# avikde/robobee3d

Hardware: AMD Instinct MI355X
Metric: closed-loop MPC steps/sec (QP+dyn) (higher is better)
Workload: dtype f32

## Files before the change

### robobee3d_amd/asmstep.py

```python
import functools
import os
import struct

from . import asmgen, asmtext, symbolic
from .asmgen import (A_D, A_L, A_LO, A_M, A_Q, NLDS, NVZ, S_ALPHA, S_CNT, S_ITERS, S_OMA, S_RHO, S_RINV, S_SIGMA,
                     V_W, V_WZ, V_X, V_Y, V_Z, Emit, f32bits, pk, _sb, _vp)

HERE = os.path.dirname(os.path.abspath(__file__))

PTRS = ["state", "ctrl", "ref", "ws", "out", "stats", "status", "info", "Ib", "gain", "aT0",
        "taskf", "weights", "wl", "wlu", "wlw",
        "done"]
NPTR_RES = 11
INTS = ["stride", "K", "maxIter", "nsub", "plant", "seq"]
TAIL_INTS = ["refstep"]
FLOATS = ["dt", "dtg", "Tmax", "wpr", "wpf", "ws_", "wvr", "wvf", "wds", "wthrust", "wmom",
          "iwpr", "iwpf", "iws", "iwvr", "iwvf", "iwds", "iwthrust", "iwmom",
          "Ib0", "Ib1", "Ib2", "Ibi0", "Ibi1", "Ibi2", "h", "hh", "h6", "taulim", "gpl", "idt", "mbg"]
WNAMES = ["wpr", "wpf", "ws_", "wvr", "wvf", "wds", "wthrust", "wmom"]
WROW = {"ws_": 0, "wds": 1, "wpr": 2, "wpf": 3, "wvr": 4, "wvf": 5, "wthrust": 6, "wmom": 7}
A_W, A_IW = 230, 238
S_PARAM = 4
S_PBLK = 2
S_PTR = {n: 40 + 2 * k for k, n in enumerate(PTRS[:NPTR_RES])}
S_PTR["taskf"], S_PTR["weights"] = 0, 96
S_PTR["wl"], S_PTR["wlu"], S_PTR["wlw"] = 30, 32, 34
S_INT = {"stride": 10, "K": 13, "maxIter": S_ITERS, "nsub": 5, "plant": 39}
S_F = {n: 64 + k for k, n in enumerate(FLOATS)}
assert max(S_F.values()) <= 95
S_STEP, S_SUB, S_RUIZ = 12, 15, 15
S_EXACT = 14
S_MBAD, S_MP0 = 62, 14
S_M0, S_M1, S_M2, S_M3 = 30, 32, 34, 36
S_C = {"minscal": 16, "maxscal": 17, "c45": 18, "eps10": 19, "eps": 38, "rho": 6, "rinv": 7, "rmin": 8,
       "rmininv": 9, "infty_ms": 100, "rhotol": 101}
S_TMP = 4
OFF = {}
_o = 0
for _n in PTRS:
    OFF[_n] = _o
    _o += 8
for _n in INTS + FLOATS + TAIL_INTS:
    OFF[_n] = _o
    _o += 4
PARAM_BYTES = _o
HIST_INTS = ["statestep", "outstep", "statusstep", "infostep"]
HIST_OFF = (PARAM_BYTES + 7) // 8 * 8
for _k, _n in enumerate(HIST_INTS):
    OFF[_n] = HIST_OFF + 4 * _k
HIST_BYTES = 4 * len(HIST_INTS)
S_HIST = 32
IMP_OFF = HIST_OFF + HIST_BYTES
assert IMP_OFF % 8 == 0
OFF["imp"], OFF["impstep"] = IMP_OFF, IMP_OFF + 8
IMP_BYTES = 16
S_IMP = 32

VFIRST, VEND = 2, 256
NRING = 6
XV_N, XV_B = 2, 254
NT_PTRS = ("state", "ctrl", "ref", "out", "stats")
A_SPARE, N_SPARE_D = 246, 9


class Pool:

    def __init__(self, e):
        self.e = e
        self.free_ = set(range(VFIRST, VEND))
        self.peak = 0
        self.fixed = set()

    def _take(self, regs):
        for r in regs:
            assert r in self.free_, "v%d is not free" % r
            self.free_.discard(r)
        self.peak = max(self.peak, VEND - VFIRST - len(self.free_))

    def reserve(self, lo, n):
        self._take(range(lo, lo + n))
        return lo

    def get(self):
        cand = sorted(self.free_)
        assert cand, "out of VGPRs"
        for r in cand:
            if (r ^ 1) not in self.free_:
                self._take([r])
                return r
        self._take([cand[0]])
        return cand[0]

    def get2(self):
        for r in sorted(self.free_):
            if r % 2 == 0 and r + 1 in self.free_:
                self._take([r, r + 1])
                return r
        raise AssertionError("out of aligned VGPR pairs")

    def get4(self):
        for r in sorted(self.free_):
            if r % 4 == 0 and all(r + k in self.free_ for k in range(4)):
                self._take([r, r + 1, r + 2, r + 3])
                return r
        raise AssertionError("out of aligned VGPR quads")

    def getn(self, n):
        for r in sorted(self.free_):
            if r % 2 == 0 and all(r + k in self.free_ for k in range(n)):
                self._take(range(r, r + n))
                return r
        raise AssertionError("out of consecutive VGPRs")

    def getn_high(self, n):
        r = VEND - n - (VEND - n) % 2
        assert all(r + k in self.free_ for k in range(n)), "top of the register file is not free"
        self._take(range(r, r + n))
        return r

    def free(self, *regs, kill=True):
        for r in regs:
            assert r not in self.free_ and VFIRST <= r < VEND, "double free v%d" % r
            self.free_.add(r)
            if kill:
                self.e("kill", "v%d" % r)

    def free_range(self, lo, n, kill=True):
        self.free(*range(lo, lo + n), kill=kill)


def v(n):
    return "v%d" % n


def SF_(n):
    return "s%d" % S_F[n]


def sg(n):
    return "s%d" % n


def sp(n):
    return "s[%d:%d]" % (n, n + 1)

# ... 17 lines not shown
    return ("v[%d:%d]" % (base, base + 1), lo_reg % 2, hi_reg % 2)


def PS(sreg):
    if sreg % 2 == 0:
        return ("s[%d:%d]" % (sreg, sreg + 1), 0, 0)
    return ("s[%d:%d]" % (sreg - 1, sreg), 1, 1)


class Struct:
    def __init__(self, N=3, perm=None):
        s = symbolic.analyse(N, perm)
        self.s = s
        self.plan = asmgen.solve_plan(s)
        self.lpos = self.plan[2]
        self.xs, self.zs, self.xinv, self.zinv = asmgen.slot_maps(s)
        nx, nc = s.nx, s.nc
        self.neq = 2 * s.N * symbolic.NY
        self.col_of = [0] * len(s.A_i)
        self.rows = [[] for _ in range(nc)]
        for j in range(nx):
            for p in range(s.A_p[j], s.A_p[j + 1]):
                self.col_of[p] = j
                self.rows[s.A_i[p]].append(p)
        self.unit = {}
        for p, tag in enumerate(s.A_tag):
            if tag[0] == 'c' and abs(tag[1]) == 1.0 and s.A_i[p] not in self.unit:
                self.unit[s.A_i[p]] = (p, self.col_of[p])
        assert len(self.unit) == nc
        used, pairs = set(), []
        for p in range(len(s.A_i)):
            if p in used:
                continue
            i0, j0 = s.A_i[p], self.col_of[p]
            for q_ in range(p + 1, len(s.A_i)):
                if q_ in used:
                    continue
                i1, j1 = s.A_i[q_], self.col_of[q_]
                if (self.zs[i0] ^ 1) == self.zs[i1] and (j0 == j1 or (self.xs[j0] ^ 1) == self.xs[j1]):
                    lo, hi = (p, q_) if self.zs[i0] % 2 == 0 else (q_, p)
                    pairs.append((lo, hi))
                    used.update((p, q_))
                    break
        self.apairs = pairs
        self.asingles = [p for p in range(len(s.A_i)) if p not in used]
        self.apos = [0] * len(s.A_i)
        k = 0
        for (lo, hi) in pairs:
            self.apos[lo], self.apos[hi] = k, k + 1
            k += 2
        for p in self.asingles:
            self.apos[p] = k
            k += 1
        self.na = k
        self.pair_of = {}
        for (lo, hi) in pairs:
            self.pair_of[lo] = self.pair_of[hi] = (lo, hi)
        NYv = symbolic.NY
        self.qnz = list(range(s.N * NYv)) + [s.N * NYv + k_ * NYv + i for k_ in range(s.N) for i in range(3)]
        self.qslot = {}
        for j in range(s.N * NYv):
            self.qslot[j] = self.xs[j]
        base = s.N * NYv
        for k_ in range(s.N):
            for i in range(3):
                self.qslot[s.N * NYv + k_ * NYv + i] = base + 3 * k_ + i
        self.nq = base + 3 * s.N
        self.qzero = frozenset(j for j in range(nx) if j not in self.qslot)
        lnz = set(range(6)) | set(range(3 * 6, 3 * 6 + 6)) | set(range(4 * 6, 4 * 6 + 3)) | {5 * 6 + 2}
        self.lzero = frozenset(i for i in range(self.neq) if i not in lnz) if s.N == 3 else frozenset()

    def weight_of(self, j):
        N, NYv = self.s.N, symbolic.NY
        if j < N * NYv:
            k, i = divmod(j, NYv)
            return ("wpf" if k == N - 1 else "wpr") if i < 3 else "ws_"
        if j < 2 * N * NYv:
            k, i = divmod(j - N * NYv, NYv)
            return ("wvf" if k == N - 1 else "wvr") if i < 3 else "wds"
        return "wthrust" if (j - 2 * N * NYv) % 3 == 0 else "wmom"


class StepGen:
    def __init__(self, N=3, perm=None, quad=False, exact_ruiz=False):
        self.st = Struct(N, perm)
        self.s = self.st.s
        self.e = Emit()
        self.pool = Pool(self.e)
        self.lab = 20
        self.lab_spec = 500
        self.quad = quad
        self.speculate = not quad and not exact_ruiz
        self.ruiz_span = self.restart_at = None
        self.nt = () if quad else ("nt",)
        self.homes = asmgen.Homes(NRING, 0 if quad else XV_N, XV_B)

    def label(self):
        self.lab += 1
        return str(self.lab)

    def label_spec(self):
        self.lab_spec += 1
        return str(self.lab_spec)

    def rcp_nr(self, dst, src, t):
        e = self.e
        e("v_rcp_f32", v(dst), v(src))
        e("s_nop", 0)
        e("v_fma_f32", v(t), "-" + v(src), v(dst), 1.0)
        e("v_fma_f32", v(dst), v(t), v(dst), v(dst))

    def rows_ptr(self, voff, first_row):
        e = self.e
        if first_row == 0:
            e("v_mov_b32", v(voff), "v0")
        else:
            e("s_mul_i32", sg(S_TMP), sg(S_INT["stride"]), first_row)
            e("v_add_u32", v(voff), sg(S_TMP), "v0")

    def load_taskf(self):
        e = self.e
        e("s_lshl_b32", sg(S_TMP), sg(S_STEP), 5)
        e("s_load_dwordx2", sp(S_M0), sp(S_PTR["taskf"]), sg(S_TMP), "offset:0")
        e("s_load_dwordx4", "s[%d:%d]" % (S_M0 + 2, S_M0 + 5), sp(S_PTR["taskf"]), sg(S_TMP), "offset:8")
        e("s_load_dwordx2", sp(S_M0 + 6), sp(S_PTR["taskf"]), sg(S_TMP), "offset:24")
        e("s_waitcnt", "vmcnt(0) lgkmcnt(0)")

    def adv(self, voff):
        self.e("v_add_u32", v(voff), sg(S_INT["stride"]), v(voff))

    def advance_ptr(self, ptr, sstep):
        e, lo = self.e, S_PTR[ptr]
        e("s_add_i32", sg(lo), sg(lo), sg(sstep))
        e("s_cmp_lt_u32", sg(lo), sg(sstep))
        e("s_cselect_b32", sg(sstep), 1, 0)
        e("s_add_i32", sg(lo + 1), sg(lo + 1), sg(sstep))

    def impulse(self, Y0, YS):
        e = self.e
        lab_off = self.label()
        lo, hi, st, oh = S_IMP, S_IMP + 1, S_IMP + 2, S_IMP + 3
        e("s_mov_b32", sg(S_TMP), IMP_OFF)
        e("s_load_dwordx4", "s[%d:%d]" % (S_IMP, S_IMP + 3), sp(S_PBLK), sg(S_TMP))
        e("s_waitcnt", "lgkmcnt(0)")
        e("s_cmp_eq_u64", sp(lo), 0)
        e("s_cbranch_scc1", lab_off + "f")
        e("s_mul_hi_u32", sg(oh), sg(S_STEP), sg(st))
        e("s_mul_i32", sg(st), sg(S_STEP), sg(st))
        e("s_add_i32", sg(hi), sg(hi), sg(oh))
        for i in range(6):
            addend = st if i == 0 else S_INT["stride"]
            lab_nc = self.label()
            e("s_add_i32", sg(lo), sg(lo), sg(addend))
            e("s_cmp_gt_u32", sg(addend), sg(lo))
            e("s_cbranch_scc0", lab_nc + "f")
            e("s_add_i32", sg(hi), sg(hi), 1)
            e("label", lab_nc)
            e("global_load_dword", v(YS + i), "v0", sp(lo))
        e("s_waitcnt", "vmcnt(0)")
        for i in range(6):
            e("v_add_f32", v(Y0 + 12 + i), v(Y0 + 12 + i), v(YS + i))
        e("label", lab_off)

    def load_rows(self, ptr, first_row, regs, voff=None):
        own = voff is None
        if own:
            voff = self.pool.get()
        self.rows_ptr(voff, first_row)
        for k, r in enumerate(regs):
            self.e("global_load_dword", r if isinstance(r, str) else v(r), v(voff), sp(S_PTR[ptr]),
                   *(self.nt if ptr in NT_PTRS or ptr == "ws" else ()))
            if k + 1 < len(regs):
                self.adv(voff)
        if own:
            self.pool.free(voff, kill=False)

    def store_rows(self, ptr, first_row, regs, voff=None):
        own = voff is None
        if own:
            voff = self.pool.get()
        self.rows_ptr(voff, first_row)
        for k, r in enumerate(regs):
            self.e("global_store_dword", v(voff), v(r), sp(S_PTR[ptr]),
                   *(self.nt if ptr in NT_PTRS else ()))
            if k + 1 < len(regs):
                self.adv(voff)
        if own:
            self.pool.free(voff, kill=False)

    def prologue(self):
        e = self.e
        P = sp(S_PARAM)
        e("s_mov_b64", sp(S_PBLK), P)
        P = sp(S_PBLK)
        e("s_load_dwordx16", "s[40:55]", P, OFF["state"])
        e("s_load_dwordx4", "s[56:59]", P, OFF["state"] + 64)
        e("s_load_dwordx2", "s[60:61]", P, OFF["state"] + 80)
        e("s_load_dwordx2", sp(S_PTR["taskf"]), P, OFF["taskf"])
        e("s_load_dwordx2", sp(S_PTR["weights"]), P, OFF["weights"])
        e("s_load_dwordx16", "s[64:79]", P, OFF[FLOATS[0]])
        e("s_load_dwordx16", "s[80:95]", P, OFF[FLOATS[0]] + 64)
        for n in S_INT:
            e("s_load_dword", sg(S_INT[n]), P, OFF[n])
        assert len(FLOATS) == 32
        import numpy as np
        f32 = np.float32
        for reg, val in ((S_ALPHA, 1.6), (S_OMA, float(f32(1.0) - f32(1.6))), (S_SIGMA, 1e-6), (S_RINV, 0.01), (S_RHO, 100.0)):
            e("s_mov_b32", sg(reg), f32bits(val))
            e("s_mov_b32", sg(reg + 1), f32bits(val))
        for name, val in (("minscal", 1e-4), ("maxscal", 1e4), ("c45", float(f32(1.0) / f32(self.s.nx))),
                          ("eps", 1e-4), ("eps10", float(f32(10) * f32(1e-4))), ("rho", 0.1), ("rinv", float(f32(1.0) / f32(0.1))),
                          ("rmin", 1e-6), ("rmininv", float(f32(1.0) / f32(1e-6))),
                          ("infty_ms", float(f32(1e30) * f32(1e-4))), ("rhotol", 1e-4)):
            e("s_mov_b32", sg(S_C[name]), f32bits(val))
        e("s_waitcnt", "lgkmcnt(0)")
        e("s_mov_b32", sg(S_STEP), 0)

    def phase_a(self):
        e, pool, st, s = self.e, self.pool, self.st, self.s
        N, NYv = s.N, symbolic.NY
        nx, nc, neq = s.nx, s.nc, st.neq
        SF = lambda n: sg(S_F[n])
        ST = [pool.get() for _ in range(18)]
        RF = [pool.get() for _ in range(9)]
        T0, EP = pool.get(), [pool.get() for _ in range(N)]
        voff = pool.get()
        self.load_rows("state", 0, ST, voff)
        self.load_rows("ref", 0, RF, voff)
        self.load_rows("ctrl", nx + 2 * nc, [T0] + EP, voff)
        WV = {n: pool.get() for n in WNAMES}
        IWV = {n: pool.get() for n in WNAMES}
        self.WV = WV
        lab_w, lab_w2 = self.label(), self.label()
        e("s_cmp_eq_u64", sp(S_PTR["weights"]), 0)
        e("s_cbranch_scc1", lab_w + "f")
        self.rows_ptr(voff, 0)
        by_row = sorted(WNAMES, key=lambda n: WROW[n])
        for k, n in enumerate(by_row):
            e("global_load_dword", v(WV[n]), v(voff), sp(S_PTR["weights"]))
            if k + 1 < len(by_row):
                self.adv(voff)
        e("s_waitcnt", "vmcnt(0)")
        t = pool.get()
        for n in WNAMES:
            self.rcp_nr(IWV[n], WV[n], t)
        pool.free(t)
        e("s_branch", lab_w2 + "f")
        e("label", lab_w)
        for n in WNAMES:
            e("v_mov_b32", v(WV[n]), SF(n))
            e("v_mov_b32", v(IWV[n]), SF("i" + n.rstrip("_")))
        e("label", lab_w2)
        for k, n in enumerate(WNAMES):
            e("v_accvgpr_write_b32", "a%d" % (A_W + k), v(WV[n]))
            e("v_accvgpr_write_b32", "a%d" % (A_IW + k), v(IWV[n]))
        pool.free(*IWV.values(), *WV.values())
        lab_tk = self.label()
        e("s_cmp_eq_u64", sp(S_PTR["taskf"]), 0)
        e("s_cbranch_scc1", lab_tk + "f")
        self.load_taskf()
        for i in range(3):
            e("v_add_f32", v(RF[i]), sg(S_M0 + i), v(RF[i]))
            e("v_mov_b32", v(RF[3 + i]), sg(S_M0 + 3 + i))
        e("v_mov_b32", v(RF[6]), sg(S_M0 + 6))
        e("v_mov_b32", v(RF[7]), 0)
        e("v_mov_b32", v(RF[8]), sg(S_M0 + 7))
        e("label", lab_tk)
        ibi0, ibi1 = pool.get(), pool.get()
        lab_ib, lab_ib2 = self.label(), self.label()
        e("s_cmp_eq_u64", sp(S_PTR["Ib"]), 0)
        e("s_cbranch_scc1", lab_ib + "f")
        t = pool.get()
        self.load_rows("Ib", 0, [ibi0, ibi1], voff)
        e("s_waitcnt", "vmcnt(0)")
        tt = pool.get()
        for r in (ibi0, ibi1):
            e("v_mov_b32", v(tt), v(r))
            self.rcp_nr(r, tt, t)
        pool.free(t, tt)
        e("s_branch", lab_ib2 + "f")
        e("label", lab_ib)
        e("v_mov_b32", v(ibi0), SF("Ibi0"))
        e("v_mov_b32", v(ibi1), SF("Ibi1"))
        e("label", lab_ib2)
        e("s_waitcnt", "vmcnt(0)")
        lab_t = self.label()
        e("s_cmp_eq_u64", sp(S_PTR["aT0"]), 0)
        e("s_cbranch_scc1", lab_t + "f")
        e("s_cmp_lg_u32", sg(S_STEP), 0)
        e("s_cbranch_scc1", lab_t + "f")
        t = pool.get()
        e("global_load_dword", v(t), "v0", sp(S_PTR["aT0"]))
        e("s_waitcnt", "vmcnt(0)")
        e("v_cmp_le_f32", "vcc", 0, v(t))
        e("v_cndmask_b32", v(T0), v(T0), v(t), "vcc")
        pool.free(t)
        e("label", lab_t)
        self.store_rows("ctrl", nx + 2 * nc, [T0], voff)
# ... 574 lines not shown
                    e("v_mov_b32", v(XV_B + pos - NLDS - NVZ), v(nL[j]))
                else:
                    e("v_accvgpr_write_b32", "a%d" % (A_L + pos - NLDS), v(nL[j]))
                pool.free(nL.pop(j))
            retire_dinv(c)

        for op in s.factor_ops:
            k = op["k"]
            src = s.K_src[op["diag"]]
            dk = pool.get()
            if src[0] == 'P':
                e("v_add_f32", v(dk), sg(S_SIGMA), v(RP(src[1])))
                pool.free(RP(src[1]))
            else:
                assert src[0] == 'R'
                i = src[1]
                if i < neq:
                    e("v_mul_f32", v(dk), -1.0, self._vconst_rinv())
                else:
                    e("v_accvgpr_read_b32", v(dk), "a%d" % (A_M + 9 + i - neq))
                    e("s_nop", 0)
                    e("v_mul_f32", v(dk), -1.0, v(dk))
            y = {}
            for (b, p) in op["init"]:
                assert s.K_src[p][0] == 'A'
                y[b] = (RA(s.K_src[p][1]), False)
            for (c, upd, new) in op["elim"]:
                yc, owned = y.pop(c)
                for (lj, row) in upd:
                    if row in y:
                        reg, own = y[row]
                        if own:
                            e("v_fmac_f32", v(reg), v(nL[lj]), v(yc))
                        else:
                            nr = pool.get()
                            e("v_fma_f32", v(nr), v(nL[lj]), v(yc), v(reg))
                            pool.free(reg)
                            y[row] = (nr, True)
                    else:
                        nr = pool.get()
                        e("v_mul_f32", v(nr), v(nL[lj]), v(yc))
                        y[row] = (nr, True)
                nl = pool.get()
                e("v_mul_f32", v(nl), "-" + v(yc), v(Dinv[c]))
                e("v_fmac_f32", v(dk), v(yc), v(nl))
                nL[new] = nl
                pool.free(yc)
            assert not y
            di = pool.get()
            self.rcp_nr(di, dk, t)
            pool.free(dk)
            Dinv[k] = di
            for c in done_at.get(k, []):
                retire_col(c)
            if k not in last_row:
                retire_dinv(k)
        assert not nL and not Dinv
        pool.free(t)
        if self._rinv_reg is not None:
            pool.free(self._rinv_reg)
            self._rinv_reg = None
        if st.na % 2:
            pool.free(self.VA + st.na)
        pool.free(self.VP + nx)

    _rinv_reg = None

    def _vconst_rinv(self):
        if self._rinv_reg is None:
            self._rinv_reg = self.pool.get()
            self.e("v_mov_b32", v(self._rinv_reg), sg(S_RINV))
        return v(self._rinv_reg)

    def admm(self):
        e, pool, st, s = self.e, self.pool, self.st, self.s
        nx, nc = s.nx, s.nc
        left = set(range(VFIRST, VEND)) - pool.free_ - set(range(246, 256))
        assert not left, "phase A leaked registers: %s" % sorted(left)
        pool.reserve(V_W, V_X - V_W)
        pool.reserve(V_X, V_Y - V_X)
        pool.reserve(V_Y, V_Z - V_Y)
        pool.reserve(V_Z, 40)
        voff = 245
        self.load_rows("ctrl", 0, [V_X + st.xs[r] for r in range(nx)] + [V_Y + st.zs[r] for r in range(nc)] +
                       [V_Z + st.zs[r] for r in range(nc)], voff)
        for pad in (V_X + nx, V_Y + nc, V_Z + nc, V_W + nx, V_WZ + nc):
            e("v_mov_b32", v(pad), 0)
        e("s_waitcnt", "vmcnt(0) lgkmcnt(0)")
        plan = st.plan
        zk = dict(qzero=st.qzero, lzero=st.lzero, homes=self.homes)
        asmgen.body(e, s, first=True, capture=True, plan=plan, delta_in_w=True, **zk)
        if self.quad:
            from . import asmquad
            lab6 = self.label()
            e("s_cmp_lt_i32", sg(S_ITERS), 2)
            e("s_cbranch_scc1", lab6 + "f")
            asmquad.section(e, asmquad.QuadPlan(st), self.label)
            e("label", lab6)
        else:
            self._admm_rest(plan, zk)
        for i in range(st.neq):
            pool.free(V_Z + st.zs[i], kill=True)
        pool.free_range(246, 10)


    def _admm_rest(self, plan, zk):
        e, s, st = self.e, self.s, self.st
        import numpy as np
        for p_ in range(NVZ):
            e("v_accvgpr_read_b32", v(V_Z + p_), "a%d" % (A_L + p_))
        lab7, lab6 = self.label(), self.label()
        e("s_sub_i32", sg(S_CNT), sg(S_ITERS), 1)
        e("s_cmp_lt_i32", sg(S_CNT), 1)
        e("s_cbranch_scc1", lab6 + "f")
        e("label", lab7)
        asmgen.body(e, s, first=False, capture=False, plan=plan, lv=True, dy3_in_w=True, **zk)
        e("s_sub_i32", sg(S_CNT), sg(S_CNT), 1)
        e("s_cmp_gt_i32", sg(S_CNT), 0)
        e("s_cbranch_scc1", lab7 + "b")
        k = float(np.float32(1.6) / (np.float32(1.6) - np.float32(1.0)))
        e("s_mov_b32", sg(S_TMP), f32bits(k))
        nx, neq = s.nx, st.neq
        for p_ in range(0, nx - 1, 2):
            pk(e, "v_pk_add_f32", V_W + p_, [P2(V_X + p_), P2(V_W + p_)], [0, 1])
        for p_ in range(0, nx - 1, 2):
            pk(e, "v_pk_mul_f32", V_W + p_, [PS(S_TMP), P2(V_W + p_)])
        if nx % 2:
            jl = st.xinv[nx - 1]
            e("v_sub_f32", v(V_W + st.xs[jl]), v(V_X + st.xs[jl]), v(V_W + st.xs[jl]))
            e("v_mul_f32", v(V_W + st.xs[jl]), sg(S_TMP), v(V_W + st.xs[jl]))
        for p_ in range(0, neq, 2):
            pk(e, "v_pk_add_f32", V_WZ + p_, [P2(V_Y + p_), P2(V_WZ + p_)], [0, 1])
        for p_ in range(0, neq, 2):
            pk(e, "v_pk_mul_f32", V_WZ + p_, [PS(S_TMP), P2(V_WZ + p_)])
        e("label", lab6)

    def phase_c(self):
        e, pool, st, s = self.e, self.pool, self.st, self.s
        N, NYv = s.N, symbolic.NY
        nx, nc, neq = s.nx, s.nc, st.neq
        SF = lambda n: sg(S_F[n])
        g_ = pool.get
        XR = lambda j: V_X + st.xs[j]
        YR = lambda i: V_Y + st.zs[i]
        ZR = lambda i: V_Z + st.zs[i]
        DXR = lambda j: V_W + st.xs[j]
        DYR = lambda i: V_WZ + st.zs[i]
        voff = g_()
        def slot_blocks(n, chunk=16):
            n2 = n + n % 2
            blocks = [(lo, pool.getn(min(chunk, n2 - lo))) for lo in range(0, n2, chunk)]
            def reg(slot):
                for lo, base in reversed(blocks):
                    if slot >= lo:
                        return base + slot - lo
            return reg, [(base, min(chunk, n2 - lo)) for lo, base in blocks]
        DS, dblocks = slot_blocks(nx)
        DR = lambda j: DS(st.xs[j])
        cr, T0 = g_(), g_()
        npark = 0 if self.quad else N_SPARE_D
        self.load_rows("ws", npark, [DR(j) for j in range(npark, nx)], voff)
        if npark:
            for j in range(npark):
                e("v_accvgpr_read_b32", v(DR(j)), "a%d" % (A_SPARE + j))
            e("v_accvgpr_read_b32", v(cr), "a%d" % (A_SPARE + N_SPARE_D))
        else:
            self.load_rows("ws", asmgen.WS_C - asmgen.WS_DS, [cr], voff)
        self.load_rows("ctrl", nx + 2 * nc, [T0], voff)
        e("v_mov_b32", v(DS(nx)), 0)
        zt = [g_() for _ in range(4)]
        self.rows_ptr(voff, 0)
        for r in range(nx):
            e("global_store_dword", v(voff), v(XR(r)), sp(S_PTR["ctrl"]), *self.nt)
            self.adv(voff)
        for r in range(nc):
            e("global_store_dword", v(voff), v(YR(r)), sp(S_PTR["ctrl"]), *self.nt)
            self.adv(voff)
        for r in range(nc):
            if r < neq:
                t_ = zt[r % 4]
                e("v_accvgpr_read_b32", v(t_), "a%d" % (A_LO + r))
                e("global_store_dword", v(voff), v(t_), sp(S_PTR["ctrl"]), *self.nt)
            else:
                e("global_store_dword", v(voff), v(ZR(r)), sp(S_PTR["ctrl"]), *self.nt)
            self.adv(voff)
        pool.free(*zt)
        e("s_waitcnt", "vmcnt(0)")
        for k in range(0, nx + 1, 2):
            pk(e, "v_pk_mul_f32", V_W + k, [P2(DS(k)), P2(V_W + k)])
            pk(e, "v_pk_mul_f32", V_X + k, [P2(DS(k)), P2(V_X + k)])
        for base, n_ in dblocks:
            pool.free_range(base, n_)
        ES, eblocks = slot_blocks(nc)
        ER = lambda i: ES(st.zs[i])
        ST = [g_() for _ in range(18)]
        RF = [g_() for _ in range(9)]
        self.load_rows("ws", asmgen.WS_ES - asmgen.WS_DS, [ER(i) for i in range(nc)], voff)
        self.load_rows("state", 0, ST, voff)
        self.load_rows("ref", 0, RF, voff)
        e("v_mov_b32", v(ES(nc)), 1.0)
        lab_tk = self.label()
        e("s_cmp_eq_u64", sp(S_PTR["taskf"]), 0)
        e("s_cbranch_scc1", lab_tk + "f")
        self.load_taskf()
        for i in range(3):
            e("v_add_f32", v(RF[i]), sg(S_M0 + i), v(RF[i]))
            e("v_mov_b32", v(RF[3 + i]), sg(S_M0 + 3 + i))
        e("v_mov_b32", v(RF[6]), sg(S_M0 + 6))
        e("v_mov_b32", v(RF[7]), 0)
        e("v_mov_b32", v(RF[8]), sg(S_M0 + 7))
        e("label", lab_tk)
        cinv, t = g_(), g_()
        self.rcp_nr(cinv, cr, t)
        pool.free(cr)
        ibi0, ibi1 = g_(), g_()
        lab_ib, lab_ib2 = self.label(), self.label()
        e("s_cmp_eq_u64", sp(S_PTR["Ib"]), 0)
        e("s_cbranch_scc1", lab_ib + "f")
        self.load_rows("Ib", 0, [ibi0, ibi1], voff)
        e("s_waitcnt", "vmcnt(0)")
        tt = g_()
        for r in (ibi0, ibi1):
            e("v_mov_b32", v(tt), v(r))
            self.rcp_nr(r, tt, t)
        pool.free(tt)
        e("s_branch", lab_ib2 + "f")
        e("label", lab_ib)
        e("v_mov_b32", v(ibi0), SF("Ibi0"))
        e("v_mov_b32", v(ibi1), SF("Ibi1"))
        e("label", lab_ib2)
        e("s_waitcnt", "vmcnt(0)")
        for k in range(0, nc + 1, 2):
            pk(e, "v_pk_mul_f32", V_WZ + k, [P2(ES(k)), P2(V_WZ + k)])
            pk(e, "v_pk_mul_f32", V_Y + k, [P2(ES(k)), P2(V_Y + k)])
        for k in range(0, nc + 1, 2):
            pk(e, "v_pk_mul_f32", V_Y + k, [P2(V_Y + k), PB(cinv)])
        pool.free(cinv)
        zu3 = [g_() for _ in range(N)]
        for k in range(N):
            e("v_rcp_f32", v(zu3[k]), v(ER(neq + k)))
        e("s_nop", 0)
        for k in range(N):
            e("v_mul_f32", v(zu3[k]), v(ZR(neq + k)), v(zu3[k]))
        for base, n_ in eblocks:
            pool.free_range(base, n_)
        for k in range(N):
            pool.free(ZR(neq + k))
        pool.free(V_Z + nc)
        p0, R0, dq0 = ST[0:3], ST[3:12], ST[12:18]
        dtT0 = g_()
        e("v_mul_f32", v(dtT0), SF("dt"), v(T0))
        s0dt = [g_() for _ in range(3)]
        Bdt = [g_() for _ in range(6)]
        for i in range(3):
            e("v_mul_f32", v(s0dt[i]), SF("dt"), v(R0[6 + i]))
            e("v_mul_f32", v(Bdt[i]), "-" + v(R0[i + 3]), v(ibi0))
            e("v_mul_f32", v(Bdt[3 + i]), v(R0[i]), v(ibi1))
        for i in range(6):
            e("v_mul_f32", v(Bdt[i]), SF("dt"), v(Bdt[i]))
        pool.free(ibi0, ibi1)
        ds0 = [g_() for _ in range(3)]
        for r in range(3):
            e("v_mul_f32", v(t), "-" + v(R0[r]), v(dq0[4]))
            e("v_mul_f32", v(ds0[r]), v(R0[r + 3]), v(dq0[3]))
            e("v_add_f32", v(ds0[r]), v(t), v(ds0[r]))
            e("v_mul_f32", v(ds0[r]), -1.0, v(ds0[r]))
        y0 = p0 + R0[6:9]
        dy0 = dq0[0:3] + ds0
        LR = {}
# ... 175 lines not shown
        e("v_fma_f32", v(a1), sg(S_C["eps"]), v(reld), sg(S_C["eps"]))
        lt(MD0, v(dua), v(a1))
        e("v_fma_f32", v(a1), sg(S_C["eps10"]), v(relp), sg(S_C["eps10"]))
        lt(MP1, v(pri), v(a1))
        e("v_fma_f32", v(a1), sg(S_C["eps10"]), v(reld), sg(S_C["eps10"]))
        lt(MD1, v(dua), v(a1))
        e("v_mov_b32", v(stv), -2)

        def cert(epsname, okmask, code, kind):
            nrm_, n_, s_, third = (ndy, lhs, nrm, None) if kind == "p" else (ndx, qdx, nP, nAdx)
            e("v_mul_f32", v(a1), sg(S_C[epsname]), v(nrm_))
            lt(MT, sg(S_C[epsname]), v(nrm_))
            e("s_andn2_b64", MT, MT, okmask)
            lt("vcc", v(n_), "-" + v(a1))
            e("s_and_b64", MT, MT, "vcc")
            lt("vcc", v(s_), v(a1))
            e("s_and_b64", MT, MT, "vcc")
            if third is not None:
                lt("vcc", v(a1), v(third))
                e("s_andn2_b64", MT, MT, "vcc")
            e("v_cndmask_b32_e64", v(stv), v(stv), code, MT)
        cert("eps10", MD1, 4, "d")
        cert("eps10", MP1, 3, "p")
        e("s_and_b64", MT, MP1, MD1)
        e("v_cndmask_b32_e64", v(stv), v(stv), 2, MT)
        cert("eps", MD0, -4, "d")
        cert("eps", MP0, -3, "p")
        e("s_and_b64", MT, MP0, MD0)
        e("v_cndmask_b32_e64", v(stv), v(stv), 1, MT)
        lt(MT, v(infv), v(pri))
        lt("vcc", v(infv), v(dua))
        e("s_or_b64", MT, MT, "vcc")
        e("v_cmp_u_f32", "vcc", v(nan), v(nan))
        e("s_or_b64", MT, MT, "vcc")
        e("v_cndmask_b32_e64", v(stv), v(stv), -7, MT)
        e("v_cmp_eq_i32_e64", MBAD, -7, v(stv))
        for code in (-3, 3, -4, 4):
            e("v_cmp_eq_i32_e64", MT, code, v(stv))
            e("s_or_b64", MBAD, MBAD, MT)
        pool.free(ndy, lhs, nrm, ndx, qdx, nP, nAdx, relp, reld, nAx, nz, nq, nAty, nPx, nan, infv, a3, a4)
        nanv = g_()
        e("v_mov_b32", v(nanv), f32bits(2143289344.0))
        sol = [XR(2 * N * NYv + i) for i in range(3)] + [XR(N * NYv + i) for i in range(6)]
        e("s_mov_b64", "vcc", MBAD)
        for r in sol:
            e("v_cndmask_b32", v(r), v(r), v(nanv), "vcc")
        pool.free(nanv)
        u0, u1, u2 = sol[0:3]
        dy1 = sol[3:9]
        OUT = [g_() for _ in range(9)]
        e("v_add_f32", v(OUT[0]), v(T0), v(u0))
        e("v_mov_b32", v(OUT[1]), v(u1))
        e("v_mov_b32", v(OUT[2]), v(u2))
        e("v_mul_f32", v(a1), v(R0[0]), v(dy1[3]))
        e("v_mul_f32", v(t), v(R0[1]), v(dy1[4]))
        e("v_add_f32", v(a1), v(a1), v(t))
        e("v_mul_f32", v(t), v(R0[2]), v(dy1[5]))
        e("v_add_f32", v(a1), v(a1), v(t))
        e("v_mul_f32", v(a2), v(R0[3]), v(dy1[3]))
        e("v_mul_f32", v(t), v(R0[4]), v(dy1[4]))
        e("v_add_f32", v(a2), v(a2), v(t))
        e("v_mul_f32", v(t), v(R0[5]), v(dy1[5]))
        e("v_add_f32", v(a2), v(a2), v(t))
        for i in range(3):
            e("v_sub_f32", v(OUT[3 + i]), v(dy1[i]), v(dq0[i]))
        e("v_sub_f32", v(OUT[6]), "-" + v(a2), v(dq0[3]))
        e("v_sub_f32", v(OUT[7]), v(a1), v(dq0[4]))
        e("v_sub_f32", v(OUT[8]), 0, v(dq0[5]))
        for i in range(6):
            e("v_mul_f32", v(OUT[3 + i]), SF("idt"), v(OUT[3 + i]))
        self.store_rows("out", 0, OUT, voff)
        lab_s, lab_i, lab_c = self.label(), self.label(), self.label()
        e("s_cmp_eq_u64", sp(S_PTR["status"]), 0)
        e("s_cbranch_scc1", lab_s + "f")
        e("global_store_dword", "v0", v(stv), sp(S_PTR["status"]))
        e("label", lab_s)
        e("s_cmp_eq_u64", sp(S_PTR["info"]), 0)
        e("s_cbranch_scc1", lab_i + "f")
        self.store_rows("info", 0, [pri, dua], voff)
        e("label", lab_i)
        e("s_and_saveexec_b64", sp(S_M1), MBAD)
        e("s_cbranch_execz", lab_c + "f")
        e("v_mov_b32", v(a1), 0)
        self.rows_ptr(voff, 0)
        for r in range(nx + 2 * nc):
            e("global_store_dword", v(voff), v(a1), sp(S_PTR["ctrl"]))
            self.adv(voff)
        e("label", lab_c)
        e("s_mov_b64", "exec", sp(S_M1))
        pool.free(pri, dua, stv, a1, a2, t, T0, *RF)
        pool.free_range(V_W, V_X - V_W, kill=False)
        pool.free_range(V_X, V_Y - V_X, kill=False)
        pool.free_range(V_Y, V_Z - V_Y, kill=False)
        T0n = g_()
        e("v_mov_b32", v(T0n), v(OUT[0]))
        self.wl_step(OUT, R0, T0n, voff)
        self.store_rows("ctrl", nx + 2 * nc, [T0n], voff)
        pool.free(T0n)
        self.plant(ST, OUT, voff)
        pool.free(*OUT, *ST, voff)
        assert len(pool.free_) == VEND - VFIRST, "phase C leaked registers: %s" % sorted(set(range(VFIRST, VEND)) - pool.free_)

    def wl_step(self, OUT, R0, T0n, voff):
        e, pool = self.e, self.pool
        g_ = pool.get
        lab_end = self.label()
        P = sp(S_PBLK)
        e("s_load_dwordx2", sp(S_PTR["wl"]), P, OFF["wl"])
        e("s_load_dwordx2", sp(S_PTR["wlu"]), P, OFF["wlu"])
        e("s_load_dwordx2", sp(S_PTR["wlw"]), P, OFF["wlw"])
        e("s_waitcnt", "lgkmcnt(0)")
        e("s_cmp_eq_u64", sp(S_PTR["wl"]), 0)
        e("s_cbranch_scc1", lab_end + "f")
        O_UMIN, O_UMAX, O_DUMAX, O_QW, O_A0, O_A1, O_A2, O_MD = 0, 4, 8, 12, 18, 24, 48, 144
        a1, a2, t = g_(), g_(), g_()
        zero = g_()
        e("v_mov_b32", v(zero), 0)

        def prm(dst, word):
            e("global_load_dword", v(dst), v(zero), sp(S_PTR["wl"]), "offset:%d" % (4 * word))
        u0 = [g_() for _ in range(4)]
        self.load_rows("wlu", 0, u0, voff)
        Md = [g_() for _ in range(6)]
        for i in range(6):
            prm(Md[i], O_MD + i)
        e("s_waitcnt", "vmcnt(0)")
        h0 = [g_() for _ in range(3)]
        pd = [g_() for _ in range(6)]
        for c in range(3):
            e("v_mul_f32", v(h0[c]), SF_("mbg"), v(R0[2 + 3 * c]))
        for i in range(6):
            e("v_mul_f32", v(pd[i]), v(Md[i]), v(OUT[3 + i]))
        w0 = [g_() for _ in range(6)]
        a0v = [g_() for _ in range(6)]
        A1 = [[g_() for _ in range(4)] for _ in range(6)]
        PA = [g_() for _ in range(21)]
        vout = [g_() for _ in range(4)]
        dot, quad = g_(), g_()
        for i in range(6):
            prm(PA[0], O_A0 + i)
            for l in range(4):
                prm(PA[1 + l], O_A1 + 4 * i + l)
            for k in range(16):
                prm(PA[5 + k], O_A2 + 16 * i + k)
            e("s_waitcnt", "vmcnt(0)")
            e("v_mul_f32", v(dot), v(u0[0]), v(PA[1]))
            for l in range(1, 4):
                e("v_mul_f32", v(t), v(u0[l]), v(PA[1 + l]))
                e("v_add_f32", v(dot), v(dot), v(t))
            for r in range(4):
                e("v_mul_f32", v(vout[r]), v(PA[5 + r]), v(u0[0]))
                for l in range(1, 4):
                    e("v_mul_f32", v(t), v(PA[5 + r + 4 * l]), v(u0[l]))
                    e("v_add_f32", v(vout[r]), v(vout[r]), v(t))
            e("v_mul_f32", v(quad), v(u0[0]), v(vout[0]))
            for l in range(1, 4):
                e("v_mul_f32", v(t), v(u0[l]), v(vout[l]))
                e("v_add_f32", v(quad), v(quad), v(t))
            e("v_add_f32", v(a1), v(PA[0]), v(dot))
            e("v_mul_f32", v(a2), 0.5, v(quad))
            e("v_add_f32", v(w0[i]), v(a1), v(a2))
            if i < 3:
                e("v_sub_f32", v(a0v[i]), v(w0[i]), v(h0[i]))
            else:
                e("v_mov_b32", v(a0v[i]), v(w0[i]))
            e("v_sub_f32", v(a0v[i]), v(a0v[i]), v(pd[i]))
# ... 322 lines not shown
        for k in range(0, 8, 2):
            pk(e, "v_pk_fma_f32", QS + k, [PS(S_F["hh"]), P2(QA + k), P2(Q0 + k)])
        vf(QS, QK)
        for k in range(0, 8, 2):
            pk(e, "v_pk_fma_f32", QA + k, [PB(two), P2(QK + k), P2(QA + k)])
            pk(e, "v_pk_fma_f32", QS + k, [PS(S_F["hh"]), P2(QK + k), P2(Q0 + k)])
        vf(QS, QK)
        for k in range(0, 8, 2):
            pk(e, "v_pk_fma_f32", QA + k, [PB(two), P2(QK + k), P2(QA + k)])
            pk(e, "v_pk_fma_f32", QS + k, [PS(S_F["h"]), P2(QK + k), P2(Q0 + k)])
        vf(QS, QK)
        for k in range(0, 8, 2):
            pk(e, "v_pk_add_f32", QA + k, [P2(QA + k), P2(QK + k)])
        for k in range(0, 8, 2):
            pk(e, "v_pk_fma_f32", Q0 + k, [PS(S_F["h6"]), P2(QA + k), P2(Q0 + k)])
        e("s_nop", 1)
        for r in range(3):
            e("v_mov_b32_dpp", v(PA + r), v(Q0), asmquad.qperm([r] * 4))
        e("s_nop", 1)
        for r in range(3):
            e("v_fmac_f32", v(serr), v(PA + r), v(PA + r))
        e("v_add_f32", v(seff), v(seff), v(einc))
        e("s_sub_i32", sg(S_SUB), sg(S_SUB), 1)
        e("s_cmp_gt_i32", sg(S_SUB), 0)
        e("s_cbranch_scc1", top + "b")
        e("s_nop", 1)
        for r in range(3):
            e("v_mov_b32_dpp", v(Y0 + r), v(Q0), asmquad.qperm([r] * 4))
            e("v_mov_b32_dpp", v(Y0 + 12 + r), v(Q0 + 1), asmquad.qperm([r] * 4))
            for c in range(3):
                e("v_mov_b32_dpp", v(Y0 + 3 + r + 3 * c), v(Q0 + 2 + c), asmquad.qperm([r] * 4))
        for i in range(3):
            e("v_mov_b32", v(Y0 + 15 + i), v(Q0 + 5 + i))
        e("s_nop", 1)
        e("quad_end", tuple(keep))

    def program(self):
        e = self.e
        self.prologue()
        top = self.label()
        e("label", top)
        if self.speculate:
            e("s_mov_b32", sg(S_EXACT), 0)
            self.lab_restart = self.label_spec()
            e("label", self.lab_restart)
        self.phase_a()
        self.admm()
        self.phase_c()
        e("s_load_dword", sg(S_TMP), sp(S_PBLK), OFF["refstep"])
        e("s_load_dwordx4", "s[%d:%d]" % (S_HIST, S_HIST + 3), sp(S_PBLK), HIST_OFF)
        e("s_waitcnt", "lgkmcnt(0)")
        e("s_add_u32", sg(S_PTR["ref"]), sg(S_PTR["ref"]), sg(S_TMP))
        e("s_addc_u32", sg(S_PTR["ref"] + 1), sg(S_PTR["ref"] + 1), 0)
        for n in ("out", "status", "info"):
            self.advance_ptr(n, S_HIST + HIST_INTS.index(n + "step"))
        e("s_add_i32", sg(S_STEP), sg(S_STEP), 1)
        e("s_cmp_lt_i32", sg(S_STEP), sg(S_INT["K"]))
        e("s_cbranch_scc1", top + "b")
        e("s_waitcnt", "vmcnt(0) lgkmcnt(0)")
        lab = self.label()
        e("s_load_dwordx2", sp(S_M0), sp(S_PBLK), OFF["done"])
        e("s_load_dword", sg(S_M1), sp(S_PBLK), OFF["seq"])
        e("s_waitcnt", "lgkmcnt(0)")
        e("s_cmp_eq_u64", sp(S_M0), 0)
        e("s_cbranch_scc1", lab + "f")
        e("buffer_wbl2", "sc0 sc1")
        e("s_waitcnt", "vmcnt(0)")
        a, b = self.pool.get(), self.pool.get()
        e("v_mov_b32", v(a), 0)
        e("v_mov_b32", v(b), sg(S_M1))
        e("global_store_dword", v(a), v(b), sp(S_M0), "sc0 sc1")
        e("s_waitcnt", "vmcnt(0)")
        self.pool.free(a, b)
        e("label", lab)
        return e.ins


fmt = functools.partial(asmtext.fmt, hex_ints=asmtext.HEX_ABOVE_64)


PSEUDO = ("kill", "quad_begin", "quad_end")


def write(path=None, N=3, perm=None, quad=False):
    path = path or os.path.join(HERE, "csrc", "umpc_step_asm_quad.h" if quad else "umpc_step_asm.h")
    g = StepGen(N, perm, quad=quad)
    ins = [t for t in g.program() if t[0] not in PSEUDO]
    if quad:
        head = ["// GENERATED by robobee3d_amd/asmstep.py (quad=True) + asmquad.py -- do not edit.", asmgen.switch_banner(),
               "// The all-assembly fp32 step kernel body, ONE ROBOT PER LANE QUAD (16 robots per wavefront): %d instructions."
               % len(ins),
               "// Every lane of a quad gets the same v0 (= 4 * robot) and its own LDS slice; include umpc_step_asm.h first (StepParams).",
               "#pragma once"]
    else:
        head = ["// GENERATED by robobee3d_amd/asmstep.py -- do not edit.", asmgen.switch_banner(),
               "// The all-assembly fp32 step kernel body: %d instructions (K closed-loop steps of one wavefront)." % len(ins),
               "#pragma once", "#include <stddef.h>", "#include <stdint.h>", "namespace umpcasm {",
               "// parameter block read by the kernel with s_load (byte offsets are part of the generated code)",
               "struct StepParams {"]
        for n in PTRS:
            head.append("  const void *%s;" % n)
        for n in INTS:
            head.append("  int32_t %s;" % n)
        for n in FLOATS:
            head.append("  float %s;" % n)
        for n in TAIL_INTS:
            head.append("  int32_t %s;" % n)
        head += ["};", "static_assert(sizeof(StepParams) == %d, \"StepParams layout\");" % ((PARAM_BYTES + 7) // 8 * 8),
                "// step history (umpcBatchSetHistory): bytes the state / out / status / info pointers advance per closed-loop step,",
                "// read by the stream at byte %d of the kernarg segment: the kernels take ONE StepArgs as their first argument" % HIST_OFF,
                "struct StepHist {"] + ["  int32_t %s;" % n for n in HIST_INTS] + ["};",
                "// velocity impulses (umpcBatchSetImpulses): slice `cursor` of the table [steps][6][B] (null: none) and the bytes per slice,",
                "// read by the stream at byte %d of the kernarg segment" % IMP_OFF,
                "struct StepImp {", "  const void *imp;", "  int32_t impstep;", "  int32_t pad_;", "};",
                "struct StepArgs {", "  StepParams p;", "  StepHist h;", "  StepImp i;", "};",
                "static_assert(offsetof(StepArgs, h) == %d && sizeof(StepHist) == %d, \"StepHist layout\");" % (HIST_OFF, HIST_BYTES),
                "static_assert(offsetof(StepArgs, i) == %d && sizeof(StepImp) == %d && offsetof(StepImp, impstep) == 8, \"StepImp layout\");" % (IMP_OFF, IMP_BYTES),
                "constexpr int STEP_LDS_BYTES_PER_LANE = %d;" % (NLDS * 4), "}  // namespace umpcasm",
                "// inputs: v0 = 4 * robot, v1 = lane LDS address, s[4:5] = &StepParams (kernarg)"]
    asmtext.write_if_changed(path, asmtext.asm_block(
        head, "UMPC_STEP_ASM%s(voff, ldsaddr, params)" % ("_QUAD" if quad else ""), ins,
        '"{v0}"(voff), "{v1}"(ldsaddr), "{s[4:5]}"(params)',
        asmtext.clobbers(range(2, 256), range(256), range(4, 102)), fmt))
    return path, len(ins)


_KEEP_V = {0, 1} | set(range(V_W, V_Z)) | set(range(V_Z + 2 * 3 * symbolic.NY, V_Z + 40))
QUAD = {None: None}


def _quad():
    from . import isasim
    if QUAD[None] is None:
        QUAD.update({None: isasim.Quad(v=_KEEP_V, dead_v=set(range(256)) - _KEEP_V, a=range(A_LO, 256), dead_a=range(A_LO)),
                     "ruiz": isasim.Quad(a=range(256)), "plant": isasim.Quad(a=range(256))})
    return QUAD


FLAT = ("taskf", "wl")
STRIDE = 4096
PBASE = 0x00007E0080000000


def simulate(ins, arrays, ints, floats, max_exec=3000000, ptr_xform=None, lanes=1, hits=False):
    import numpy as np
    from . import isasim
    base_of = {n: 0x00007F0080000000 + (k << 36) for k, n in enumerate(PTRS + ["impulse"])}
    ptr_xform = ptr_xform or (lambda a: a)
    blob = bytearray(IMP_OFF + IMP_BYTES)
    for n in PTRS:
        struct.pack_into("<Q", blob, OFF[n], ptr_xform(base_of[n]) if arrays.get(n) is not None else 0)
    stride = STRIDE if lanes == 1 else 4 * lanes
    allints = dict(ints, stride=stride)
    allints.setdefault("seq", 0)
    allints.setdefault("refstep", 0)
    for n in HIST_INTS:
        allints.setdefault(n, 0)
    for n in INTS + TAIL_INTS + HIST_INTS:
        struct.pack_into("<i", blob, OFF[n], int(allints[n]))
    for n in FLOATS:
        struct.pack_into("<f", blob, OFF[n], float(floats[n]))
    allints.setdefault("impstep", 6 * stride if arrays.get("impulse") is not None else 0)
    struct.pack_into("<Q", blob, OFF["imp"], ptr_xform(base_of["impulse"]) if arrays.get("impulse") is not None else 0)
    struct.pack_into("<i", blob, OFF["impstep"], int(allints["impstep"]))
    regions = [(PBASE, 4, np.frombuffer(bytes(blob), np.uint32))] + \
        [(base_of[n], 4 if n in FLAT or lanes > 1 else STRIDE, arrays[n].reshape(-1))
         for n in PTRS + ["impulse"] if arrays.get(n) is not None]
    assert all(arrays[n].flags.c_contiguous for n in PTRS + ["impulse"] if arrays.get(n) is not None)
    m = isasim.Machine(ins, lanes, regions=regions, sgpr={S_PARAM: PBASE & 0xFFFFFFFF, S_PARAM + 1: PBASE >> 32},
                       vgpr={0: 4 * np.arange(lanes)}, lds=np.zeros((lanes, NLDS), np.uint32), max_exec=max_exec,
                       quad=_quad() if lanes == 1 else None)
    if hits:
        m.hits = np.zeros(len(ins), np.int64)
    isasim.run(m)
    simulate.last_hits = m.hits
    simulate.last_quad_sections = {("admm" if k is None else k): n for k, n in m.sections.items()}
    simulate.last_quad_instructions = sum(m.sections.values())
    return m.nexec


if __name__ == "__main__":
    p, n = write()
    print("wrote", p, n, "instructions")


def host_floats(dt=5.0, g=9.81e-3, TtoWmax=2.0, ws=1e1, wds=1e3, wpr=1.0, wpf=5.0, wvr=1e3, wvf=2e3, wthrust=1e-1, wmom=1e-2,
                Ib=(3333.0, 3333.0, 1000.0), dtsim=0.2, taulim=100.0, mb=100.0):
    import numpy as np
    f = np.float32
    one = f(1.0)
    w = dict(wpr=f(wpr), wpf=f(wpf), ws_=f(ws), wvr=f(wvr), wvf=f(wvf), wds=f(wds), wthrust=f(wthrust), wmom=f(wmom))
    d = dict(dt=f(dt), dtg=f(f(dt) * f(g)), Tmax=f(f(TtoWmax) * f(g)), **w)
    for k, val in w.items():
        d["i" + k.rstrip("_")] = f(one / val)
    for i in range(3):
        d["Ib%d" % i] = f(Ib[i])
        d["Ibi%d" % i] = f(one / f(Ib[i]))
    d.update(h=f(dtsim), hh=f(f(0.5) * f(dtsim)), h6=f(f(dtsim) / f(6.0)), taulim=f(taulim), gpl=f(9.81e-3), idt=f(one / f(dt)),
             mbg=f(f(mb) * f(g)))
    assert set(d) == set(FLOATS), set(FLOATS) ^ set(d)
    return {k: float(val) for k, val in d.items()}
```

### robobee3d_amd/csrc/umpc_mi355x.hip

```cpp
#include <hip/hip_runtime.h>

#include <chrono>
#include <cstdint>
#include <cstdio>
#include <cstdlib>
#include <cstring>
#include <map>
#include <mutex>
#include <string>

#include "umpc_handle.h"
#include "umpc_step.h"
#ifndef UMPC_STEP_ASM_HEADER
#define UMPC_STEP_ASM_HEADER "umpc_step_asm.h"
#endif
#include UMPC_STEP_ASM_HEADER
#include "umpc_step_asm_quad.h"
#include "umpc_n3_general.h"

namespace {

using umpc::DevParams;
using namespace umpcgen;

// ... 99 lines not shown
}

template <typename T>
__device__ __forceinline__ void assemble_rows(const DevParams<T> &prm, int B_, int b, const T *state, const T *ctrl,
                                              const T *refA, const T *IbA, const T *actualT0, T *l, T *u, T *q, T *Px, T *Ax) {
  const size_t B = (size_t)B_;
  T p[3], R[9], dq[6], ref[9], Ibi[3];
#pragma unroll
  for (int i = 0; i < 3; ++i) p[i] = state[(size_t)i * B + b];
#pragma unroll
  for (int i = 0; i < 9; ++i) R[i] = state[(size_t)(3 + i) * B + b];
#pragma unroll
  for (int i = 0; i < 6; ++i) dq[i] = state[(size_t)(12 + i) * B + b];
#pragma unroll
  for (int i = 0; i < 9; ++i) ref[i] = refA[(size_t)i * B + b];
#pragma unroll
  for (int i = 0; i < 3; ++i) Ibi[i] = T(1) / (IbA ? IbA[(size_t)i * B + b] : prm.Ib[i]);
  T T0 = ctrl ? ctrl[(size_t)(NX + 2 * NC) * B + b] : T(0);
  if (actualT0 && (!ctrl || actualT0[b] >= T(0))) T0 = actualT0[b];
  umpc::RawQP<T> qp;
  const umpc::Weights<T> wt = {prm.ws, prm.wds, prm.wpr, prm.wpf, prm.wvr, prm.wvf, prm.wthrust, prm.wmom};
  umpc::assemble(prm, wt, Ibi, T0, p, R, dq, ref, qp);
#pragma unroll
  for (int i = 0; i < NC; ++i) {
    l[(size_t)i * B + b] = qp.l[i];
    u[(size_t)i * B + b] = i < NEQ ? qp.l[i] : qp.u3[i - NEQ];
  }
#pragma unroll
  for (int j = 0; j < NX; ++j) { q[(size_t)j * B + b] = qp.q[j]; Px[(size_t)j * B + b] = qp.Px[j]; }
  int o = 0;
#pragma unroll
  for (int k = 0; k < 3 * (N - 2); ++k) Ax[(size_t)(o++) * B + b] = qp.dtT0;
#pragma unroll
  for (int k = 0; k < 6 * N; ++k) Ax[(size_t)(o++) * B + b] = prm.dt;
#pragma unroll
  for (int k = 0; k < N; ++k)
#pragma unroll
    for (int i = 0; i < 3; ++i) Ax[(size_t)(o++) * B + b] = qp.s0dt[i];
#pragma unroll
  for (int k = 0; k < N; ++k)
#pragma unroll
    for (int i = 0; i < 6; ++i) Ax[(size_t)(o++) * B + b] = qp.Btaudt[i];
}

__global__ void umpc_taskf_kernel(DevParams<float> prm, int K, float t0, float *tab) {
  const int k = blockIdx.x * blockDim.x + threadIdx.x;
  if (k >= K) return;
  float r[9] = {0.f, 0.f, 0.f, 0.f, 0.f, 0.f, 0.f, 0.f, 0.f};
  const float tnow = t0 + float(k) * (float(prm.nsub) * prm.dtsim);
  umpc::task_reference(prm.task, prm.task_p, tnow, r);
  float *o = tab + 8 * (size_t)k;
  o[0] = r[0]; o[1] = r[1]; o[2] = r[2]; o[3] = r[3]; o[4] = r[4]; o[5] = r[5]; o[6] = r[6]; o[7] = r[8];
}

template <typename T>
__global__ void umpc_init_ctrl_kernel(int B_, T *ctrl) {
  const size_t B = (size_t)B_;
  for (size_t i = (size_t)blockIdx.x * blockDim.x + threadIdx.x; i < (size_t)UMPC_CTRL_ROWS * B;
       i += (size_t)gridDim.x * blockDim.x)
    ctrl[i] = (i / B) >= (size_t)(NX + 2 * NC + 1) ? T(1) : T(0);
}

}

struct RolloutArrays {
  void *state = nullptr, *ctrl = nullptr;
  const void *ref = nullptr, *actualT0 = nullptr, *Ib = nullptr, *gain = nullptr;
  void *out = nullptr, *stats = nullptr;
  int32_t *status = nullptr;
  void *info = nullptr;
};

struct HistStep { size_t state = 0, out = 0, status = 0, info = 0; };

static int launched(umpc_batch_t *h, const char *kernel) {
  h->last_kernel = kernel;
  return launch_status("umpcBatchRollout");
}

static umpcasm::StepParams make_step_params(umpc_batch_t *h, int K, int nsub, const RolloutArrays &io) {
  umpcasm::StepParams p;
  p.state = io.state; p.ctrl = io.ctrl; p.ref = io.ref; p.out = io.out; p.stats = io.stats; p.status = io.status;
  p.ws = (char *)h->ws + (size_t)umpcasm::WS_DS * (size_t)h->B * 4;
  p.info = io.info; p.Ib = io.Ib; p.gain = io.gain; p.aT0 = io.actualT0;
  p.taskf = nullptr; p.weights = h->weights; p.wl = h->wl; p.wlu = h->wlu; p.wlw = h->wlw;
  p.done = nullptr; p.seq = 0; p.refstep = 0;
  p.stride = h->B * 4; p.K = K; p.maxIter = h->prm.maxIter; p.nsub = nsub; p.plant = h->prm.plant_mode;
  const umpc_batch_params_t &q = h->prm;
  const float one = 1.0f;
  p.dt = (float)q.dt; p.dtg = (float)q.dt * (float)q.g; p.Tmax = (float)q.TtoWmax * (float)q.g;
  p.wpr = (float)q.wpr; p.wpf = (float)q.wpf; p.ws_ = (float)q.ws; p.wvr = (float)q.wvr; p.wvf = (float)q.wvf;
  p.wds = (float)q.wds; p.wthrust = (float)q.wthrust; p.wmom = (float)q.wmom;
  p.iwpr = one / p.wpr; p.iwpf = one / p.wpf; p.iws = one / p.ws_; p.iwvr = one / p.wvr; p.iwvf = one / p.wvf;
  p.iwds = one / p.wds; p.iwthrust = one / p.wthrust; p.iwmom = one / p.wmom;
  p.Ib0 = (float)q.Ib[0]; p.Ib1 = (float)q.Ib[1]; p.Ib2 = (float)q.Ib[2];
  p.Ibi0 = one / p.Ib0; p.Ibi1 = one / p.Ib1; p.Ibi2 = one / p.Ib2;
  p.h = (float)q.dtsim; p.hh = 0.5f * p.h; p.h6 = p.h / 6.0f; p.taulim = (float)q.taulim; p.gpl = 9.81e-3f;
  p.idt = one / p.dt;
  p.mbg = h->wl ? h->wl_md2 * (float)q.g : 0.0f;
  return p;
}

template <typename T>
static int launch_quad64_stepwise(const umpc::StepIO<T> &a, int K, const T *actualT0, const HistStep &hs, hipStream_t stream) {
  for (int k = 0; k < K; ++k) {
    umpc::StepIO<T> ak = a;
    if (hs.state) {
      ak.state = a.state + ((size_t)k + 1) * hs.state;
      const hipError_t ec = hipMemcpyAsync(ak.state, a.state + (size_t)k * hs.state, hs.state * sizeof(T),
                                           hipMemcpyDeviceToDevice, stream);
      if (ec != hipSuccess) return fail(ec, "umpcBatchRollout: history");
    }
    ak.ref = a.ref + (size_t)k * a.ref_step; ak.out = a.out + (size_t)k * hs.out;
    if (a.status) ak.status = a.status + (size_t)k * hs.status;
    if (a.info) ak.info = a.info + (size_t)k * hs.info;
    ak.t0 = a.t0 + T(k) * (T(a.prm.nsub) * a.prm.dtsim);
    ak.ref_step = ak.state_step = ak.out_step = ak.status_step = ak.info_step = ak.imp_step = 0;
    ak.imp = nullptr;
    hipLaunchKernelGGL((umpc_rollout_kernel<T, true, true, true>), dim3((a.B + kBlock / 4 - 1) / (kBlock / 4)), dim3(kBlock), 0,
                       stream, ak, 1, k == 0 ? actualT0 : nullptr, 0);
    if (a.imp)
      hipLaunchKernelGGL(umpc_impulse_kernel<T>, dim3((a.B + 255) / 256), dim3(256), 0, stream, ak.state,
                         a.imp + (size_t)k * a.imp_step, a.B);
    const hipError_t el = hipGetLastError();
    if (el != hipSuccess) return fail(el, "umpcBatchRollout: history / impulses");
  }
  return 0;
}

template <typename T>
static int launch_steps(umpc_batch_t *h, int K, int nsub, RolloutArrays io, const HistStep &hs, void *stream) {
  size_t ref_step = 0;
  if (h->reftab) {
    ref_step = (size_t)9 * (size_t)h->B;
    io.ref = (const T *)h->reftab + (size_t)h->ref_c.cursor * ref_step;
  }
  umpc::StepIO<T> a;
  a.prm = make_dev_task<T>(h);
  a.prm.nsub = nsub;
  a.B = h->B;
  a.state = (T *)io.state; a.ctrl = (T *)io.ctrl; a.ref = (const T *)io.ref; a.ref_step = (unsigned)ref_step;
  a.state_step = (unsigned)hs.state; a.out_step = (unsigned)hs.out; a.status_step = (unsigned)hs.status; a.info_step = (unsigned)hs.info;
  const size_t imp_step = (size_t)6 * (size_t)h->B;
  const bool imp_on = h->imp_on(K, nsub);
  a.imp = imp_on ? (const T *)h->imptab + (size_t)h->imp_c.cursor * imp_step : nullptr;
  a.imp_step = imp_on ? (unsigned)imp_step : 0u;
  a.weights = (const T *)h->weights; a.t0 = (T)h->t_ms;
  a.Ib = (const T *)io.Ib; a.gain = (const T *)io.gain; a.ws = (T *)h->ws; a.out = (T *)io.out; a.stats = (T *)io.stats;
  a.status = io.status; a.info = (T *)io.info;
  a.wl = h->wl; a.wlu = (T *)h->wlu; a.wlw = (T *)h->wlw;
  const hipStream_t s = (hipStream_t)stream;
  const int grid = (h->B + kBlock - 1) / kBlock, qgrid = (h->B + kBlock / 4 - 1) / (kBlock / 4);
  if constexpr (sizeof(T) == 4) {
    static const bool no_asm = getenv("UMPC_NO_ASM_STEP") != nullptr;
    const bool fits = (size_t)UMPC_CTRL_ROWS * (size_t)h->B * 4 < ((size_t)1 << 31);
    if (!no_asm && h->step_kernel != 1 && fits && K >= 1 && h->prm.maxIter >= 1) {
      umpcasm::StepArgs pa;
      umpcasm::StepParams &p = pa.p;
      p = make_step_params(h, K, nsub, io);
      p.refstep = (int32_t)(ref_step * 4);
      pa.h.statestep = (int32_t)(hs.state * 4); pa.h.outstep = (int32_t)(hs.out * 4);
      pa.h.statusstep = (int32_t)(hs.status * 4); pa.h.infostep = (int32_t)(hs.info * 4);
      pa.i.imp = a.imp; pa.i.impstep = (int32_t)(a.imp_step * 4); pa.i.pad_ = 0;
      if (h->task != 0) {
        if (K > h->taskf_cap) {
          if (h->taskf) (void)hipFree(h->taskf);
          h->taskf = nullptr; h->taskf_cap = 0;
          const int cap = K < 1024 ? 1024 : K;
          const hipError_t em = hipMalloc((void **)&h->taskf, (size_t)cap * 8 * sizeof(float));
          if (em != hipSuccess) return fail(em, "umpcBatchRollout: task table");
          h->taskf_cap = cap;
        }
        hipLaunchKernelGGL(umpc_taskf_kernel, dim3((K + 255) / 256), dim3(256), 0, s, a.prm, K, a.t0, h->taskf);
        p.taskf = h->taskf;
      }
      if (h->step_kernel == 3 || (h->step_kernel == 0 && h->global_B <= quad_max_b())) {
        hipLaunchKernelGGL(umpc_rollout_asm_quad_kernel, dim3(qgrid), dim3(kBlock), 0, s, pa, h->B);
        return launched(h, "umpc_rollout_asm_quad_kernel");
      }
      static const int skew_us10 = [] { const char *e_ = getenv("UMPC_ASM_SKEW_US"); return e_ ? (int)(atof(e_) * 10) : 0; }();
      static const int skew_groups = [] { const char *e_ = getenv("UMPC_ASM_SKEW_GROUPS"); return e_ ? atoi(e_) : 4; }();
      const int skew_ticks = (h->B >= 32768 && K >= 2) ? skew_us10 * 10 : 0;
      hipLaunchKernelGGL(umpc_rollout_asm_kernel, dim3(grid), dim3(kBlock), 0, s, pa, h->B, skew_ticks,
                         skew_groups < 1 ? 1 : skew_groups);
      return launched(h, "umpc_rollout_asm_kernel");
    }
  }
  const T *const aT0 = (const T *)io.actualT0;
  if constexpr (sizeof(T) == 8) {
    static const bool no_ldsf = getenv("UMPC_NO_F64_LDS") != nullptr;
    static const bool no_asm64 = getenv("UMPC_NO_ASM64") != nullptr;
    static const int ldsf_max_grid = [] { const char *e_ = getenv("UMPC_F64_LDS_MAX_GRID"); return e_ ? atoi(e_) : 0x7fffffff; }();
    if (!no_ldsf && grid <= ldsf_max_grid) {
      const bool asm64 = !no_asm64 && h->step_kernel != 1 && (size_t)umpc::WS_ROWS * (size_t)h->B * 8 < ((size_t)1 << 31);
      static const int quad64_max_b = [] { const char *e_ = getenv("UMPC_QUAD64"); return e_ ? atoi(e_) : 4096; }();
      const bool want_quad = h->step_kernel == 3 || (h->step_kernel == 0 && h->global_B <= quad64_max_b);
      if (asm64 && h->prm.maxIter >= 2 && want_quad) {
        const bool moved = hs.state || hs.out || hs.status || hs.info || a.imp;
        if (!moved) hipLaunchKernelGGL((umpc_rollout_kernel<T, true, true, true>), dim3(qgrid), dim3(kBlock), 0, s, a, K, aT0, 0);
        else if (const int rc = launch_quad64_stepwise<T>(a, K, aT0, hs, s)) return rc;
        return launched(h, "umpc_rollout_kernel<double, LDSF, ASM64, QUAD>");
      }
      if (asm64 && h->prm.maxIter >= 1) {
        hipLaunchKernelGGL((umpc_rollout_kernel<T, true, true>), dim3(grid), dim3(kBlock), 0, s, a, K, aT0, 0);
        return launched(h, "umpc_rollout_kernel<double, LDSF, ASM64>");
      }
      hipLaunchKernelGGL((umpc_rollout_kernel<T, true, false>), dim3(grid), dim3(kBlock), 0, s, a, K, aT0, 0);
      return launched(h, "umpc_rollout_kernel<double, LDSF>");
    }
  }
  const char *env = getenv("UMPC_SKEW_US");
  const int skew_us = env ? atoi(env) : (K >= 64 && sizeof(T) == 4 && h->B >= 32768 ? 80 : 0);
  hipLaunchKernelGGL((umpc_rollout_kernel<T, false, false>), dim3(grid), dim3(kBlock), 0, s, a, K, aT0, skew_us * 100);
  return launched(h, sizeof(T) == 4 ? "umpc_rollout_kernel<float>" : "umpc_rollout_kernel<double>");
}

template <typename T>
static int launch_rollout(umpc_batch_t *h, int K, int nsub, const RolloutArrays &io, void *stream) {
  const bool hist = h->hist_on(K, nsub), imp = h->imp_on(K, nsub);
  if (h->reftab && !h->ref_c.fits("umpcBatchRollout", "reference trajectory", "K ", K)) return -1;
  if (hist && !h->hist_c.fits("umpcBatchRollout", "step history", "K ", K)) return -1;
  if (imp && !h->imp_c.fits("umpcBatchRollout", "impulse table", "K ", K)) return -1;
  if (!io.state || !io.ctrl || (!io.ref && !h->reftab) || !io.out) { g_err = "umpcBatchRollout: null array"; return -1; }
  RolloutArrays t = io;
  HistStep hs;
  const size_t B = (size_t)h->B, c = (size_t)h->hist_c.cursor, last = (size_t)K - 1;
  if (hist && h->hist_state) { hs.state = 18 * B; t.state = (T *)h->hist_state + c * hs.state; }
  if (hist && h->hist_out) { hs.out = 9 * B; t.out = (T *)h->hist_out + c * hs.out; }
  if (hist && h->hist_status) { hs.status = B; t.status = h->hist_status + c * hs.status; }
  if (hist && h->hist_info) { hs.info = 2 * B; t.info = (T *)h->hist_info + c * hs.info; }
  const hipStream_t s = (hipStream_t)stream;
  hipError_t e = hipSuccess;
  if (hs.state && t.state != io.state) e = hipMemcpyAsync(t.state, io.state, hs.state * sizeof(T), hipMemcpyDeviceToDevice, s);
  if (e != hipSuccess) return fail(e, "umpcBatchRollout: history");
  if (const int rc = launch_steps<T>(h, K, nsub, t, hs, stream)) return rc;
  T *const st_end = (T *)t.state + (size_t)K * hs.state;
  if (hs.state && st_end != (T *)io.state) e = hipMemcpyAsync(io.state, st_end, hs.state * sizeof(T), hipMemcpyDeviceToDevice, s);
  if (e == hipSuccess && hs.out)
// ... 501 lines not shown
```

### robobee3d_amd/csrc/umpc_step_asm.h

```cpp
#pragma once
#include <stddef.h>
#include <stdint.h>
namespace umpcasm {
struct StepParams {
  const void *state;
  const void *ctrl;
  const void *ref;
  const void *ws;
  const void *out;
  const void *stats;
  const void *status;
  const void *info;
  const void *Ib;
  const void *gain;
  const void *aT0;
  const void *taskf;
  const void *weights;
  const void *wl;
  const void *wlu;
  const void *wlw;
  const void *done;
  int32_t stride;
  int32_t K;
  int32_t maxIter;
  int32_t nsub;
  int32_t plant;
  int32_t seq;
  float dt;
  float dtg;
  float Tmax;
  float wpr;
  float wpf;
  float ws_;
  float wvr;
  float wvf;
  float wds;
  float wthrust;
  float wmom;
  float iwpr;
  float iwpf;
  float iws;
  float iwvr;
  float iwvf;
  float iwds;
  float iwthrust;
  float iwmom;
  float Ib0;
  float Ib1;
  float Ib2;
  float Ibi0;
  float Ibi1;
  float Ibi2;
  float h;
  float hh;
  float h6;
  float taulim;
  float gpl;
  float idt;
  float mbg;
  int32_t refstep;
};
static_assert(sizeof(StepParams) == 296, "StepParams layout");
struct StepHist {
  int32_t statestep;
  int32_t outstep;
  int32_t statusstep;
  int32_t infostep;
};
struct StepImp {
  const void *imp;
  int32_t impstep;
  int32_t pad_;
};
struct StepArgs {
  StepParams p;
  StepHist h;
  StepImp i;
};
static_assert(offsetof(StepArgs, h) == 296 && sizeof(StepHist) == 16, "StepHist layout");
static_assert(offsetof(StepArgs, i) == 312 && sizeof(StepImp) == 16 && offsetof(StepImp, impstep) == 8, "StepImp layout");
constexpr int STEP_LDS_BYTES_PER_LANE = 640;
}
#define UMPC_STEP_ASM(voff, ldsaddr, params) asm volatile( \
  "s_mov_b64 s[2:3], s[4:5]\n" \
  "s_load_dwordx16 s[40:55], s[2:3], 0x0\n" \
  "s_load_dwordx4 s[56:59], s[2:3], 0x40\n" \
  "s_load_dwordx2 s[60:61], s[2:3], 0x50\n" \
  "s_load_dwordx2 s[0:1], s[2:3], 0x58\n" \
  "s_load_dwordx2 s[96:97], s[2:3], 0x60\n" \
  "s_load_dwordx16 s[64:79], s[2:3], 0xa0\n" \
  "s_load_dwordx16 s[80:95], s[2:3], 0xe0\n" \
  "s_load_dword s10, s[2:3], 0x88\n" \
  "s_load_dword s13, s[2:3], 0x8c\n" \
  "s_load_dword s11, s[2:3], 0x90\n" \
  "s_load_dword s5, s[2:3], 0x94\n" \
  "s_load_dword s39, s[2:3], 0x98\n" \
  "s_mov_b32 s20, 0x3fcccccd\n" \
  "s_mov_b32 s21, 0x3fcccccd\n" \
  "s_mov_b32 s22, 0xbf19999a\n" \
  "s_mov_b32 s23, 0xbf19999a\n" \
  "s_mov_b32 s24, 0x358637bd\n" \
  "s_mov_b32 s25, 0x358637bd\n" \
  "s_mov_b32 s26, 0x3c23d70a\n" \
  "s_mov_b32 s27, 0x3c23d70a\n" \
  "s_mov_b32 s28, 0x42c80000\n" \
  "s_mov_b32 s29, 0x42c80000\n" \
  "s_mov_b32 s16, 0x38d1b717\n" \
  "s_mov_b32 s17, 0x461c4000\n" \
  "s_mov_b32 s18, 0x3cb60b61\n" \
  "s_mov_b32 s38, 0x38d1b717\n" \
  "s_mov_b32 s19, 0x3a83126e\n" \
  "s_mov_b32 s6, 0x3dcccccd\n" \
  "s_mov_b32 s7, 0x41200000\n" \
  "s_mov_b32 s8, 0x358637bd\n" \
  "s_mov_b32 s9, 0x49742400\n" \
  "s_mov_b32 s100, 0x6aa56fa6\n" \
  "s_mov_b32 s101, 0x38d1b717\n" \
  "s_waitcnt lgkmcnt(0)\n" \
  "s_mov_b32 s12, 0\n" \
  "21:\n" \
  "s_mov_b32 s14, 0\n" \
  "501:\n" \
  "v_mov_b32 v33, v0\n" \
  "global_load_dword v2, v33, s[40:41] nt\n" \
  "v_add_u32 v33, s10, v33\n" \
  "global_load_dword v3, v33, s[40:41] nt\n" \
  "v_add_u32 v33, s10, v33\n" \
  "global_load_dword v4, v33, s[40:41] nt\n" \
  "v_add_u32 v33, s10, v33\n" \
  "global_load_dword v5, v33, s[40:41] nt\n" \
  "v_add_u32 v33, s10, v33\n" \
  "global_load_dword v6, v33, s[40:41] nt\n" \
  "v_add_u32 v33, s10, v33\n" \
  "global_load_dword v7, v33, s[40:41] nt\n" \
  "v_add_u32 v33, s10, v33\n" \
  "global_load_dword v8, v33, s[40:41] nt\n" \
  "v_add_u32 v33, s10, v33\n" \
  "global_load_dword v9, v33, s[40:41] nt\n" \
  "v_add_u32 v33, s10, v33\n" \
  "global_load_dword v10, v33, s[40:41] nt\n" \
  "v_add_u32 v33, s10, v33\n" \
  "global_load_dword v11, v33, s[40:41] nt\n" \
  "v_add_u32 v33, s10, v33\n" \
  "global_load_dword v12, v33, s[40:41] nt\n" \
  "v_add_u32 v33, s10, v33\n" \
  "global_load_dword v13, v33, s[40:41] nt\n" \
  "v_add_u32 v33, s10, v33\n" \
  "global_load_dword v14, v33, s[40:41] nt\n" \
  "v_add_u32 v33, s10, v33\n" \
  "global_load_dword v15, v33, s[40:41] nt\n" \
  "v_add_u32 v33, s10, v33\n" \
  "global_load_dword v16, v33, s[40:41] nt\n" \
  "v_add_u32 v33, s10, v33\n" \
  "global_load_dword v17, v33, s[40:41] nt\n" \
  "v_add_u32 v33, s10, v33\n" \
  "global_load_dword v18, v33, s[40:41] nt\n" \
  "v_add_u32 v33, s10, v33\n" \
  "global_load_dword v19, v33, s[40:41] nt\n" \
  "v_mov_b32 v33, v0\n" \
  "global_load_dword v20, v33, s[44:45] nt\n" \
  "v_add_u32 v33, s10, v33\n" \
  "global_load_dword v21, v33, s[44:45] nt\n" \
  "v_add_u32 v33, s10, v33\n" \
  "global_load_dword v22, v33, s[44:45] nt\n" \
  "v_add_u32 v33, s10, v33\n" \
  "global_load_dword v23, v33, s[44:45] nt\n" \
  "v_add_u32 v33, s10, v33\n" \
  "global_load_dword v24, v33, s[44:45] nt\n" \
  "v_add_u32 v33, s10, v33\n" \
  "global_load_dword v25, v33, s[44:45] nt\n" \
  "v_add_u32 v33, s10, v33\n" \
  "global_load_dword v26, v33, s[44:45] nt\n" \
  "v_add_u32 v33, s10, v33\n" \
  "global_load_dword v27, v33, s[44:45] nt\n" \
  "v_add_u32 v33, s10, v33\n" \
  "global_load_dword v28, v33, s[44:45] nt\n" \
  "s_mul_i32 s4, s10, 0x7b\n" \
  "v_add_u32 v33, s4, v0\n" \
  "global_load_dword v29, v33, s[42:43] nt\n" \
  "v_add_u32 v33, s10, v33\n" \
  "global_load_dword v30, v33, s[42:43] nt\n" \
  "v_add_u32 v33, s10, v33\n" \
  "global_load_dword v31, v33, s[42:43] nt\n" \
  "v_add_u32 v33, s10, v33\n" \
  "global_load_dword v32, v33, s[42:43] nt\n" \
  "s_cmp_eq_u64 s[96:97], 0\n" \
  "s_cbranch_scc1 22f\n" \
  "v_mov_b32 v33, v0\n" \
  "global_load_dword v36, v33, s[96:97]\n" \
  "v_add_u32 v33, s10, v33\n" \
  "global_load_dword v39, v33, s[96:97]\n" \
  "v_add_u32 v33, s10, v33\n" \
  "global_load_dword v34, v33, s[96:97]\n" \
  "v_add_u32 v33, s10, v33\n" \
  "global_load_dword v35, v33, s[96:97]\n" \
  "v_add_u32 v33, s10, v33\n" \
  "global_load_dword v37, v33, s[96:97]\n" \
  "v_add_u32 v33, s10, v33\n" \
  "global_load_dword v38, v33, s[96:97]\n" \
  "v_add_u32 v33, s10, v33\n" \
  "global_load_dword v40, v33, s[96:97]\n" \
// ... 3645 lines not shown
  "v_fmac_f32 v14, v144, v159\n" \
  "v_mul_f32 v12, -v159, v4\n" \
  "v_fmac_f32 v3, v159, v12\n" \
  "v_fmac_f32 v121, v139, v93\n" \
  "v_fmac_f32 v14, v120, v93\n" \
  "v_mul_f32 v159, -v93, v164\n" \
  "v_fmac_f32 v3, v93, v159\n" \
  "v_fmac_f32 v14, v7, v121\n" \
  "v_mul_f32 v93, -v121, v6\n" \
  "v_fmac_f32 v3, v121, v93\n" \
  "v_mul_f32 v121, -v14, v27\n" \
  "v_fmac_f32 v3, v14, v121\n" \
  "v_rcp_f32 v14, v3\n" \
  "s_nop 0\n" \
  "v_fma_f32 v2, -v3, v14, 1.0\n" \
  "v_fma_f32 v14, v2, v14, v14\n" \
  "ds_write_b32 v1, v188 offset:6156\n" \
  "ds_write_b32 v1, v136 offset:7172\n" \
  "v_accvgpr_write_b32 a76, v17\n" \
  "ds_write_b32 v1, v135 offset:24580\n" \
  "ds_write_b32 v1, v165 offset:24588\n" \
  "v_accvgpr_write_b32 a88, v137\n" \
  "ds_write_b32 v1, v147 offset:11276\n" \
  "ds_write_b32 v1, v124 offset:12292\n" \
  "ds_write_b32 v1, v176 offset:12300\n" \
  "v_accvgpr_write_b32 a103, v97\n" \
  "ds_write_b32 v1, v73 offset:32780\n" \
  "ds_write_b32 v1, v134 offset:30724\n" \
  "ds_write_b32 v1, v189 offset:30732\n" \
  "v_accvgpr_write_b32 a108, v154\n" \
  "ds_write_b32 v1, v96 offset:20480\n" \
  "ds_write_b32 v1, v145 offset:20484\n" \
  "ds_write_b32 v1, v85 offset:27660\n" \
  "v_accvgpr_write_b32 a123, v11\n" \
  "ds_write_b32 v1, v95 offset:20488\n" \
  "ds_write_b32 v1, v140 offset:20492\n" \
  "ds_write_b32 v1, v22 offset:21504\n" \
  "v_accvgpr_write_b32 a124, v15\n" \
  "ds_write_b32 v1, v155 offset:37896\n" \
  "ds_write_b32 v1, v141 offset:39944\n" \
  "v_accvgpr_write_b32 a0, v206\n" \
  "ds_write_b32 v1, v106 offset:37900\n" \
  "v_accvgpr_write_b32 a126, v114\n" \
  "v_accvgpr_write_b32 a7, v13\n" \
  "ds_write_b32 v1, v127 offset:39948\n" \
  "v_accvgpr_write_b32 a8, v208\n" \
  "v_accvgpr_write_b32 a1, v122\n" \
  "v_accvgpr_write_b32 a9, v123\n" \
  "v_accvgpr_write_b32 a128, v158\n" \
  "v_accvgpr_write_b32 a27, v23\n" \
  "v_accvgpr_write_b32 a28, v5\n" \
  "v_accvgpr_write_b32 a29, v128\n" \
  "v_accvgpr_write_b32 a30, v146\n" \
  "v_accvgpr_write_b32 a31, v207\n" \
  "v_accvgpr_write_b32 a129, v84\n" \
  "v_accvgpr_write_b32 a32, v125\n" \
  "v_accvgpr_write_b32 a33, v10\n" \
  "v_mov_b32 v254, v26\n" \
  "v_accvgpr_write_b32 a39, v92\n" \
  "v_accvgpr_write_b32 a34, v129\n" \
  "v_accvgpr_write_b32 a35, v177\n" \
  "v_accvgpr_write_b32 a130, v126\n" \
  "v_accvgpr_write_b32 a40, v16\n" \
  "v_accvgpr_write_b32 a38, v107\n" \
  "v_mov_b32 v255, v90\n" \
  "v_accvgpr_write_b32 a41, v138\n" \
  "v_accvgpr_write_b32 a42, v91\n" \
  "v_accvgpr_write_b32 a131, v94\n" \
  "v_accvgpr_write_b32 a43, v72\n" \
  "v_accvgpr_write_b32 a44, v102\n" \
  "v_accvgpr_write_b32 a45, v144\n" \
  "v_accvgpr_write_b32 a46, v12\n" \
  "v_accvgpr_write_b32 a132, v4\n" \
  "v_accvgpr_write_b32 a47, v139\n" \
  "v_accvgpr_write_b32 a48, v120\n" \
  "v_accvgpr_write_b32 a49, v159\n" \
  "v_accvgpr_write_b32 a133, v164\n" \
  "v_accvgpr_write_b32 a50, v7\n" \
  "v_accvgpr_write_b32 a51, v93\n" \
  "v_accvgpr_write_b32 a134, v6\n" \
  "v_accvgpr_write_b32 a52, v121\n" \
  "v_accvgpr_write_b32 a135, v27\n" \
  "v_accvgpr_write_b32 a136, v14\n" \
  "v_mov_b32 v245, v0\n" \
  "global_load_dword v88, v245, s[42:43] nt\n" \
  "v_add_u32 v245, s10, v245\n" \
  "global_load_dword v89, v245, s[42:43] nt\n" \
  "v_add_u32 v245, s10, v245\n" \
  "global_load_dword v90, v245, s[42:43] nt\n" \
  "v_add_u32 v245, s10, v245\n" \
  "global_load_dword v92, v245, s[42:43] nt\n" \
  "v_add_u32 v245, s10, v245\n" \
  "global_load_dword v93, v245, s[42:43] nt\n" \
  "v_add_u32 v245, s10, v245\n" \
  "global_load_dword v91, v245, s[42:43] nt\n" \
  "v_add_u32 v245, s10, v245\n" \
  "global_load_dword v94, v245, s[42:43] nt\n" \
  "v_add_u32 v245, s10, v245\n" \
  "global_load_dword v95, v245, s[42:43] nt\n" \
  "v_add_u32 v245, s10, v245\n" \
  "global_load_dword v96, v245, s[42:43] nt\n" \
  "v_add_u32 v245, s10, v245\n" \
  "global_load_dword v98, v245, s[42:43] nt\n" \
  "v_add_u32 v245, s10, v245\n" \
  "global_load_dword v99, v245, s[42:43] nt\n" \
  "v_add_u32 v245, s10, v245\n" \
  "global_load_dword v97, v245, s[42:43] nt\n" \
  "v_add_u32 v245, s10, v245\n" \
  "global_load_dword v100, v245, s[42:43] nt\n" \
  "v_add_u32 v245, s10, v245\n" \
  "global_load_dword v101, v245, s[42:43] nt\n" \
  "v_add_u32 v245, s10, v245\n" \
  "global_load_dword v102, v245, s[42:43] nt\n" \
  "v_add_u32 v245, s10, v245\n" \
  "global_load_dword v104, v245, s[42:43] nt\n" \
  "v_add_u32 v245, s10, v245\n" \
  "global_load_dword v105, v245, s[42:43] nt\n" \
  "v_add_u32 v245, s10, v245\n" \
  "global_load_dword v103, v245, s[42:43] nt\n" \
  "v_add_u32 v245, s10, v245\n" \
  "global_load_dword v106, v245, s[42:43] nt\n" \
  "v_add_u32 v245, s10, v245\n" \
  "global_load_dword v107, v245, s[42:43] nt\n" \
  "v_add_u32 v245, s10, v245\n" \
  "global_load_dword v108, v245, s[42:43] nt\n" \
  "v_add_u32 v245, s10, v245\n" \
  "global_load_dword v110, v245, s[42:43] nt\n" \
  "v_add_u32 v245, s10, v245\n" \
  "global_load_dword v111, v245, s[42:43] nt\n" \
  "v_add_u32 v245, s10, v245\n" \
  "global_load_dword v109, v245, s[42:43] nt\n" \
  "v_add_u32 v245, s10, v245\n" \
  "global_load_dword v112, v245, s[42:43] nt\n" \
  "v_add_u32 v245, s10, v245\n" \
  "global_load_dword v113, v245, s[42:43] nt\n" \
  "v_add_u32 v245, s10, v245\n" \
  "global_load_dword v114, v245, s[42:43] nt\n" \
  "v_add_u32 v245, s10, v245\n" \
  "global_load_dword v116, v245, s[42:43] nt\n" \
  "v_add_u32 v245, s10, v245\n" \
  "global_load_dword v117, v245, s[42:43] nt\n" \
  "v_add_u32 v245, s10, v245\n" \
  "global_load_dword v115, v245, s[42:43] nt\n" \
  "v_add_u32 v245, s10, v245\n" \
  "global_load_dword v118, v245, s[42:43] nt\n" \
  "v_add_u32 v245, s10, v245\n" \
  "global_load_dword v119, v245, s[42:43] nt\n" \
  "v_add_u32 v245, s10, v245\n" \
  "global_load_dword v120, v245, s[42:43] nt\n" \
  "v_add_u32 v245, s10, v245\n" \
  "global_load_dword v122, v245, s[42:43] nt\n" \
  "v_add_u32 v245, s10, v245\n" \
  "global_load_dword v123, v245, s[42:43] nt\n" \
  "v_add_u32 v245, s10, v245\n" \
  "global_load_dword v121, v245, s[42:43] nt\n" \
  "v_add_u32 v245, s10, v245\n" \
  "global_load_dword v124, v245, s[42:43] nt\n" \
  "v_add_u32 v245, s10, v245\n" \
  "global_load_dword v125, v245, s[42:43] nt\n" \
  "v_add_u32 v245, s10, v245\n" \
  "global_load_dword v126, v245, s[42:43] nt\n" \
  "v_add_u32 v245, s10, v245\n" \
  "global_load_dword v127, v245, s[42:43] nt\n" \
  "v_add_u32 v245, s10, v245\n" \
  "global_load_dword v128, v245, s[42:43] nt\n" \
  "v_add_u32 v245, s10, v245\n" \
// ... 80 lines not shown
  "global_load_dword v170, v245, s[42:43] nt\n" \
  "v_add_u32 v245, s10, v245\n" \
  "global_load_dword v171, v245, s[42:43] nt\n" \
  "v_add_u32 v245, s10, v245\n" \
  "global_load_dword v172, v245, s[42:43] nt\n" \
  "v_add_u32 v245, s10, v245\n" \
  "global_load_dword v174, v245, s[42:43] nt\n" \
  "v_add_u32 v245, s10, v245\n" \
  "global_load_dword v175, v245, s[42:43] nt\n" \
  "v_add_u32 v245, s10, v245\n" \
  "global_load_dword v176, v245, s[42:43] nt\n" \
  "v_add_u32 v245, s10, v245\n" \
  "global_load_dword v178, v245, s[42:43] nt\n" \
  "v_add_u32 v245, s10, v245\n" \
  "global_load_dword v179, v245, s[42:43] nt\n" \
  "v_add_u32 v245, s10, v245\n" \
  "global_load_dword v177, v245, s[42:43] nt\n" \
  "v_add_u32 v245, s10, v245\n" \
  "global_load_dword v180, v245, s[42:43] nt\n" \
  "v_add_u32 v245, s10, v245\n" \
  "global_load_dword v181, v245, s[42:43] nt\n" \
  "v_add_u32 v245, s10, v245\n" \
  "global_load_dword v182, v245, s[42:43] nt\n" \
  "v_add_u32 v245, s10, v245\n" \
  "global_load_dword v184, v245, s[42:43] nt\n" \
  "v_add_u32 v245, s10, v245\n" \
  "global_load_dword v185, v245, s[42:43] nt\n" \
  "v_add_u32 v245, s10, v245\n" \
  "global_load_dword v183, v245, s[42:43] nt\n" \
  "v_add_u32 v245, s10, v245\n" \
  "global_load_dword v186, v245, s[42:43] nt\n" \
  "v_add_u32 v245, s10, v245\n" \
  "global_load_dword v187, v245, s[42:43] nt\n" \
  "v_add_u32 v245, s10, v245\n" \
  "global_load_dword v188, v245, s[42:43] nt\n" \
  "v_add_u32 v245, s10, v245\n" \
  "global_load_dword v190, v245, s[42:43] nt\n" \
  "v_add_u32 v245, s10, v245\n" \
  "global_load_dword v191, v245, s[42:43] nt\n" \
  "v_add_u32 v245, s10, v245\n" \
  "global_load_dword v189, v245, s[42:43] nt\n" \
  "v_add_u32 v245, s10, v245\n" \
  "global_load_dword v192, v245, s[42:43] nt\n" \
  "v_add_u32 v245, s10, v245\n" \
  "global_load_dword v193, v245, s[42:43] nt\n" \
  "v_add_u32 v245, s10, v245\n" \
  "global_load_dword v194, v245, s[42:43] nt\n" \
  "v_add_u32 v245, s10, v245\n" \
  "global_load_dword v196, v245, s[42:43] nt\n" \
  "v_add_u32 v245, s10, v245\n" \
  "global_load_dword v197, v245, s[42:43] nt\n" \
  "v_add_u32 v245, s10, v245\n" \
  "global_load_dword v195, v245, s[42:43] nt\n" \
  "v_add_u32 v245, s10, v245\n" \
  "global_load_dword v198, v245, s[42:43] nt\n" \
  "v_add_u32 v245, s10, v245\n" \
  "global_load_dword v199, v245, s[42:43] nt\n" \
  "v_add_u32 v245, s10, v245\n" \
  "global_load_dword v200, v245, s[42:43] nt\n" \
  "v_add_u32 v245, s10, v245\n" \
  "global_load_dword v202, v245, s[42:43] nt\n" \
  "v_add_u32 v245, s10, v245\n" \
  "global_load_dword v203, v245, s[42:43] nt\n" \
  "v_add_u32 v245, s10, v245\n" \
  "global_load_dword v201, v245, s[42:43] nt\n" \
  "v_add_u32 v245, s10, v245\n" \
  "global_load_dword v204, v245, s[42:43] nt\n" \
  "v_add_u32 v245, s10, v245\n" \
  "global_load_dword v205, v245, s[42:43] nt\n" \
  "v_add_u32 v245, s10, v245\n" \
  "global_load_dword v206, v245, s[42:43] nt\n" \
  "v_add_u32 v245, s10, v245\n" \
  "global_load_dword v208, v245, s[42:43] nt\n" \
  "v_add_u32 v245, s10, v245\n" \
  "global_load_dword v209, v245, s[42:43] nt\n" \
  "v_add_u32 v245, s10, v245\n" \
  "global_load_dword v207, v245, s[42:43] nt\n" \
  "v_add_u32 v245, s10, v245\n" \
  "global_load_dword v210, v245, s[42:43] nt\n" \
  "v_add_u32 v245, s10, v245\n" \
  "global_load_dword v211, v245, s[42:43] nt\n" \
  "v_add_u32 v245, s10, v245\n" \
  "global_load_dword v212, v245, s[42:43] nt\n" \
  "v_mov_b32 v133, 0\n" \
  "v_mov_b32 v173, 0\n" \
  "v_mov_b32 v213, 0\n" \
  "v_mov_b32 v47, 0\n" \
  "v_mov_b32 v87, 0\n" \
  "s_waitcnt vmcnt(0) lgkmcnt(0)\n" \
  "v_accvgpr_read_b32 v230, a137\n" \
  "v_accvgpr_read_b32 v231, a138\n" \
  "v_accvgpr_read_b32 v232, a139\n" \
  "v_accvgpr_read_b32 v233, a142\n" \
  "v_accvgpr_read_b32 v234, a140\n" \
  "v_accvgpr_read_b32 v235, a141\n" \
  "v_pk_fma_f32 v[2:3], s[24:25], v[88:89], v[230:231] op_sel:[0,0,0] op_sel_hi:[0,1,1] neg_lo:[0,0,1] neg_hi:[0,0,1]\n" \
  "v_accvgpr_read_b32 v236, a143\n" \
  "v_accvgpr_read_b32 v237, a144\n" \
  "v_pk_fma_f32 v[4:5], s[24:25], v[90:91], v[232:233] op_sel:[0,0,0] op_sel_hi:[0,1,1] neg_lo:[0,0,1] neg_hi:[0,0,1]\n" \
  "v_accvgpr_read_b32 v230, a145\n" \
  "v_accvgpr_read_b32 v231, a148\n" \
  "v_pk_fma_f32 v[6:7], s[24:25], v[92:93], v[234:235] op_sel:[0,0,0] op_sel_hi:[0,1,1] neg_lo:[0,0,1] neg_hi:[0,0,1]\n" \
  "v_accvgpr_read_b32 v232, a146\n" \
  "v_accvgpr_read_b32 v233, a147\n" \
  "v_pk_fma_f32 v[8:9], s[24:25], v[94:95], v[236:237] op_sel:[0,0,0] op_sel_hi:[0,1,1] neg_lo:[0,0,1] neg_hi:[0,0,1]\n" \
  "v_accvgpr_read_b32 v234, a149\n" \
  "v_accvgpr_read_b32 v235, a150\n" \
  "v_pk_fma_f32 v[10:11], s[24:25], v[96:97], v[230:231] op_sel:[0,0,0] op_sel_hi:[0,1,1] neg_lo:[0,0,1] neg_hi:[0,0,1]\n" \
  "v_accvgpr_read_b32 v236, a151\n" \
  "v_accvgpr_read_b32 v237, a154\n" \
  "v_pk_fma_f32 v[12:13], s[24:25], v[98:99], v[232:233] op_sel:[0,0,0] op_sel_hi:[0,1,1] neg_lo:[0,0,1] neg_hi:[0,0,1]\n" \
  "v_accvgpr_read_b32 v230, a152\n" \
  "v_accvgpr_read_b32 v231, a153\n" \
  "v_pk_fma_f32 v[14:15], s[24:25], v[100:101], v[234:235] op_sel:[0,0,0] op_sel_hi:[0,1,1] neg_lo:[0,0,1] neg_hi:[0,0,1]\n" \
  "v_accvgpr_read_b32 v232, a155\n" \
  "v_accvgpr_read_b32 v233, a156\n" \
  "v_pk_fma_f32 v[16:17], s[24:25], v[102:103], v[236:237] op_sel:[0,0,0] op_sel_hi:[0,1,1] neg_lo:[0,0,1] neg_hi:[0,0,1]\n" \
  "v_accvgpr_read_b32 v234, a157\n" \
  "v_pk_fma_f32 v[18:19], s[24:25], v[104:105], v[230:231] op_sel:[0,0,0] op_sel_hi:[0,1,1] neg_lo:[0,0,1] neg_hi:[0,0,1]\n" \
  "v_pk_fma_f32 v[20:21], s[24:25], v[106:107], v[232:233] op_sel:[0,0,0] op_sel_hi:[0,1,1] neg_lo:[0,0,1] neg_hi:[0,0,1]\n" \
  "v_accvgpr_read_b32 v236, a161\n" \
  "v_accvgpr_read_b32 v237, a162\n" \
  "v_pk_mul_f32 v[22:23], s[24:25], v[108:109] op_sel:[0,0] op_sel_hi:[0,1] neg_lo:[0,0] neg_hi:[0,0]\n" \
  "v_sub_f32 v22, v22, v234\n" \
  "v_accvgpr_read_b32 v230, a163\n" \
  "v_pk_mul_f32 v[24:25], s[24:25], v[110:111] op_sel:[0,0] op_sel_hi:[0,1] neg_lo:[0,0] neg_hi:[0,0]\n" \
  "v_pk_fma_f32 v[26:27], s[24:25], v[112:113], v[236:237] op_sel:[0,0,0] op_sel_hi:[0,1,1] neg_lo:[0,0,1] neg_hi:[0,0,1]\n" \
  "v_accvgpr_read_b32 v232, a167\n" \
  "v_accvgpr_read_b32 v233, a168\n" \
  "v_pk_mul_f32 v[28:29], s[24:25], v[114:115] op_sel:[0,0] op_sel_hi:[0,1] neg_lo:[0,0] neg_hi:[0,0]\n" \
  "v_sub_f32 v28, v28, v230\n" \
  "v_accvgpr_read_b32 v234, a169\n" \
  "v_pk_mul_f32 v[30:31], s[24:25], v[116:117] op_sel:[0,0] op_sel_hi:[0,1] neg_lo:[0,0] neg_hi:[0,0]\n" \
  "v_pk_fma_f32 v[32:33], s[24:25], v[118:119], v[232:233] op_sel:[0,0,0] op_sel_hi:[0,1,1] neg_lo:[0,0,1] neg_hi:[0,0,1]\n" \
  "v_pk_mul_f32 v[34:35], s[24:25], v[120:121] op_sel:[0,0] op_sel_hi:[0,1] neg_lo:[0,0] neg_hi:[0,0]\n" \
  "v_sub_f32 v34, v34, v234\n" \
  "v_pk_mul_f32 v[36:37], s[24:25], v[122:123] op_sel:[0,0] op_sel_hi:[0,1] neg_lo:[0,0] neg_hi:[0,0]\n" \
  "v_pk_mul_f32 v[38:39], s[24:25], v[124:125] op_sel:[0,0] op_sel_hi:[0,1] neg_lo:[0,0] neg_hi:[0,0]\n" \
  "v_pk_mul_f32 v[40:41], s[24:25], v[126:127] op_sel:[0,0] op_sel_hi:[0,1] neg_lo:[0,0] neg_hi:[0,0]\n" \
  "v_pk_mul_f32 v[42:43], s[24:25], v[128:129] op_sel:[0,0] op_sel_hi:[0,1] neg_lo:[0,0] neg_hi:[0,0]\n" \
  "v_pk_mul_f32 v[44:45], s[24:25], v[130:131] op_sel:[0,0] op_sel_hi:[0,1] neg_lo:[0,0] neg_hi:[0,0]\n" \
  "v_mul_f32 v46, s24, v132\n" \
  "v_pk_fma_f32 v[48:49], s[26:27], v[134:135], v[174:175] op_sel:[0,0,0] op_sel_hi:[0,1,1] neg_lo:[1,0,0] neg_hi:[1,0,0]\n" \
  "ds_read_b128 v[214:217], v1 offset:0\n" \
  "v_pk_fma_f32 v[50:51], s[26:27], v[136:137], v[176:177] op_sel:[0,0,0] op_sel_hi:[0,1,1] neg_lo:[1,0,0] neg_hi:[1,0,0]\n" \
  "v_pk_fma_f32 v[52:53], s[26:27], v[138:139], v[178:179] op_sel:[0,0,0] op_sel_hi:[0,1,1] neg_lo:[1,0,0] neg_hi:[1,0,0]\n" \
  "ds_read_b128 v[218:221], v1 offset:1024\n" \
  "v_pk_fma_f32 v[54:55], s[26:27], v[140:141], v[180:181] op_sel:[0,0,0] op_sel_hi:[0,1,1] neg_lo:[1,0,0] neg_hi:[1,0,0]\n" \
  "v_pk_fma_f32 v[56:57], s[26:27], v[142:143], v[182:183] op_sel:[0,0,0] op_sel_hi:[0,1,1] neg_lo:[1,0,0] neg_hi:[1,0,0]\n" \
  "ds_read_b128 v[222:225], v1 offset:2048\n" \
  "v_pk_fma_f32 v[58:59], s[26:27], v[144:145], v[184:185] op_sel:[0,0,0] op_sel_hi:[0,1,1] neg_lo:[1,0,0] neg_hi:[1,0,0]\n" \
  "v_pk_fma_f32 v[60:61], s[26:27], v[146:147], v[186:187] op_sel:[0,0,0] op_sel_hi:[0,1,1] neg_lo:[1,0,0] neg_hi:[1,0,0]\n" \
  "ds_read_b128 v[226:229], v1 offset:3072\n" \
  "v_pk_fma_f32 v[62:63], s[26:27], v[148:149], v[188:189] op_sel:[0,0,0] op_sel_hi:[0,1,1] neg_lo:[1,0,0] neg_hi:[1,0,0]\n" \
  "v_pk_fma_f32 v[64:65], s[26:27], v[150:151], v[190:191] op_sel:[0,0,0] op_sel_hi:[0,1,1] neg_lo:[1,0,0] neg_hi:[1,0,0]\n" \
  "ds_read_b128 v[246:249], v1 offset:4096\n" \
  "v_pk_fma_f32 v[66:67], s[26:27], v[152:153], v[192:193] op_sel:[0,0,0] op_sel_hi:[0,1,1] neg_lo:[1,0,0] neg_hi:[1,0,0]\n" \
  "v_pk_fma_f32 v[68:69], s[26:27], v[154:155], v[194:195] op_sel:[0,0,0] op_sel_hi:[0,1,1] neg_lo:[1,0,0] neg_hi:[1,0,0]\n" \
  "ds_read_b128 v[250:253], v1 offset:5120\n" \
  "v_pk_fma_f32 v[70:71], s[26:27], v[156:157], v[196:197] op_sel:[0,0,0] op_sel_hi:[0,1,1] neg_lo:[1,0,0] neg_hi:[1,0,0]\n" \
  "v_pk_fma_f32 v[72:73], s[26:27], v[158:159], v[198:199] op_sel:[0,0,0] op_sel_hi:[0,1,1] neg_lo:[1,0,0] neg_hi:[1,0,0]\n" \
  "v_pk_fma_f32 v[74:75], s[26:27], v[160:161], v[200:201] op_sel:[0,0,0] op_sel_hi:[0,1,1] neg_lo:[1,0,0] neg_hi:[1,0,0]\n" \
  "v_pk_fma_f32 v[76:77], s[26:27], v[162:163], v[202:203] op_sel:[0,0,0] op_sel_hi:[0,1,1] neg_lo:[1,0,0] neg_hi:[1,0,0]\n" \
  "v_pk_fma_f32 v[78:79], s[26:27], v[164:165], v[204:205] op_sel:[0,0,0] op_sel_hi:[0,1,1] neg_lo:[1,0,0] neg_hi:[1,0,0]\n" \
  "v_accvgpr_read_b32 v236, a227\n" \
  "v_pk_fma_f32 v[80:81], s[26:27], v[166:167], v[206:207] op_sel:[0,0,0] op_sel_hi:[0,1,1] neg_lo:[1,0,0] neg_hi:[1,0,0]\n" \
// ... 1914 lines not shown
  "v_pk_add_f32 v[2:3], v[88:89], v[2:3] op_sel:[0,0] op_sel_hi:[1,1] neg_lo:[0,1] neg_hi:[0,1]\n" \
  "v_pk_add_f32 v[4:5], v[90:91], v[4:5] op_sel:[0,0] op_sel_hi:[1,1] neg_lo:[0,1] neg_hi:[0,1]\n" \
  "v_pk_add_f32 v[6:7], v[92:93], v[6:7] op_sel:[0,0] op_sel_hi:[1,1] neg_lo:[0,1] neg_hi:[0,1]\n" \
  "v_pk_add_f32 v[8:9], v[94:95], v[8:9] op_sel:[0,0] op_sel_hi:[1,1] neg_lo:[0,1] neg_hi:[0,1]\n" \
  "v_pk_add_f32 v[10:11], v[96:97], v[10:11] op_sel:[0,0] op_sel_hi:[1,1] neg_lo:[0,1] neg_hi:[0,1]\n" \
  "v_pk_add_f32 v[12:13], v[98:99], v[12:13] op_sel:[0,0] op_sel_hi:[1,1] neg_lo:[0,1] neg_hi:[0,1]\n" \
  "v_pk_add_f32 v[14:15], v[100:101], v[14:15] op_sel:[0,0] op_sel_hi:[1,1] neg_lo:[0,1] neg_hi:[0,1]\n" \
  "v_pk_add_f32 v[16:17], v[102:103], v[16:17] op_sel:[0,0] op_sel_hi:[1,1] neg_lo:[0,1] neg_hi:[0,1]\n" \
  "v_pk_add_f32 v[18:19], v[104:105], v[18:19] op_sel:[0,0] op_sel_hi:[1,1] neg_lo:[0,1] neg_hi:[0,1]\n" \
  "v_pk_add_f32 v[20:21], v[106:107], v[20:21] op_sel:[0,0] op_sel_hi:[1,1] neg_lo:[0,1] neg_hi:[0,1]\n" \
  "v_pk_add_f32 v[22:23], v[108:109], v[22:23] op_sel:[0,0] op_sel_hi:[1,1] neg_lo:[0,1] neg_hi:[0,1]\n" \
  "v_pk_add_f32 v[24:25], v[110:111], v[24:25] op_sel:[0,0] op_sel_hi:[1,1] neg_lo:[0,1] neg_hi:[0,1]\n" \
  "v_pk_add_f32 v[26:27], v[112:113], v[26:27] op_sel:[0,0] op_sel_hi:[1,1] neg_lo:[0,1] neg_hi:[0,1]\n" \
  "v_pk_add_f32 v[28:29], v[114:115], v[28:29] op_sel:[0,0] op_sel_hi:[1,1] neg_lo:[0,1] neg_hi:[0,1]\n" \
  "v_pk_add_f32 v[30:31], v[116:117], v[30:31] op_sel:[0,0] op_sel_hi:[1,1] neg_lo:[0,1] neg_hi:[0,1]\n" \
  "v_pk_add_f32 v[32:33], v[118:119], v[32:33] op_sel:[0,0] op_sel_hi:[1,1] neg_lo:[0,1] neg_hi:[0,1]\n" \
  "v_pk_add_f32 v[34:35], v[120:121], v[34:35] op_sel:[0,0] op_sel_hi:[1,1] neg_lo:[0,1] neg_hi:[0,1]\n" \
  "v_pk_add_f32 v[36:37], v[122:123], v[36:37] op_sel:[0,0] op_sel_hi:[1,1] neg_lo:[0,1] neg_hi:[0,1]\n" \
  "v_pk_add_f32 v[38:39], v[124:125], v[38:39] op_sel:[0,0] op_sel_hi:[1,1] neg_lo:[0,1] neg_hi:[0,1]\n" \
  "v_pk_add_f32 v[40:41], v[126:127], v[40:41] op_sel:[0,0] op_sel_hi:[1,1] neg_lo:[0,1] neg_hi:[0,1]\n" \
  "v_pk_add_f32 v[42:43], v[128:129], v[42:43] op_sel:[0,0] op_sel_hi:[1,1] neg_lo:[0,1] neg_hi:[0,1]\n" \
  "v_pk_add_f32 v[44:45], v[130:131], v[44:45] op_sel:[0,0] op_sel_hi:[1,1] neg_lo:[0,1] neg_hi:[0,1]\n" \
  "v_pk_mul_f32 v[2:3], s[4:5], v[2:3] op_sel:[0,0] op_sel_hi:[0,1] neg_lo:[0,0] neg_hi:[0,0]\n" \
  "v_pk_mul_f32 v[4:5], s[4:5], v[4:5] op_sel:[0,0] op_sel_hi:[0,1] neg_lo:[0,0] neg_hi:[0,0]\n" \
  "v_pk_mul_f32 v[6:7], s[4:5], v[6:7] op_sel:[0,0] op_sel_hi:[0,1] neg_lo:[0,0] neg_hi:[0,0]\n" \
  "v_pk_mul_f32 v[8:9], s[4:5], v[8:9] op_sel:[0,0] op_sel_hi:[0,1] neg_lo:[0,0] neg_hi:[0,0]\n" \
  "v_pk_mul_f32 v[10:11], s[4:5], v[10:11] op_sel:[0,0] op_sel_hi:[0,1] neg_lo:[0,0] neg_hi:[0,0]\n" \
  "v_pk_mul_f32 v[12:13], s[4:5], v[12:13] op_sel:[0,0] op_sel_hi:[0,1] neg_lo:[0,0] neg_hi:[0,0]\n" \
  "v_pk_mul_f32 v[14:15], s[4:5], v[14:15] op_sel:[0,0] op_sel_hi:[0,1] neg_lo:[0,0] neg_hi:[0,0]\n" \
  "v_pk_mul_f32 v[16:17], s[4:5], v[16:17] op_sel:[0,0] op_sel_hi:[0,1] neg_lo:[0,0] neg_hi:[0,0]\n" \
  "v_pk_mul_f32 v[18:19], s[4:5], v[18:19] op_sel:[0,0] op_sel_hi:[0,1] neg_lo:[0,0] neg_hi:[0,0]\n" \
  "v_pk_mul_f32 v[20:21], s[4:5], v[20:21] op_sel:[0,0] op_sel_hi:[0,1] neg_lo:[0,0] neg_hi:[0,0]\n" \
  "v_pk_mul_f32 v[22:23], s[4:5], v[22:23] op_sel:[0,0] op_sel_hi:[0,1] neg_lo:[0,0] neg_hi:[0,0]\n" \
  "v_pk_mul_f32 v[24:25], s[4:5], v[24:25] op_sel:[0,0] op_sel_hi:[0,1] neg_lo:[0,0] neg_hi:[0,0]\n" \
  "v_pk_mul_f32 v[26:27], s[4:5], v[26:27] op_sel:[0,0] op_sel_hi:[0,1] neg_lo:[0,0] neg_hi:[0,0]\n" \
  "v_pk_mul_f32 v[28:29], s[4:5], v[28:29] op_sel:[0,0] op_sel_hi:[0,1] neg_lo:[0,0] neg_hi:[0,0]\n" \
  "v_pk_mul_f32 v[30:31], s[4:5], v[30:31] op_sel:[0,0] op_sel_hi:[0,1] neg_lo:[0,0] neg_hi:[0,0]\n" \
  "v_pk_mul_f32 v[32:33], s[4:5], v[32:33] op_sel:[0,0] op_sel_hi:[0,1] neg_lo:[0,0] neg_hi:[0,0]\n" \
  "v_pk_mul_f32 v[34:35], s[4:5], v[34:35] op_sel:[0,0] op_sel_hi:[0,1] neg_lo:[0,0] neg_hi:[0,0]\n" \
  "v_pk_mul_f32 v[36:37], s[4:5], v[36:37] op_sel:[0,0] op_sel_hi:[0,1] neg_lo:[0,0] neg_hi:[0,0]\n" \
  "v_pk_mul_f32 v[38:39], s[4:5], v[38:39] op_sel:[0,0] op_sel_hi:[0,1] neg_lo:[0,0] neg_hi:[0,0]\n" \
  "v_pk_mul_f32 v[40:41], s[4:5], v[40:41] op_sel:[0,0] op_sel_hi:[0,1] neg_lo:[0,0] neg_hi:[0,0]\n" \
  "v_pk_mul_f32 v[42:43], s[4:5], v[42:43] op_sel:[0,0] op_sel_hi:[0,1] neg_lo:[0,0] neg_hi:[0,0]\n" \
  "v_pk_mul_f32 v[44:45], s[4:5], v[44:45] op_sel:[0,0] op_sel_hi:[0,1] neg_lo:[0,0] neg_hi:[0,0]\n" \
  "v_sub_f32 v46, v132, v46\n" \
  "v_mul_f32 v46, s4, v46\n" \
  "v_pk_add_f32 v[48:49], v[134:135], v[48:49] op_sel:[0,0] op_sel_hi:[1,1] neg_lo:[0,1] neg_hi:[0,1]\n" \
  "v_pk_add_f32 v[50:51], v[136:137], v[50:51] op_sel:[0,0] op_sel_hi:[1,1] neg_lo:[0,1] neg_hi:[0,1]\n" \
  "v_pk_add_f32 v[52:53], v[138:139], v[52:53] op_sel:[0,0] op_sel_hi:[1,1] neg_lo:[0,1] neg_hi:[0,1]\n" \
  "v_pk_add_f32 v[54:55], v[140:141], v[54:55] op_sel:[0,0] op_sel_hi:[1,1] neg_lo:[0,1] neg_hi:[0,1]\n" \
  "v_pk_add_f32 v[56:57], v[142:143], v[56:57] op_sel:[0,0] op_sel_hi:[1,1] neg_lo:[0,1] neg_hi:[0,1]\n" \
  "v_pk_add_f32 v[58:59], v[144:145], v[58:59] op_sel:[0,0] op_sel_hi:[1,1] neg_lo:[0,1] neg_hi:[0,1]\n" \
  "v_pk_add_f32 v[60:61], v[146:147], v[60:61] op_sel:[0,0] op_sel_hi:[1,1] neg_lo:[0,1] neg_hi:[0,1]\n" \
  "v_pk_add_f32 v[62:63], v[148:149], v[62:63] op_sel:[0,0] op_sel_hi:[1,1] neg_lo:[0,1] neg_hi:[0,1]\n" \
  "v_pk_add_f32 v[64:65], v[150:151], v[64:65] op_sel:[0,0] op_sel_hi:[1,1] neg_lo:[0,1] neg_hi:[0,1]\n" \
  "v_pk_add_f32 v[66:67], v[152:153], v[66:67] op_sel:[0,0] op_sel_hi:[1,1] neg_lo:[0,1] neg_hi:[0,1]\n" \
  "v_pk_add_f32 v[68:69], v[154:155], v[68:69] op_sel:[0,0] op_sel_hi:[1,1] neg_lo:[0,1] neg_hi:[0,1]\n" \
  "v_pk_add_f32 v[70:71], v[156:157], v[70:71] op_sel:[0,0] op_sel_hi:[1,1] neg_lo:[0,1] neg_hi:[0,1]\n" \
  "v_pk_add_f32 v[72:73], v[158:159], v[72:73] op_sel:[0,0] op_sel_hi:[1,1] neg_lo:[0,1] neg_hi:[0,1]\n" \
  "v_pk_add_f32 v[74:75], v[160:161], v[74:75] op_sel:[0,0] op_sel_hi:[1,1] neg_lo:[0,1] neg_hi:[0,1]\n" \
  "v_pk_add_f32 v[76:77], v[162:163], v[76:77] op_sel:[0,0] op_sel_hi:[1,1] neg_lo:[0,1] neg_hi:[0,1]\n" \
  "v_pk_add_f32 v[78:79], v[164:165], v[78:79] op_sel:[0,0] op_sel_hi:[1,1] neg_lo:[0,1] neg_hi:[0,1]\n" \
  "v_pk_add_f32 v[80:81], v[166:167], v[80:81] op_sel:[0,0] op_sel_hi:[1,1] neg_lo:[0,1] neg_hi:[0,1]\n" \
  "v_pk_add_f32 v[82:83], v[168:169], v[82:83] op_sel:[0,0] op_sel_hi:[1,1] neg_lo:[0,1] neg_hi:[0,1]\n" \
  "v_pk_mul_f32 v[48:49], s[4:5], v[48:49] op_sel:[0,0] op_sel_hi:[0,1] neg_lo:[0,0] neg_hi:[0,0]\n" \
  "v_pk_mul_f32 v[50:51], s[4:5], v[50:51] op_sel:[0,0] op_sel_hi:[0,1] neg_lo:[0,0] neg_hi:[0,0]\n" \
  "v_pk_mul_f32 v[52:53], s[4:5], v[52:53] op_sel:[0,0] op_sel_hi:[0,1] neg_lo:[0,0] neg_hi:[0,0]\n" \
  "v_pk_mul_f32 v[54:55], s[4:5], v[54:55] op_sel:[0,0] op_sel_hi:[0,1] neg_lo:[0,0] neg_hi:[0,0]\n" \
  "v_pk_mul_f32 v[56:57], s[4:5], v[56:57] op_sel:[0,0] op_sel_hi:[0,1] neg_lo:[0,0] neg_hi:[0,0]\n" \
  "v_pk_mul_f32 v[58:59], s[4:5], v[58:59] op_sel:[0,0] op_sel_hi:[0,1] neg_lo:[0,0] neg_hi:[0,0]\n" \
  "v_pk_mul_f32 v[60:61], s[4:5], v[60:61] op_sel:[0,0] op_sel_hi:[0,1] neg_lo:[0,0] neg_hi:[0,0]\n" \
  "v_pk_mul_f32 v[62:63], s[4:5], v[62:63] op_sel:[0,0] op_sel_hi:[0,1] neg_lo:[0,0] neg_hi:[0,0]\n" \
  "v_pk_mul_f32 v[64:65], s[4:5], v[64:65] op_sel:[0,0] op_sel_hi:[0,1] neg_lo:[0,0] neg_hi:[0,0]\n" \
  "v_pk_mul_f32 v[66:67], s[4:5], v[66:67] op_sel:[0,0] op_sel_hi:[0,1] neg_lo:[0,0] neg_hi:[0,0]\n" \
  "v_pk_mul_f32 v[68:69], s[4:5], v[68:69] op_sel:[0,0] op_sel_hi:[0,1] neg_lo:[0,0] neg_hi:[0,0]\n" \
  "v_pk_mul_f32 v[70:71], s[4:5], v[70:71] op_sel:[0,0] op_sel_hi:[0,1] neg_lo:[0,0] neg_hi:[0,0]\n" \
  "v_pk_mul_f32 v[72:73], s[4:5], v[72:73] op_sel:[0,0] op_sel_hi:[0,1] neg_lo:[0,0] neg_hi:[0,0]\n" \
  "v_pk_mul_f32 v[74:75], s[4:5], v[74:75] op_sel:[0,0] op_sel_hi:[0,1] neg_lo:[0,0] neg_hi:[0,0]\n" \
  "v_pk_mul_f32 v[76:77], s[4:5], v[76:77] op_sel:[0,0] op_sel_hi:[0,1] neg_lo:[0,0] neg_hi:[0,0]\n" \
  "v_pk_mul_f32 v[78:79], s[4:5], v[78:79] op_sel:[0,0] op_sel_hi:[0,1] neg_lo:[0,0] neg_hi:[0,0]\n" \
  "v_pk_mul_f32 v[80:81], s[4:5], v[80:81] op_sel:[0,0] op_sel_hi:[0,1] neg_lo:[0,0] neg_hi:[0,0]\n" \
  "v_pk_mul_f32 v[82:83], s[4:5], v[82:83] op_sel:[0,0] op_sel_hi:[0,1] neg_lo:[0,0] neg_hi:[0,0]\n" \
  "30:\n" \
  "s_mul_i32 s4, s10, 9\n" \
  "v_add_u32 v174, s4, v0\n" \
  "global_load_dword v186, v174, s[46:47] nt\n" \
  "v_add_u32 v174, s10, v174\n" \
  "global_load_dword v187, v174, s[46:47] nt\n" \
  "v_add_u32 v174, s10, v174\n" \
  "global_load_dword v185, v174, s[46:47] nt\n" \
  "v_add_u32 v174, s10, v174\n" \
  "global_load_dword v188, v174, s[46:47] nt\n" \
  "v_add_u32 v174, s10, v174\n" \
  "global_load_dword v189, v174, s[46:47] nt\n" \
  "v_add_u32 v174, s10, v174\n" \
  "global_load_dword v190, v174, s[46:47] nt\n" \
  "v_add_u32 v174, s10, v174\n" \
  "global_load_dword v192, v174, s[46:47] nt\n" \
  "v_add_u32 v174, s10, v174\n" \
  "global_load_dword v193, v174, s[46:47] nt\n" \
  "v_add_u32 v174, s10, v174\n" \
  "global_load_dword v191, v174, s[46:47] nt\n" \
  "v_add_u32 v174, s10, v174\n" \
  "global_load_dword v194, v174, s[46:47] nt\n" \
  "v_add_u32 v174, s10, v174\n" \
  "global_load_dword v195, v174, s[46:47] nt\n" \
  "v_add_u32 v174, s10, v174\n" \
  "global_load_dword v196, v174, s[46:47] nt\n" \
  "v_add_u32 v174, s10, v174\n" \
  "global_load_dword v198, v174, s[46:47] nt\n" \
  "v_add_u32 v174, s10, v174\n" \
  "global_load_dword v199, v174, s[46:47] nt\n" \
  "v_add_u32 v174, s10, v174\n" \
  "global_load_dword v197, v174, s[46:47] nt\n" \
  "v_add_u32 v174, s10, v174\n" \
  "global_load_dword v200, v174, s[46:47] nt\n" \
  "v_add_u32 v174, s10, v174\n" \
  "global_load_dword v201, v174, s[46:47] nt\n" \
  "v_add_u32 v174, s10, v174\n" \
  "global_load_dword v202, v174, s[46:47] nt\n" \
  "v_add_u32 v174, s10, v174\n" \
  "global_load_dword v204, v174, s[46:47] nt\n" \
  "v_add_u32 v174, s10, v174\n" \
  "global_load_dword v205, v174, s[46:47] nt\n" \
  "v_add_u32 v174, s10, v174\n" \
  "global_load_dword v203, v174, s[46:47] nt\n" \
  "v_add_u32 v174, s10, v174\n" \
  "global_load_dword v206, v174, s[46:47] nt\n" \
  "v_add_u32 v174, s10, v174\n" \
  "global_load_dword v207, v174, s[46:47] nt\n" \
  "v_add_u32 v174, s10, v174\n" \
  "global_load_dword v214, v174, s[46:47] nt\n" \
  "v_add_u32 v174, s10, v174\n" \
  "global_load_dword v216, v174, s[46:47] nt\n" \
  "v_add_u32 v174, s10, v174\n" \
  "global_load_dword v217, v174, s[46:47] nt\n" \
  "v_add_u32 v174, s10, v174\n" \
  "global_load_dword v215, v174, s[46:47] nt\n" \
  "v_add_u32 v174, s10, v174\n" \
  "global_load_dword v218, v174, s[46:47] nt\n" \
  "v_add_u32 v174, s10, v174\n" \
  "global_load_dword v219, v174, s[46:47] nt\n" \
  "v_add_u32 v174, s10, v174\n" \
  "global_load_dword v220, v174, s[46:47] nt\n" \
  "v_add_u32 v174, s10, v174\n" \
  "global_load_dword v221, v174, s[46:47] nt\n" \
  "v_add_u32 v174, s10, v174\n" \
  "global_load_dword v222, v174, s[46:47] nt\n" \
  "v_add_u32 v174, s10, v174\n" \
  "global_load_dword v223, v174, s[46:47] nt\n" \
  "v_add_u32 v174, s10, v174\n" \
  "global_load_dword v224, v174, s[46:47] nt\n" \
  "v_add_u32 v174, s10, v174\n" \
  "global_load_dword v225, v174, s[46:47] nt\n" \
  "v_add_u32 v174, s10, v174\n" \
  "global_load_dword v226, v174, s[46:47] nt\n" \
  "v_accvgpr_read_b32 v176, a246\n" \
  "v_accvgpr_read_b32 v177, a247\n" \
  "v_accvgpr_read_b32 v178, a248\n" \
  "v_accvgpr_read_b32 v180, a249\n" \
  "v_accvgpr_read_b32 v181, a250\n" \
  "v_accvgpr_read_b32 v179, a251\n" \
  "v_accvgpr_read_b32 v182, a252\n" \
  "v_accvgpr_read_b32 v183, a253\n" \
  "v_accvgpr_read_b32 v184, a254\n" \
  "v_accvgpr_read_b32 v175, a255\n" \
  "s_mul_i32 s4, s10, 0x7b\n" \
  "v_add_u32 v174, s4, v0\n" \
  "global_load_dword v208, v174, s[42:43] nt\n" \
  "v_mov_b32 v227, 0\n" \
  "v_mov_b32 v174, v0\n" \
  "global_store_dword v174, v88, s[42:43] nt\n" \
  "v_add_u32 v174, s10, v174\n" \
  "global_store_dword v174, v89, s[42:43] nt\n" \
  "v_add_u32 v174, s10, v174\n" \
  "global_store_dword v174, v90, s[42:43] nt\n" \
  "v_add_u32 v174, s10, v174\n" \
  "global_store_dword v174, v92, s[42:43] nt\n" \
  "v_add_u32 v174, s10, v174\n" \
  "global_store_dword v174, v93, s[42:43] nt\n" \
  "v_add_u32 v174, s10, v174\n" \
  "global_store_dword v174, v91, s[42:43] nt\n" \
  "v_add_u32 v174, s10, v174\n" \
  "global_store_dword v174, v94, s[42:43] nt\n" \
  "v_add_u32 v174, s10, v174\n" \
  "global_store_dword v174, v95, s[42:43] nt\n" \
  "v_add_u32 v174, s10, v174\n" \
  "global_store_dword v174, v96, s[42:43] nt\n" \
  "v_add_u32 v174, s10, v174\n" \
  "global_store_dword v174, v98, s[42:43] nt\n" \
  "v_add_u32 v174, s10, v174\n" \
  "global_store_dword v174, v99, s[42:43] nt\n" \
  "v_add_u32 v174, s10, v174\n" \
  "global_store_dword v174, v97, s[42:43] nt\n" \
  "v_add_u32 v174, s10, v174\n" \
  "global_store_dword v174, v100, s[42:43] nt\n" \
  "v_add_u32 v174, s10, v174\n" \
  "global_store_dword v174, v101, s[42:43] nt\n" \
  "v_add_u32 v174, s10, v174\n" \
  "global_store_dword v174, v102, s[42:43] nt\n" \
  "v_add_u32 v174, s10, v174\n" \
  "global_store_dword v174, v104, s[42:43] nt\n" \
  "v_add_u32 v174, s10, v174\n" \
  "global_store_dword v174, v105, s[42:43] nt\n" \
  "v_add_u32 v174, s10, v174\n" \
  "global_store_dword v174, v103, s[42:43] nt\n" \
  "v_add_u32 v174, s10, v174\n" \
  "global_store_dword v174, v106, s[42:43] nt\n" \
  "v_add_u32 v174, s10, v174\n" \
  "global_store_dword v174, v107, s[42:43] nt\n" \
  "v_add_u32 v174, s10, v174\n" \
  "global_store_dword v174, v108, s[42:43] nt\n" \
  "v_add_u32 v174, s10, v174\n" \
  "global_store_dword v174, v110, s[42:43] nt\n" \
  "v_add_u32 v174, s10, v174\n" \
  "global_store_dword v174, v111, s[42:43] nt\n" \
  "v_add_u32 v174, s10, v174\n" \
  "global_store_dword v174, v109, s[42:43] nt\n" \
  "v_add_u32 v174, s10, v174\n" \
  "global_store_dword v174, v112, s[42:43] nt\n" \
  "v_add_u32 v174, s10, v174\n" \
  "global_store_dword v174, v113, s[42:43] nt\n" \
  "v_add_u32 v174, s10, v174\n" \
  "global_store_dword v174, v114, s[42:43] nt\n" \
  "v_add_u32 v174, s10, v174\n" \
  "global_store_dword v174, v116, s[42:43] nt\n" \
  "v_add_u32 v174, s10, v174\n" \
  "global_store_dword v174, v117, s[42:43] nt\n" \
  "v_add_u32 v174, s10, v174\n" \
  "global_store_dword v174, v115, s[42:43] nt\n" \
  "v_add_u32 v174, s10, v174\n" \
  "global_store_dword v174, v118, s[42:43] nt\n" \
  "v_add_u32 v174, s10, v174\n" \
  "global_store_dword v174, v119, s[42:43] nt\n" \
  "v_add_u32 v174, s10, v174\n" \
  "global_store_dword v174, v120, s[42:43] nt\n" \
  "v_add_u32 v174, s10, v174\n" \
  "global_store_dword v174, v122, s[42:43] nt\n" \
  "v_add_u32 v174, s10, v174\n" \
  "global_store_dword v174, v123, s[42:43] nt\n" \
  "v_add_u32 v174, s10, v174\n" \
  "global_store_dword v174, v121, s[42:43] nt\n" \
  "v_add_u32 v174, s10, v174\n" \
  "global_store_dword v174, v124, s[42:43] nt\n" \
  "v_add_u32 v174, s10, v174\n" \
  "global_store_dword v174, v125, s[42:43] nt\n" \
  "v_add_u32 v174, s10, v174\n" \
  "global_store_dword v174, v126, s[42:43] nt\n" \
  "v_add_u32 v174, s10, v174\n" \
  "global_store_dword v174, v127, s[42:43] nt\n" \
  "v_add_u32 v174, s10, v174\n" \
  "global_store_dword v174, v128, s[42:43] nt\n" \
  "v_add_u32 v174, s10, v174\n" \
// ... 117 lines not shown
  "global_store_dword v174, v229, s[42:43] nt\n" \
  "v_add_u32 v174, s10, v174\n" \
  "v_accvgpr_read_b32 v230, a193\n" \
  "global_store_dword v174, v230, s[42:43] nt\n" \
  "v_add_u32 v174, s10, v174\n" \
  "v_accvgpr_read_b32 v209, a194\n" \
  "global_store_dword v174, v209, s[42:43] nt\n" \
  "v_add_u32 v174, s10, v174\n" \
  "v_accvgpr_read_b32 v228, a195\n" \
  "global_store_dword v174, v228, s[42:43] nt\n" \
  "v_add_u32 v174, s10, v174\n" \
  "v_accvgpr_read_b32 v229, a196\n" \
  "global_store_dword v174, v229, s[42:43] nt\n" \
  "v_add_u32 v174, s10, v174\n" \
  "v_accvgpr_read_b32 v230, a197\n" \
  "global_store_dword v174, v230, s[42:43] nt\n" \
  "v_add_u32 v174, s10, v174\n" \
  "v_accvgpr_read_b32 v209, a198\n" \
  "global_store_dword v174, v209, s[42:43] nt\n" \
  "v_add_u32 v174, s10, v174\n" \
  "v_accvgpr_read_b32 v228, a199\n" \
  "global_store_dword v174, v228, s[42:43] nt\n" \
  "v_add_u32 v174, s10, v174\n" \
  "v_accvgpr_read_b32 v229, a200\n" \
  "global_store_dword v174, v229, s[42:43] nt\n" \
  "v_add_u32 v174, s10, v174\n" \
  "v_accvgpr_read_b32 v230, a201\n" \
  "global_store_dword v174, v230, s[42:43] nt\n" \
  "v_add_u32 v174, s10, v174\n" \
  "v_accvgpr_read_b32 v209, a202\n" \
  "global_store_dword v174, v209, s[42:43] nt\n" \
  "v_add_u32 v174, s10, v174\n" \
  "v_accvgpr_read_b32 v228, a203\n" \
  "global_store_dword v174, v228, s[42:43] nt\n" \
  "v_add_u32 v174, s10, v174\n" \
  "v_accvgpr_read_b32 v229, a204\n" \
  "global_store_dword v174, v229, s[42:43] nt\n" \
  "v_add_u32 v174, s10, v174\n" \
  "v_accvgpr_read_b32 v230, a205\n" \
  "global_store_dword v174, v230, s[42:43] nt\n" \
  "v_add_u32 v174, s10, v174\n" \
  "v_accvgpr_read_b32 v209, a206\n" \
  "global_store_dword v174, v209, s[42:43] nt\n" \
  "v_add_u32 v174, s10, v174\n" \
  "v_accvgpr_read_b32 v228, a207\n" \
  "global_store_dword v174, v228, s[42:43] nt\n" \
  "v_add_u32 v174, s10, v174\n" \
  "v_accvgpr_read_b32 v229, a208\n" \
  "global_store_dword v174, v229, s[42:43] nt\n" \
  "v_add_u32 v174, s10, v174\n" \
  "v_accvgpr_read_b32 v230, a209\n" \
  "global_store_dword v174, v230, s[42:43] nt\n" \
  "v_add_u32 v174, s10, v174\n" \
  "v_accvgpr_read_b32 v209, a210\n" \
  "global_store_dword v174, v209, s[42:43] nt\n" \
  "v_add_u32 v174, s10, v174\n" \
  "v_accvgpr_read_b32 v228, a211\n" \
  "global_store_dword v174, v228, s[42:43] nt\n" \
  "v_add_u32 v174, s10, v174\n" \
  "v_accvgpr_read_b32 v229, a212\n" \
  "global_store_dword v174, v229, s[42:43] nt\n" \
  "v_add_u32 v174, s10, v174\n" \
  "v_accvgpr_read_b32 v230, a213\n" \
  "global_store_dword v174, v230, s[42:43] nt\n" \
  "v_add_u32 v174, s10, v174\n" \
  "v_accvgpr_read_b32 v209, a214\n" \
  "global_store_dword v174, v209, s[42:43] nt\n" \
  "v_add_u32 v174, s10, v174\n" \
  "v_accvgpr_read_b32 v228, a215\n" \
  "global_store_dword v174, v228, s[42:43] nt\n" \
  "v_add_u32 v174, s10, v174\n" \
  "v_accvgpr_read_b32 v229, a216\n" \
  "global_store_dword v174, v229, s[42:43] nt\n" \
  "v_add_u32 v174, s10, v174\n" \
  "v_accvgpr_read_b32 v230, a217\n" \
  "global_store_dword v174, v230, s[42:43] nt\n" \
  "v_add_u32 v174, s10, v174\n" \
  "global_store_dword v174, v210, s[42:43] nt\n" \
  "v_add_u32 v174, s10, v174\n" \
  "global_store_dword v174, v211, s[42:43] nt\n" \
  "v_add_u32 v174, s10, v174\n" \
  "global_store_dword v174, v212, s[42:43] nt\n" \
  "v_add_u32 v174, s10, v174\n" \
  "s_waitcnt vmcnt(0)\n" \
  "v_pk_mul_f32 v[2:3], v[176:177], v[2:3] op_sel:[0,0] op_sel_hi:[1,1] neg_lo:[0,0] neg_hi:[0,0]\n" \
  "v_pk_mul_f32 v[88:89], v[176:177], v[88:89] op_sel:[0,0] op_sel_hi:[1,1] neg_lo:[0,0] neg_hi:[0,0]\n" \
  "v_pk_mul_f32 v[4:5], v[178:179], v[4:5] op_sel:[0,0] op_sel_hi:[1,1] neg_lo:[0,0] neg_hi:[0,0]\n" \
  "v_pk_mul_f32 v[90:91], v[178:179], v[90:91] op_sel:[0,0] op_sel_hi:[1,1] neg_lo:[0,0] neg_hi:[0,0]\n" \
  "v_pk_mul_f32 v[6:7], v[180:181], v[6:7] op_sel:[0,0] op_sel_hi:[1,1] neg_lo:[0,0] neg_hi:[0,0]\n" \
  "v_pk_mul_f32 v[92:93], v[180:181], v[92:93] op_sel:[0,0] op_sel_hi:[1,1] neg_lo:[0,0] neg_hi:[0,0]\n" \
  "v_pk_mul_f32 v[8:9], v[182:183], v[8:9] op_sel:[0,0] op_sel_hi:[1,1] neg_lo:[0,0] neg_hi:[0,0]\n" \
  "v_pk_mul_f32 v[94:95], v[182:183], v[94:95] op_sel:[0,0] op_sel_hi:[1,1] neg_lo:[0,0] neg_hi:[0,0]\n" \
  "v_pk_mul_f32 v[10:11], v[184:185], v[10:11] op_sel:[0,0] op_sel_hi:[1,1] neg_lo:[0,0] neg_hi:[0,0]\n" \
  "v_pk_mul_f32 v[96:97], v[184:185], v[96:97] op_sel:[0,0] op_sel_hi:[1,1] neg_lo:[0,0] neg_hi:[0,0]\n" \
  "v_pk_mul_f32 v[12:13], v[186:187], v[12:13] op_sel:[0,0] op_sel_hi:[1,1] neg_lo:[0,0] neg_hi:[0,0]\n" \
  "v_pk_mul_f32 v[98:99], v[186:187], v[98:99] op_sel:[0,0] op_sel_hi:[1,1] neg_lo:[0,0] neg_hi:[0,0]\n" \
  "v_pk_mul_f32 v[14:15], v[188:189], v[14:15] op_sel:[0,0] op_sel_hi:[1,1] neg_lo:[0,0] neg_hi:[0,0]\n" \
  "v_pk_mul_f32 v[100:101], v[188:189], v[100:101] op_sel:[0,0] op_sel_hi:[1,1] neg_lo:[0,0] neg_hi:[0,0]\n" \
  "v_pk_mul_f32 v[16:17], v[190:191], v[16:17] op_sel:[0,0] op_sel_hi:[1,1] neg_lo:[0,0] neg_hi:[0,0]\n" \
  "v_pk_mul_f32 v[102:103], v[190:191], v[102:103] op_sel:[0,0] op_sel_hi:[1,1] neg_lo:[0,0] neg_hi:[0,0]\n" \
  "v_pk_mul_f32 v[18:19], v[192:193], v[18:19] op_sel:[0,0] op_sel_hi:[1,1] neg_lo:[0,0] neg_hi:[0,0]\n" \
  "v_pk_mul_f32 v[104:105], v[192:193], v[104:105] op_sel:[0,0] op_sel_hi:[1,1] neg_lo:[0,0] neg_hi:[0,0]\n" \
  "v_pk_mul_f32 v[20:21], v[194:195], v[20:21] op_sel:[0,0] op_sel_hi:[1,1] neg_lo:[0,0] neg_hi:[0,0]\n" \
  "v_pk_mul_f32 v[106:107], v[194:195], v[106:107] op_sel:[0,0] op_sel_hi:[1,1] neg_lo:[0,0] neg_hi:[0,0]\n" \
  "v_pk_mul_f32 v[22:23], v[196:197], v[22:23] op_sel:[0,0] op_sel_hi:[1,1] neg_lo:[0,0] neg_hi:[0,0]\n" \
  "v_pk_mul_f32 v[108:109], v[196:197], v[108:109] op_sel:[0,0] op_sel_hi:[1,1] neg_lo:[0,0] neg_hi:[0,0]\n" \
  "v_pk_mul_f32 v[24:25], v[198:199], v[24:25] op_sel:[0,0] op_sel_hi:[1,1] neg_lo:[0,0] neg_hi:[0,0]\n" \
  "v_pk_mul_f32 v[110:111], v[198:199], v[110:111] op_sel:[0,0] op_sel_hi:[1,1] neg_lo:[0,0] neg_hi:[0,0]\n" \
  "v_pk_mul_f32 v[26:27], v[200:201], v[26:27] op_sel:[0,0] op_sel_hi:[1,1] neg_lo:[0,0] neg_hi:[0,0]\n" \
  "v_pk_mul_f32 v[112:113], v[200:201], v[112:113] op_sel:[0,0] op_sel_hi:[1,1] neg_lo:[0,0] neg_hi:[0,0]\n" \
  "v_pk_mul_f32 v[28:29], v[202:203], v[28:29] op_sel:[0,0] op_sel_hi:[1,1] neg_lo:[0,0] neg_hi:[0,0]\n" \
  "v_pk_mul_f32 v[114:115], v[202:203], v[114:115] op_sel:[0,0] op_sel_hi:[1,1] neg_lo:[0,0] neg_hi:[0,0]\n" \
  "v_pk_mul_f32 v[30:31], v[204:205], v[30:31] op_sel:[0,0] op_sel_hi:[1,1] neg_lo:[0,0] neg_hi:[0,0]\n" \
  "v_pk_mul_f32 v[116:117], v[204:205], v[116:117] op_sel:[0,0] op_sel_hi:[1,1] neg_lo:[0,0] neg_hi:[0,0]\n" \
  "v_pk_mul_f32 v[32:33], v[206:207], v[32:33] op_sel:[0,0] op_sel_hi:[1,1] neg_lo:[0,0] neg_hi:[0,0]\n" \
  "v_pk_mul_f32 v[118:119], v[206:207], v[118:119] op_sel:[0,0] op_sel_hi:[1,1] neg_lo:[0,0] neg_hi:[0,0]\n" \
  "v_pk_mul_f32 v[34:35], v[214:215], v[34:35] op_sel:[0,0] op_sel_hi:[1,1] neg_lo:[0,0] neg_hi:[0,0]\n" \
  "v_pk_mul_f32 v[120:121], v[214:215], v[120:121] op_sel:[0,0] op_sel_hi:[1,1] neg_lo:[0,0] neg_hi:[0,0]\n" \
  "v_pk_mul_f32 v[36:37], v[216:217], v[36:37] op_sel:[0,0] op_sel_hi:[1,1] neg_lo:[0,0] neg_hi:[0,0]\n" \
  "v_pk_mul_f32 v[122:123], v[216:217], v[122:123] op_sel:[0,0] op_sel_hi:[1,1] neg_lo:[0,0] neg_hi:[0,0]\n" \
  "v_pk_mul_f32 v[38:39], v[218:219], v[38:39] op_sel:[0,0] op_sel_hi:[1,1] neg_lo:[0,0] neg_hi:[0,0]\n" \
  "v_pk_mul_f32 v[124:125], v[218:219], v[124:125] op_sel:[0,0] op_sel_hi:[1,1] neg_lo:[0,0] neg_hi:[0,0]\n" \
  "v_pk_mul_f32 v[40:41], v[220:221], v[40:41] op_sel:[0,0] op_sel_hi:[1,1] neg_lo:[0,0] neg_hi:[0,0]\n" \
  "v_pk_mul_f32 v[126:127], v[220:221], v[126:127] op_sel:[0,0] op_sel_hi:[1,1] neg_lo:[0,0] neg_hi:[0,0]\n" \
  "v_pk_mul_f32 v[42:43], v[222:223], v[42:43] op_sel:[0,0] op_sel_hi:[1,1] neg_lo:[0,0] neg_hi:[0,0]\n" \
  "v_pk_mul_f32 v[128:129], v[222:223], v[128:129] op_sel:[0,0] op_sel_hi:[1,1] neg_lo:[0,0] neg_hi:[0,0]\n" \
  "v_pk_mul_f32 v[44:45], v[224:225], v[44:45] op_sel:[0,0] op_sel_hi:[1,1] neg_lo:[0,0] neg_hi:[0,0]\n" \
  "v_pk_mul_f32 v[130:131], v[224:225], v[130:131] op_sel:[0,0] op_sel_hi:[1,1] neg_lo:[0,0] neg_hi:[0,0]\n" \
  "v_pk_mul_f32 v[46:47], v[226:227], v[46:47] op_sel:[0,0] op_sel_hi:[1,1] neg_lo:[0,0] neg_hi:[0,0]\n" \
  "v_pk_mul_f32 v[132:133], v[226:227], v[132:133] op_sel:[0,0] op_sel_hi:[1,1] neg_lo:[0,0] neg_hi:[0,0]\n" \
  "s_mul_i32 s4, s10, 45\n" \
  "v_add_u32 v174, s4, v0\n" \
  "global_load_dword v176, v174, s[46:47] nt\n" \
  "v_add_u32 v174, s10, v174\n" \
  "global_load_dword v177, v174, s[46:47] nt\n" \
  "v_add_u32 v174, s10, v174\n" \
  "global_load_dword v178, v174, s[46:47] nt\n" \
  "v_add_u32 v174, s10, v174\n" \
  "global_load_dword v180, v174, s[46:47] nt\n" \
  "v_add_u32 v174, s10, v174\n" \
  "global_load_dword v181, v174, s[46:47] nt\n" \
  "v_add_u32 v174, s10, v174\n" \
  "global_load_dword v179, v174, s[46:47] nt\n" \
  "v_add_u32 v174, s10, v174\n" \
  "global_load_dword v182, v174, s[46:47] nt\n" \
  "v_add_u32 v174, s10, v174\n" \
  "global_load_dword v183, v174, s[46:47] nt\n" \
  "v_add_u32 v174, s10, v174\n" \
  "global_load_dword v184, v174, s[46:47] nt\n" \
  "v_add_u32 v174, s10, v174\n" \
  "global_load_dword v186, v174, s[46:47] nt\n" \
  "v_add_u32 v174, s10, v174\n" \
  "global_load_dword v187, v174, s[46:47] nt\n" \
  "v_add_u32 v174, s10, v174\n" \
  "global_load_dword v185, v174, s[46:47] nt\n" \
  "v_add_u32 v174, s10, v174\n" \
  "global_load_dword v188, v174, s[46:47] nt\n" \
  "v_add_u32 v174, s10, v174\n" \
  "global_load_dword v189, v174, s[46:47] nt\n" \
  "v_add_u32 v174, s10, v174\n" \
  "global_load_dword v190, v174, s[46:47] nt\n" \
  "v_add_u32 v174, s10, v174\n" \
  "global_load_dword v192, v174, s[46:47] nt\n" \
  "v_add_u32 v174, s10, v174\n" \
  "global_load_dword v193, v174, s[46:47] nt\n" \
  "v_add_u32 v174, s10, v174\n" \
// ... 1637 lines not shown
  "v_cmp_lt_f32_e64 s[30:31], v255, v211\n" \
  "v_cmp_lt_f32_e64 vcc, v255, v187\n" \
  "s_or_b64 s[30:31], s[30:31], vcc\n" \
  "v_cmp_u_f32 vcc, v191, v191\n" \
  "s_or_b64 s[30:31], s[30:31], vcc\n" \
  "v_cndmask_b32_e64 v248, v248, -7, s[30:31]\n" \
  "v_cmp_eq_i32_e64 s[62:63], -7, v248\n" \
  "v_cmp_eq_i32_e64 s[30:31], -3, v248\n" \
  "s_or_b64 s[62:63], s[62:63], s[30:31]\n" \
  "v_cmp_eq_i32_e64 s[30:31], 3, v248\n" \
  "s_or_b64 s[62:63], s[62:63], s[30:31]\n" \
  "v_cmp_eq_i32_e64 s[30:31], -4, v248\n" \
  "s_or_b64 s[62:63], s[62:63], s[30:31]\n" \
  "v_cmp_eq_i32_e64 s[30:31], 4, v248\n" \
  "s_or_b64 s[62:63], s[62:63], s[30:31]\n" \
  "v_mov_b32 v175, 0x4eff8000\n" \
  "s_mov_b64 vcc, s[62:63]\n" \
  "v_cndmask_b32 v124, v124, v175, vcc\n" \
  "v_cndmask_b32 v125, v125, v175, vcc\n" \
  "v_cndmask_b32 v126, v126, v175, vcc\n" \
  "v_cndmask_b32 v106, v106, v175, vcc\n" \
  "v_cndmask_b32 v107, v107, v175, vcc\n" \
  "v_cndmask_b32 v108, v108, v175, vcc\n" \
  "v_cndmask_b32 v110, v110, v175, vcc\n" \
  "v_cndmask_b32 v111, v111, v175, vcc\n" \
  "v_cndmask_b32 v109, v109, v175, vcc\n" \
  "v_add_f32 v175, v208, v124\n" \
  "v_mov_b32 v186, v125\n" \
  "v_mov_b32 v210, v126\n" \
  "v_mul_f32 v212, v224, v110\n" \
  "v_mul_f32 v249, v225, v111\n" \
  "v_add_f32 v212, v212, v249\n" \
  "v_mul_f32 v249, v226, v109\n" \
  "v_add_f32 v212, v212, v249\n" \
  "v_mul_f32 v213, v227, v110\n" \
  "v_mul_f32 v249, v228, v111\n" \
  "v_add_f32 v213, v213, v249\n" \
  "v_mul_f32 v249, v229, v109\n" \
  "v_add_f32 v213, v213, v249\n" \
  "v_sub_f32 v176, v106, v233\n" \
  "v_sub_f32 v177, v107, v234\n" \
  "v_sub_f32 v178, v108, v235\n" \
  "v_sub_f32 v179, -v213, v236\n" \
  "v_sub_f32 v180, v212, v237\n" \
  "v_sub_f32 v181, 0, v238\n" \
  "v_mul_f32 v176, s94, v176\n" \
  "v_mul_f32 v177, s94, v177\n" \
  "v_mul_f32 v178, s94, v178\n" \
  "v_mul_f32 v179, s94, v179\n" \
  "v_mul_f32 v180, s94, v180\n" \
  "v_mul_f32 v181, s94, v181\n" \
  "v_mov_b32 v174, v0\n" \
  "global_store_dword v174, v175, s[48:49] nt\n" \
  "v_add_u32 v174, s10, v174\n" \
  "global_store_dword v174, v186, s[48:49] nt\n" \
  "v_add_u32 v174, s10, v174\n" \
  "global_store_dword v174, v210, s[48:49] nt\n" \
  "v_add_u32 v174, s10, v174\n" \
  "global_store_dword v174, v176, s[48:49] nt\n" \
  "v_add_u32 v174, s10, v174\n" \
  "global_store_dword v174, v177, s[48:49] nt\n" \
  "v_add_u32 v174, s10, v174\n" \
  "global_store_dword v174, v178, s[48:49] nt\n" \
  "v_add_u32 v174, s10, v174\n" \
  "global_store_dword v174, v179, s[48:49] nt\n" \
  "v_add_u32 v174, s10, v174\n" \
  "global_store_dword v174, v180, s[48:49] nt\n" \
  "v_add_u32 v174, s10, v174\n" \
  "global_store_dword v174, v181, s[48:49] nt\n" \
  "s_cmp_eq_u64 s[52:53], 0\n" \
  "s_cbranch_scc1 36f\n" \
  "global_store_dword v0, v248, s[52:53]\n" \
  "36:\n" \
  "s_cmp_eq_u64 s[54:55], 0\n" \
  "s_cbranch_scc1 37f\n" \
  "v_mov_b32 v174, v0\n" \
  "global_store_dword v174, v211, s[54:55]\n" \
  "v_add_u32 v174, s10, v174\n" \
  "global_store_dword v174, v187, s[54:55]\n" \
  "37:\n" \
  "s_and_saveexec_b64 s[32:33], s[62:63]\n" \
  "s_cbranch_execz 38f\n" \
  "v_mov_b32 v212, 0\n" \
  "v_mov_b32 v174, v0\n" \
  "global_store_dword v174, v212, s[42:43]\n" \
  "v_add_u32 v174, s10, v174\n" \
  "global_store_dword v174, v212, s[42:43]\n" \
  "v_add_u32 v174, s10, v174\n" \
  "global_store_dword v174, v212, s[42:43]\n" \
  "v_add_u32 v174, s10, v174\n" \
  "global_store_dword v174, v212, s[42:43]\n" \
  "v_add_u32 v174, s10, v174\n" \
  "global_store_dword v174, v212, s[42:43]\n" \
  "v_add_u32 v174, s10, v174\n" \
  "global_store_dword v174, v212, s[42:43]\n" \
  "v_add_u32 v174, s10, v174\n" \
  "global_store_dword v174, v212, s[42:43]\n" \
  "v_add_u32 v174, s10, v174\n" \
  "global_store_dword v174, v212, s[42:43]\n" \
  "v_add_u32 v174, s10, v174\n" \
  "global_store_dword v174, v212, s[42:43]\n" \
  "v_add_u32 v174, s10, v174\n" \
  "global_store_dword v174, v212, s[42:43]\n" \
  "v_add_u32 v174, s10, v174\n" \
  "global_store_dword v174, v212, s[42:43]\n" \
  "v_add_u32 v174, s10, v174\n" \
  "global_store_dword v174, v212, s[42:43]\n" \
  "v_add_u32 v174, s10, v174\n" \
  "global_store_dword v174, v212, s[42:43]\n" \
  "v_add_u32 v174, s10, v174\n" \
  "global_store_dword v174, v212, s[42:43]\n" \
  "v_add_u32 v174, s10, v174\n" \
  "global_store_dword v174, v212, s[42:43]\n" \
  "v_add_u32 v174, s10, v174\n" \
  "global_store_dword v174, v212, s[42:43]\n" \
  "v_add_u32 v174, s10, v174\n" \
  "global_store_dword v174, v212, s[42:43]\n" \
  "v_add_u32 v174, s10, v174\n" \
  "global_store_dword v174, v212, s[42:43]\n" \
  "v_add_u32 v174, s10, v174\n" \
  "global_store_dword v174, v212, s[42:43]\n" \
  "v_add_u32 v174, s10, v174\n" \
  "global_store_dword v174, v212, s[42:43]\n" \
  "v_add_u32 v174, s10, v174\n" \
  "global_store_dword v174, v212, s[42:43]\n" \
  "v_add_u32 v174, s10, v174\n" \
  "global_store_dword v174, v212, s[42:43]\n" \
  "v_add_u32 v174, s10, v174\n" \
  "global_store_dword v174, v212, s[42:43]\n" \
  "v_add_u32 v174, s10, v174\n" \
  "global_store_dword v174, v212, s[42:43]\n" \
  "v_add_u32 v174, s10, v174\n" \
  "global_store_dword v174, v212, s[42:43]\n" \
  "v_add_u32 v174, s10, v174\n" \
  "global_store_dword v174, v212, s[42:43]\n" \
  "v_add_u32 v174, s10, v174\n" \
  "global_store_dword v174, v212, s[42:43]\n" \
  "v_add_u32 v174, s10, v174\n" \
  "global_store_dword v174, v212, s[42:43]\n" \
  "v_add_u32 v174, s10, v174\n" \
  "global_store_dword v174, v212, s[42:43]\n" \
  "v_add_u32 v174, s10, v174\n" \
  "global_store_dword v174, v212, s[42:43]\n" \
  "v_add_u32 v174, s10, v174\n" \
  "global_store_dword v174, v212, s[42:43]\n" \
  "v_add_u32 v174, s10, v174\n" \
  "global_store_dword v174, v212, s[42:43]\n" \
  "v_add_u32 v174, s10, v174\n" \
  "global_store_dword v174, v212, s[42:43]\n" \
  "v_add_u32 v174, s10, v174\n" \
  "global_store_dword v174, v212, s[42:43]\n" \
  "v_add_u32 v174, s10, v174\n" \
  "global_store_dword v174, v212, s[42:43]\n" \
  "v_add_u32 v174, s10, v174\n" \
  "global_store_dword v174, v212, s[42:43]\n" \
  "v_add_u32 v174, s10, v174\n" \
  "global_store_dword v174, v212, s[42:43]\n" \
  "v_add_u32 v174, s10, v174\n" \
  "global_store_dword v174, v212, s[42:43]\n" \
  "v_add_u32 v174, s10, v174\n" \
  "global_store_dword v174, v212, s[42:43]\n" \
  "v_add_u32 v174, s10, v174\n" \
  "global_store_dword v174, v212, s[42:43]\n" \
  "v_add_u32 v174, s10, v174\n" \
  "global_store_dword v174, v212, s[42:43]\n" \
  "v_add_u32 v174, s10, v174\n" \
// ... 1355 lines not shown
```

### robobee3d_amd/isasim.py

```python
import functools
import re
from fractions import Fraction

import numpy as np

f32, f64, u32, u64 = np.float32, np.float64, np.uint32, np.uint64
POISON = 0x7ff8dead
VCC = 106
LANE_LDS_VGPR = 1


class AddressFault(Exception):
    """A simulated global access outside every array handed to the interpreter (on the GPU: a memory access fault)."""


class Quad:

    def __init__(self, v=(), a=(), lds=(), dead_v=(), dead_a=(), dead_lds=()):
        self.v, self.a, self.lds = list(v), list(a), list(lds)
        self.dead_v, self.dead_a, self.dead_lds = list(dead_v), list(dead_a), list(dead_lds)


_REG = re.compile(r"([vas])(\d+)$|([vas])\[(\d+):(\d+)\]$")

# ... 521 lines not shown
    sel = t[-1]["op_sel"]
    halves = [mc.bits("%s%d" % (x[0], _decode(x)[1] + sel[q])) for q, x in enumerate(t[2:4])]
    mc.write(t[1], halves[0])
    mc.write(t[1], halves[1], 1)


def _cmp(kind):
    def f(mc, t):
        op = _CMP[t[0][len("v_cmp_"):].split("_")[0]]
        if kind == "f32":
            cond = op(mc.f(t[2]), mc.f(t[3]))
        elif kind == "f64":
            cond = op(mc.d(t[2]), mc.d(t[3]))
        else:
            cond = op(mc.bits(t[2]), mc.bits(t[3]))
        mc.wmask(t[1], np.asarray(cond, bool))
    return f


def _cndmask(mc, t):
    sel = mc.lanes_of(mc.s64(t[4] if len(t) > 4 else "vcc"))
    mc.write(t[1], np.where(sel, mc.bits(t[3]), mc.bits(t[2])).astype(u32))


def _ds(mc, t):
    m = t[0]
    n = {"b32": 1, "b64": 2, "b128": 4, "f32": 1}[m.rsplit("_", 1)[1]]
    read = m.startswith("ds_read")
    base, reg = (t[2], t[1]) if read else (t[1], t[2])
    k, lo = _decode(reg)[:2]
    for ln in mc.active():
        sl, w = mc.lds_word(base, t[3], ln)
        if read:
            mc.V[ln, lo:lo + n] = mc.lds[sl, w:w + n]
        elif m == "ds_min_f32":
            cur, val = mc.lds[sl, w:w + 1].view(f32)[0], mc.V[ln, lo:lo + 1].view(f32)[0]
            mc.lds[sl, w] = np.array(val if val < cur else cur, f32).view(u32)
        else:
            mc.lds[sl, w:w + n] = mc.V[ln, lo:lo + n]
    if mc.log is not None:
        sl, w = mc.lds_word(base, t[3], mc.active()[0])
        if read:
            for h in range(n):
                mc.src_word[("v", lo + h)], mc.src_phase[("v", lo + h)] = w + h, mc.phase
        else:
            mc.log["a" if m == "ds_min_f32" else "w"].update(range(w, w + n))


def _global(mc, t):
    m = t[0]
    n = {"dword": 1, "dwordx2": 2, "dwordx4": 4}[m.rsplit("_", 1)[1]]
    load = m.startswith("global_load")
    voff, reg = (t[2], t[1]) if load else (t[1], t[2])
    k, lo = _decode(reg)[:2]
    R = mc.V if k == "v" else mc.A
    for ln in mc.active():
        words, w0 = mc.gaddr(t[3], voff, _imm(t, 4), ln, n)
        if load:
            R[ln, lo:lo + n] = words[w0:w0 + n]
        else:
            words[w0:w0 + n] = R[ln, lo:lo + n]


def _readfirstlane(mc, t):
    act = mc.active()
    mc.S[_decode(t[1])[1]] = int(mc.bits(t[2])[act[0] if act else 0])


def _bitop(op):
    return lambda mc, t: mc.write(t[1], op(mc.bits(t[2]).astype(u64), mc.bits(t[3]).astype(u64)).astype(u32))


VECTOR = {
    "v_mov_b32": lambda mc, t: mc.write(t[1], mc.bits(t[2])),
    "v_mov_b32_dpp": lambda mc, t: mc.write(t[1], mc.bits(t[2], t[3])),
    "v_accvgpr_read_b32": lambda mc, t: mc.write(t[1], mc.bits(t[2])),
    "v_accvgpr_write_b32": lambda mc, t: mc.write(t[1], mc.bits(t[2])),
    "v_readfirstlane_b32": _readfirstlane,
    "v_pk_mov_b32": _pk_mov,
    "v_add_u32": _bitop(lambda a, b: (a + b) & u64(0xFFFFFFFF)),
    "v_and_b32": _bitop(lambda a, b: a & b),
    "v_or_b32": _bitop(lambda a, b: a | b),
    "v_lshrrev_b32": _bitop(lambda a, b: b >> (a & u64(31))),
    "v_mul_u32_u24": _bitop(lambda a, b: ((a & u64(0xFFFFFF)) * (b & u64(0xFFFFFF))) & u64(0xFFFFFFFF)),
    "v_bfe_u32": lambda mc, t: mc.write(t[1], (mc.bits(t[2]) >> u32(t[3] & 31)) & u32((1 << t[4]) - 1)),
    "v_cvt_f32_i32": lambda mc, t: mc.wf(t[1], mc.bits(t[2]).view(np.int32).astype(f32)),
    "v_fma_f32": _f32op(_fma32),
    "v_fmac_f32": _fmac(),
    "v_fmac_f32_dpp": _fmac(True),
    "v_fmaak_f32": lambda mc, t: mc.wf(t[1], _fma32(mc.f(t[2]), mc.f(t[3]), mc.f(t[4]))),
    "v_mul_f32": _f32op(lambda a, b: a * b),
    "v_mul_f32_dpp": _f32op(lambda a, b: a * b, True),
    "v_add_f32": _f32op(lambda a, b: a + b),
    "v_add_f32_dpp": _f32op(lambda a, b: a + b, True),
    "v_sub_f32": _f32op(lambda a, b: a - b),
    "v_subrev_f32": _f32op(lambda a, b: b - a),
    "v_max_f32": _f32op(_fmax),
    "v_max_f32_dpp": _f32op(_fmax, True),
    "v_min_f32": _f32op(_fmin),
    "v_max3_f32": _f32op(_nanless(np.fmax)),
    "v_min3_f32": _f32op(_nanless(np.fmin)),
    "v_med3_f32": _f32op(lambda a, b, c: np.sort(np.stack([a, b, c]), 0)[1]),
    "v_rcp_f32": _f32op(lambda a: f32(1.0) / a),
    "v_rsq_f32": _f32op(lambda a: (1.0 / np.sqrt(a.astype(f64))).astype(f32)),
    "v_sqrt_f32": _f32op(lambda a: np.sqrt(a.astype(f64)).astype(f32)),
    "v_pk_fma_f32": _pk("fma"),
    "v_pk_mul_f32": _pk("mul"),
    "v_pk_add_f32": _pk("add"),
    "v_cndmask_b32": _cndmask,
    "v_cndmask_b32_e64": _cndmask,
    "v_fma_f64": _f64op(_fma64),
    "v_mul_f64": _f64op(lambda a, b: a * b),
    "v_add_f64": _f64op(lambda a, b: a + b),
    "v_max_f64": _f64op(_fmax),
    "v_min_f64": _f64op(_fmin),
    "v_rcp_f64": _f64op(lambda a: 1.0 / a),
    "v_rsq_f64": _f64op(lambda a: 1.0 / np.sqrt(a)),
    "v_cmp_nlt_f64": _cmp("f64"),
    "v_cmp_eq_i32_e64": _cmp("int"),
    "v_cmp_ne_u32": _cmp("int"),
}
for _op in ("lt", "le", "gt", "ge", "eq", "nlt", "neq", "u"):
    VECTOR["v_cmp_%s_f32" % _op] = VECTOR["v_cmp_%s_f32_e64" % _op] = _cmp("f32")
OPS = dict(SALU, **VECTOR)
for _m in ("ds_read_b32", "ds_read_b64", "ds_read_b128", "ds_write_b32", "ds_write_b64", "ds_write_b128", "ds_min_f32",
           "global_load_dword", "global_load_dwordx2", "global_load_dwordx4", "global_store_dword", "global_store_dwordx2"):
    OPS[_m] = _ds if _m.startswith("ds_") else _global
```

Baseline: 547.7 million.

## Carry ADMM iterates between steps in a lane-interleaved shadow with dwordx4 transfers

Between consecutive MPC steps in one launch, the x/y/z warm-start iterates are now saved to and restored from a shadow region just below the workspace. It is laid out per lane as contiguous groups of four dwords, so each lane moves them with global_load/store_dwordx4 instead of many strided single-dword accesses to the ctrl array. The final step still writes ctrl in the original layout, and the bad-solve path zeroes the shadow. The cost is extra branches, a larger workspace offset bound, and a second copy of the state whose consistency with ctrl depends on the step index.

```diff
diff --git a/robobee3d_amd/asmstep.py b/robobee3d_amd/asmstep.py
--- a/robobee3d_amd/asmstep.py
+++ b/robobee3d_amd/asmstep.py
@@ -35,6 +35,7 @@
 S_C = {"minscal": 16, "maxscal": 17, "c45": 18, "eps10": 19, "eps": 38, "rho": 6, "rinv": 7, "rmin": 8,
        "rmininv": 9, "infty_ms": 100, "rhotol": 101}
 S_TMP = 4
+S_SHADOW = 98
 OFF = {}
 _o = 0
 for _n in PTRS:
@@ -61,6 +62,9 @@
 XV_N, XV_B = 2, 254
 NT_PTRS = ("state", "ctrl", "ref", "out", "stats")
 A_SPARE, N_SPARE_D = 246, 9
+SHADOW_LO, SHADOW_HI = V_X, V_Z + 40
+SHADOW_ROWS = (SHADOW_HI - SHADOW_LO + 3) // 4 * 4
+assert SHADOW_LO % 2 == 0 and (SHADOW_HI - SHADOW_LO) % 4 in (0, 2) and SHADOW_ROWS <= asmgen.WS_DS
 
 
 class Pool:
@@ -244,7 +248,7 @@
 
 
 class StepGen:
-    def __init__(self, N=3, perm=None, quad=False, exact_ruiz=False):
+    def __init__(self, N=3, perm=None, quad=False, exact_ruiz=False, wide_spill=True):
         self.st = Struct(N, perm)
         self.s = self.st.s
         self.e = Emit()
@@ -252,6 +256,9 @@
         self.lab = 20
         self.lab_spec = 500
         self.quad = quad
+        self.wide_iter = bool(wide_spill) and not quad
+        self.lab_wide = 600
+        self.spill_plan = dict(wide=0, adds=0, dwords=0, dword_adds=0)
         self.speculate = not quad and not exact_ruiz
         self.ruiz_span = self.restart_at = None
         self.nt = () if quad else ("nt",)
@@ -260,6 +267,10 @@
     def label(self):
         self.lab += 1
         return str(self.lab)
+
+    def label_wide(self):
+        self.lab_wide += 1
+        return str(self.lab_wide)
 
     def label_spec(self):
         self.lab_spec += 1
@@ -349,6 +360,47 @@
                 self.adv(voff)
         if own:
             self.pool.free(voff, kill=False)
+
+    def group_ptr(self, voff, first_group=0, plan=True):
+        e = self.e
+        e("v_lshlrev_b32", v(voff), 2, "v0")
+        if first_group:
+            e("s_mul_i32", sg(S_TMP), sg(S_INT["stride"]), 4 * first_group)
+            e("v_add_u32", v(voff), sg(S_TMP), v(voff))
+            self.spill_plan["adds"] += plan
+        e("s_lshl_b32", sg(S_TMP), sg(S_INT["stride"]), 2)
+
+    def adv_group(self, voff, plan=True):
+        self.e("v_add_u32", v(voff), sg(S_TMP), v(voff))
+        self.spill_plan["adds"] += plan
+
+    @staticmethod
+    def _tuple(kind, lo, n):
+        return "%s[%d:%d]" % (kind, lo, lo + n - 1)
+
+    def store_group(self, voff, lo, n, plan=True):
+        assert lo % 2 == 0
+        self.e("global_store_dwordx%d" % n, v(voff), self._tuple("v", lo, n), sp(S_SHADOW), *self.nt)
+        self.spill_plan["wide"] += plan
+
+    def load_group(self, voff, lo, n):
+        assert lo % 2 == 0
+        self.e("global_load_dwordx%d" % n, self._tuple("v", lo, n), v(voff), sp(S_SHADOW), *self.nt)
+        self.spill_plan["wide"] += 1
+
+    def shadow_groups(self):
+        return [(lo, min(4, SHADOW_HI - lo)) for lo in range(SHADOW_LO, SHADOW_HI, 4)]
+
+    def shadow_rw(self, voff, load, lo_of=None, plan=True, part=slice(None)):
+        groups = self.shadow_groups()[part]
+        self.group_ptr(voff, part.start or 0, plan)
+        for k, (lo, n) in enumerate(groups):
+            if load:
+                self.load_group(voff, lo, n)
+            else:
+                self.store_group(voff, lo if lo_of is None else lo_of, n, plan)
+            if k + 1 < len(groups):
+                self.adv_group(voff, plan)
 
     def prologue(self):
         e = self.e
@@ -376,6 +428,16 @@
                           ("infty_ms", float(f32(1e30) * f32(1e-4))), ("rhotol", 1e-4)):
             e("s_mov_b32", sg(S_C[name]), f32bits(val))
         e("s_waitcnt", "lgkmcnt(0)")
+        if self.wide_iter:
+            lab = self.label_wide()
+            lo, hi, ws = S_SHADOW, S_SHADOW + 1, S_PTR["ws"]
+            e("s_mul_i32", sg(lo), sg(S_INT["stride"]), SHADOW_ROWS)
+            e("s_mov_b32", sg(hi), sg(ws + 1))
+            e("s_cmp_gt_u32", sg(lo), sg(ws))
+            e("s_cbranch_scc0", lab + "f")
+            e("s_sub_i32", sg(hi), sg(hi), 1)
+            e("label", lab)
+            e("s_sub_i32", sg(lo), sg(ws), sg(lo))
         e("s_mov_b32", sg(S_STEP), 0)
 
     def phase_a(self):
@@ -1116,8 +1178,20 @@
         pool.reserve(V_Y, V_Z - V_Y)
         pool.reserve(V_Z, 40)
         voff = 245
+        if self.wide_iter:
+            lab_first, lab_join = self.label_wide(), self.label_wide()
+            e("s_cmp_eq_u32", sg(S_STEP), 0)
+            e("s_cbranch_scc1", lab_first + "f")
+            self.shadow_rw(voff, load=True)
+            e("s_waitcnt", "vmcnt(0)")
+            e("s_branch", lab_join + "f")
+            e("label", lab_first)
         self.load_rows("ctrl", 0, [V_X + st.xs[r] for r in range(nx)] + [V_Y + st.zs[r] for r in range(nc)] +
                        [V_Z + st.zs[r] for r in range(nc)], voff)
+        if self.wide_iter:
+            e("label", lab_join)
+            self.spill_plan["dwords"] += nx + 2 * nc
+            self.spill_plan["dword_adds"] += nx + 2 * nc - 1
         for pad in (V_X + nx, V_Y + nc, V_Z + nc, V_W + nx, V_WZ + nc):
             e("v_mov_b32", v(pad), 0)
         e("s_waitcnt", "vmcnt(0) lgkmcnt(0)")
@@ -1134,7 +1208,10 @@
         else:
             self._admm_rest(plan, zk)
         for i in range(st.neq):
-            pool.free(V_Z + st.zs[i], kill=True)
+            if self.wide_iter:
+                e("kill", v(V_Z + st.zs[i]))
+            else:
+                pool.free(V_Z + st.zs[i], kill=True)
         pool.free_range(246, 10)
 
 
@@ -1169,6 +1246,28 @@
             pk(e, "v_pk_mul_f32", V_WZ + p_, [PS(S_TMP), P2(V_WZ + p_)])
         e("label", lab6)
 
+    def branch_if_last_step(self, lab):
+        e = self.e
+        e("s_add_i32", sg(S_TMP), sg(S_STEP), 1)
+        e("s_cmp_lt_i32", sg(S_TMP), sg(S_INT["K"]))
+        e("s_cbranch_scc0", lab + "f")
+
+    def z_groups(self):
+        return next(k for k, (lo, n) in enumerate(self.shadow_groups()) if lo + n > V_Z)
+
+    def store_iterates_z(self):
+        e, pool, st = self.e, self.pool, self.st
+        voff = pool.get()
+        lab_last = self.label_wide()
+        self.branch_if_last_step(lab_last)
+        for r in range(st.neq):
+            e("v_accvgpr_read_b32", v(V_Z + st.zs[r]), "a%d" % (A_LO + r))
+        self.shadow_rw(voff, load=False, part=slice(self.z_groups(), None))
+        e("label", lab_last)
+        pool.free(voff, kill=False)
+        for i in range(st.neq):
+            pool.free(V_Z + st.zs[i], kill=False)
+
     def phase_c(self):
         e, pool, st, s = self.e, self.pool, self.st, self.s
         N, NYv = s.N, symbolic.NY
@@ -1180,6 +1279,8 @@
         ZR = lambda i: V_Z + st.zs[i]
         DXR = lambda j: V_W + st.xs[j]
         DYR = lambda i: V_WZ + st.zs[i]
+        if self.wide_iter:
+            self.store_iterates_z()
         voff = g_()
         def slot_blocks(n, chunk=16):
             n2 = n + n % 2
@@ -1202,23 +1303,34 @@
             self.load_rows("ws", asmgen.WS_C - asmgen.WS_DS, [cr], voff)
         self.load_rows("ctrl", nx + 2 * nc, [T0], voff)
         e("v_mov_b32", v(DS(nx)), 0)
-        zt = [g_() for _ in range(4)]
-        self.rows_ptr(voff, 0)
-        for r in range(nx):
-            e("global_store_dword", v(voff), v(XR(r)), sp(S_PTR["ctrl"]), *self.nt)
-            self.adv(voff)
-        for r in range(nc):
-            e("global_store_dword", v(voff), v(YR(r)), sp(S_PTR["ctrl"]), *self.nt)
-            self.adv(voff)
-        for r in range(nc):
-            if r < neq:
-                t_ = zt[r % 4]
-                e("v_accvgpr_read_b32", v(t_), "a%d" % (A_LO + r))
-                e("global_store_dword", v(voff), v(t_), sp(S_PTR["ctrl"]), *self.nt)
-            else:
-                e("global_store_dword", v(voff), v(ZR(r)), sp(S_PTR["ctrl"]), *self.nt)
-            self.adv(voff)
-        pool.free(*zt)
+        if True:
+            zt = [g_() for _ in range(4)]
+            if self.wide_iter:
+                lab_last, lab_done = self.label_wide(), self.label_wide()
+                self.branch_if_last_step(lab_last)
+                self.shadow_rw(voff, load=False, part=slice(0, self.z_groups()))
+                e("s_branch", lab_done + "f")
+                e("label", lab_last)
+                self.spill_plan["dwords"] += nx + 2 * nc
+                self.spill_plan["dword_adds"] += nx + 2 * nc
+            self.rows_ptr(voff, 0)
+            for r in range(nx):
+                e("global_store_dword", v(voff), v(XR(r)), sp(S_PTR["ctrl"]), *self.nt)
+                self.adv(voff)
+            for r in range(nc):
+                e("global_store_dword", v(voff), v(YR(r)), sp(S_PTR["ctrl"]), *self.nt)
+                self.adv(voff)
+            for r in range(nc):
+                if r < neq:
+                    t_ = zt[r % 4]
+                    e("v_accvgpr_read_b32", v(t_), "a%d" % (A_LO + r))
+                    e("global_store_dword", v(voff), v(t_), sp(S_PTR["ctrl"]), *self.nt)
+                else:
+                    e("global_store_dword", v(voff), v(ZR(r)), sp(S_PTR["ctrl"]), *self.nt)
+                self.adv(voff)
+            if self.wide_iter:
+                e("label", lab_done)
+            pool.free(*zt)
         e("s_waitcnt", "vmcnt(0)")
         for k in range(0, nx + 1, 2):
             pk(e, "v_pk_mul_f32", V_W + k, [P2(DS(k)), P2(V_W + k)])
@@ -1560,6 +1672,16 @@
         e("s_and_saveexec_b64", sp(S_M1), MBAD)
         e("s_cbranch_execz", lab_c + "f")
         e("v_mov_b32", v(a1), 0)
+        if self.wide_iter:
+            lab_last = self.label_wide()
+            self.branch_if_last_step(lab_last)
+            zq = pool.getn(4)
+            for k in range(4):
+                e("v_mov_b32", v(zq + k), 0)
+            self.shadow_rw(voff, load=False, lo_of=zq, plan=False)
+            pool.free_range(zq, 4, kill=False)
+            e("s_branch", lab_c + "f")
+            e("label", lab_last)
         self.rows_ptr(voff, 0)
         for r in range(nx + 2 * nc):
             e("global_store_dword", v(voff), v(a1), sp(S_PTR["ctrl"]))
@@ -2048,9 +2170,9 @@
 PSEUDO = ("kill", "quad_begin", "quad_end")
 
 
-def write(path=None, N=3, perm=None, quad=False):
+def write(path=None, N=3, perm=None, quad=False, wide_spill=True):
     path = path or os.path.join(HERE, "csrc", "umpc_step_asm_quad.h" if quad else "umpc_step_asm.h")
-    g = StepGen(N, perm, quad=quad)
+    g = StepGen(N, perm, quad=quad, wide_spill=wide_spill)
     ins = [t for t in g.program() if t[0] not in PSEUDO]
     if quad:
         head = ["// GENERATED by robobee3d_amd/asmstep.py (quad=True) + asmquad.py -- do not edit.", asmgen.switch_banner(),
@@ -2082,7 +2204,9 @@
                 "struct StepArgs {", "  StepParams p;", "  StepHist h;", "  StepImp i;", "};",
                 "static_assert(offsetof(StepArgs, h) == %d && sizeof(StepHist) == %d, \"StepHist layout\");" % (HIST_OFF, HIST_BYTES),
                 "static_assert(offsetof(StepArgs, i) == %d && sizeof(StepImp) == %d && offsetof(StepImp, impstep) == 8, \"StepImp layout\");" % (IMP_OFF, IMP_BYTES),
-                "constexpr int STEP_LDS_BYTES_PER_LANE = %d;" % (NLDS * 4), "}  // namespace umpcasm",
+                "constexpr int STEP_LDS_BYTES_PER_LANE = %d;" % (NLDS * 4),
+                "// workspace rows of the iterate shadow (x, y, z between two steps of one launch): the rows BELOW the one `ws` points at",
+                "constexpr int STEP_SHADOW_ROWS = %d;" % SHADOW_ROWS, "}  // namespace umpcasm",
                 "// inputs: v0 = 4 * robot, v1 = lane LDS address, s[4:5] = &StepParams (kernarg)"]
     asmtext.write_if_changed(path, asmtext.asm_block(
         head, "UMPC_STEP_ASM%s(voff, ldsaddr, params)" % ("_QUAD" if quad else ""), ins,
@@ -2122,6 +2246,8 @@
     allints.setdefault("refstep", 0)
     for n in HIST_INTS:
         allints.setdefault(n, 0)
+    shadow_base = base_of["ws"] - SHADOW_ROWS * stride
+    shadow = np.full(SHADOW_ROWS * stride // 4, np.nan, np.float32)
     for n in INTS + TAIL_INTS + HIST_INTS:
         struct.pack_into("<i", blob, OFF[n], int(allints[n]))
     for n in FLOATS:
@@ -2132,6 +2258,8 @@
     regions = [(PBASE, 4, np.frombuffer(bytes(blob), np.uint32))] + \
         [(base_of[n], 4 if n in FLAT or lanes > 1 else STRIDE, arrays[n].reshape(-1))
          for n in PTRS + ["impulse"] if arrays.get(n) is not None]
+    if arrays.get("ws") is not None:
+        regions.append((shadow_base, 4, shadow))
     assert all(arrays[n].flags.c_contiguous for n in PTRS + ["impulse"] if arrays.get(n) is not None)
     m = isasim.Machine(ins, lanes, regions=regions, sgpr={S_PARAM: PBASE & 0xFFFFFFFF, S_PARAM + 1: PBASE >> 32},
                        vgpr={0: 4 * np.arange(lanes)}, lds=np.zeros((lanes, NLDS), np.uint32), max_exec=max_exec,
diff --git a/robobee3d_amd/csrc/umpc_mi355x.hip b/robobee3d_amd/csrc/umpc_mi355x.hip
--- a/robobee3d_amd/csrc/umpc_mi355x.hip
+++ b/robobee3d_amd/csrc/umpc_mi355x.hip
@@ -205,6 +205,7 @@
   umpcasm::StepParams p;
   p.state = io.state; p.ctrl = io.ctrl; p.ref = io.ref; p.out = io.out; p.stats = io.stats; p.status = io.status;
   p.ws = (char *)h->ws + (size_t)umpcasm::WS_DS * (size_t)h->B * 4;
+  static_assert(umpcasm::STEP_SHADOW_ROWS <= umpcasm::WS_DS, "the iterate shadow lies inside the workspace");
   p.info = io.info; p.Ib = io.Ib; p.gain = io.gain; p.aT0 = io.actualT0;
   p.taskf = nullptr; p.weights = h->weights; p.wl = h->wl; p.wlu = h->wlu; p.wlw = h->wlw;
   p.done = nullptr; p.seq = 0; p.refstep = 0;
@@ -276,7 +277,8 @@
   const int grid = (h->B + kBlock - 1) / kBlock, qgrid = (h->B + kBlock / 4 - 1) / (kBlock / 4);
   if constexpr (sizeof(T) == 4) {
     static const bool no_asm = getenv("UMPC_NO_ASM_STEP") != nullptr;
-    const bool fits = (size_t)UMPC_CTRL_ROWS * (size_t)h->B * 4 < ((size_t)1 << 31);
+    static_assert(umpcasm::STEP_SHADOW_ROWS >= UMPC_CTRL_ROWS, "the shadow bounds the lane offsets");
+    const bool fits = (size_t)umpcasm::STEP_SHADOW_ROWS * (size_t)h->B * 4 < ((size_t)1 << 31);
     if (!no_asm && h->step_kernel != 1 && fits && K >= 1 && h->prm.maxIter >= 1) {
       umpcasm::StepArgs pa;
       umpcasm::StepParams &p = pa.p;
diff --git a/robobee3d_amd/csrc/umpc_step_asm.h b/robobee3d_amd/csrc/umpc_step_asm.h
--- a/robobee3d_amd/csrc/umpc_step_asm.h
+++ b/robobee3d_amd/csrc/umpc_step_asm.h
@@ -80,6 +80,7 @@
 static_assert(offsetof(StepArgs, h) == 296 && sizeof(StepHist) == 16, "StepHist layout");
 static_assert(offsetof(StepArgs, i) == 312 && sizeof(StepImp) == 16 && offsetof(StepImp, impstep) == 8, "StepImp layout");
 constexpr int STEP_LDS_BYTES_PER_LANE = 640;
+constexpr int STEP_SHADOW_ROWS = 128;
 }
 #define UMPC_STEP_ASM(voff, ldsaddr, params) asm volatile( \
   "s_mov_b64 s[2:3], s[4:5]\n" \
@@ -117,6 +118,13 @@
   "s_mov_b32 s100, 0x6aa56fa6\n" \
   "s_mov_b32 s101, 0x38d1b717\n" \
   "s_waitcnt lgkmcnt(0)\n" \
+  "s_mul_i32 s98, s10, 0x80\n" \
+  "s_mov_b32 s99, s47\n" \
+  "s_cmp_gt_u32 s98, s46\n" \
+  "s_cbranch_scc0 601f\n" \
+  "s_sub_i32 s99, s99, 1\n" \
+  "601:\n" \
+  "s_sub_i32 s98, s46, s98\n" \
   "s_mov_b32 s12, 0\n" \
   "21:\n" \
   "s_mov_b32 s14, 0\n" \
@@ -3928,6 +3936,76 @@
   "v_accvgpr_write_b32 a52, v121\n" \
   "v_accvgpr_write_b32 a135, v27\n" \
   "v_accvgpr_write_b32 a136, v14\n" \
+  "s_cmp_eq_u32 s12, 0\n" \
+  "s_cbranch_scc1 602f\n" \
+  "v_lshlrev_b32 v245, 2, v0\n" \
+  "s_lshl_b32 s4, s10, 2\n" \
+  "global_load_dwordx4 v[88:91], v245, s[98:99] nt\n" \
+  "v_add_u32 v245, s4, v245\n" \
+  "global_load_dwordx4 v[92:95], v245, s[98:99] nt\n" \
+  "v_add_u32 v245, s4, v245\n" \
+  "global_load_dwordx4 v[96:99], v245, s[98:99] nt\n" \
+  "v_add_u32 v245, s4, v245\n" \
+  "global_load_dwordx4 v[100:103], v245, s[98:99] nt\n" \
+  "v_add_u32 v245, s4, v245\n" \
+  "global_load_dwordx4 v[104:107], v245, s[98:99] nt\n" \
+  "v_add_u32 v245, s4, v245\n" \
+  "global_load_dwordx4 v[108:111], v245, s[98:99] nt\n" \
+  "v_add_u32 v245, s4, v245\n" \
+  "global_load_dwordx4 v[112:115], v245, s[98:99] nt\n" \
+  "v_add_u32 v245, s4, v245\n" \
+  "global_load_dwordx4 v[116:119], v245, s[98:99] nt\n" \
+  "v_add_u32 v245, s4, v245\n" \
+  "global_load_dwordx4 v[120:123], v245, s[98:99] nt\n" \
+  "v_add_u32 v245, s4, v245\n" \
+  "global_load_dwordx4 v[124:127], v245, s[98:99] nt\n" \
+  "v_add_u32 v245, s4, v245\n" \
+  "global_load_dwordx4 v[128:131], v245, s[98:99] nt\n" \
+  "v_add_u32 v245, s4, v245\n" \
+  "global_load_dwordx4 v[132:135], v245, s[98:99] nt\n" \
+  "v_add_u32 v245, s4, v245\n" \
+  "global_load_dwordx4 v[136:139], v245, s[98:99] nt\n" \
+  "v_add_u32 v245, s4, v245\n" \
+  "global_load_dwordx4 v[140:143], v245, s[98:99] nt\n" \
+  "v_add_u32 v245, s4, v245\n" \
+  "global_load_dwordx4 v[144:147], v245, s[98:99] nt\n" \
+  "v_add_u32 v245, s4, v245\n" \
+  "global_load_dwordx4 v[148:151], v245, s[98:99] nt\n" \
+  "v_add_u32 v245, s4, v245\n" \
+  "global_load_dwordx4 v[152:155], v245, s[98:99] nt\n" \
+  "v_add_u32 v245, s4, v245\n" \
+  "global_load_dwordx4 v[156:159], v245, s[98:99] nt\n" \
+  "v_add_u32 v245, s4, v245\n" \
+  "global_load_dwordx4 v[160:163], v245, s[98:99] nt\n" \
+  "v_add_u32 v245, s4, v245\n" \
+  "global_load_dwordx4 v[164:167], v245, s[98:99] nt\n" \
+  "v_add_u32 v245, s4, v245\n" \
+  "global_load_dwordx4 v[168:171], v245, s[98:99] nt\n" \
+  "v_add_u32 v245, s4, v245\n" \
+  "global_load_dwordx4 v[172:175], v245, s[98:99] nt\n" \
+  "v_add_u32 v245, s4, v245\n" \
+  "global_load_dwordx4 v[176:179], v245, s[98:99] nt\n" \
+  "v_add_u32 v245, s4, v245\n" \
+  "global_load_dwordx4 v[180:183], v245, s[98:99] nt\n" \
+  "v_add_u32 v245, s4, v245\n" \
+  "global_load_dwordx4 v[184:187], v245, s[98:99] nt\n" \
+  "v_add_u32 v245, s4, v245\n" \
+  "global_load_dwordx4 v[188:191], v245, s[98:99] nt\n" \
+  "v_add_u32 v245, s4, v245\n" \
+  "global_load_dwordx4 v[192:195], v245, s[98:99] nt\n" \
+  "v_add_u32 v245, s4, v245\n" \
+  "global_load_dwordx4 v[196:199], v245, s[98:99] nt\n" \
+  "v_add_u32 v245, s4, v245\n" \
+  "global_load_dwordx4 v[200:203], v245, s[98:99] nt\n" \
+  "v_add_u32 v245, s4, v245\n" \
+  "global_load_dwordx4 v[204:207], v245, s[98:99] nt\n" \
+  "v_add_u32 v245, s4, v245\n" \
+  "global_load_dwordx4 v[208:211], v245, s[98:99] nt\n" \
+  "v_add_u32 v245, s4, v245\n" \
+  "global_load_dwordx2 v[212:213], v245, s[98:99] nt\n" \
+  "s_waitcnt vmcnt(0)\n" \
+  "s_branch 603f\n" \
+  "602:\n" \
   "v_mov_b32 v245, v0\n" \
   "global_load_dword v88, v245, s[42:43] nt\n" \
   "v_add_u32 v245, s10, v245\n" \
@@ -4174,6 +4252,7 @@
   "global_load_dword v211, v245, s[42:43] nt\n" \
   "v_add_u32 v245, s10, v245\n" \
   "global_load_dword v212, v245, s[42:43] nt\n" \
+  "603:\n" \
   "v_mov_b32 v133, 0\n" \
   "v_mov_b32 v173, 0\n" \
   "v_mov_b32 v213, 0\n" \
@@ -6254,6 +6333,71 @@
   "v_pk_mul_f32 v[80:81], s[4:5], v[80:81] op_sel:[0,0] op_sel_hi:[0,1] neg_lo:[0,0] neg_hi:[0,0]\n" \
   "v_pk_mul_f32 v[82:83], s[4:5], v[82:83] op_sel:[0,0] op_sel_hi:[0,1] neg_lo:[0,0] neg_hi:[0,0]\n" \
   "30:\n" \
+  "s_add_i32 s4, s12, 1\n" \
+  "s_cmp_lt_i32 s4, s13\n" \
+  "s_cbranch_scc0 604f\n" \
+  "v_accvgpr_read_b32 v174, a182\n" \
+  "v_accvgpr_read_b32 v175, a183\n" \
+  "v_accvgpr_read_b32 v176, a184\n" \
+  "v_accvgpr_read_b32 v178, a185\n" \
+  "v_accvgpr_read_b32 v179, a186\n" \
+  "v_accvgpr_read_b32 v177, a187\n" \
+  "v_accvgpr_read_b32 v180, a188\n" \
+  "v_accvgpr_read_b32 v181, a189\n" \
+  "v_accvgpr_read_b32 v182, a190\n" \
+  "v_accvgpr_read_b32 v184, a191\n" \
+  "v_accvgpr_read_b32 v185, a192\n" \
+  "v_accvgpr_read_b32 v183, a193\n" \
+  "v_accvgpr_read_b32 v186, a194\n" \
+  "v_accvgpr_read_b32 v187, a195\n" \
+  "v_accvgpr_read_b32 v188, a196\n" \
+  "v_accvgpr_read_b32 v190, a197\n" \
+  "v_accvgpr_read_b32 v191, a198\n" \
+  "v_accvgpr_read_b32 v189, a199\n" \
+  "v_accvgpr_read_b32 v192, a200\n" \
+  "v_accvgpr_read_b32 v193, a201\n" \
+  "v_accvgpr_read_b32 v194, a202\n" \
+  "v_accvgpr_read_b32 v196, a203\n" \
+  "v_accvgpr_read_b32 v197, a204\n" \
+  "v_accvgpr_read_b32 v195, a205\n" \
+  "v_accvgpr_read_b32 v198, a206\n" \
+  "v_accvgpr_read_b32 v199, a207\n" \
+  "v_accvgpr_read_b32 v200, a208\n" \
+  "v_accvgpr_read_b32 v202, a209\n" \
+  "v_accvgpr_read_b32 v203, a210\n" \
+  "v_accvgpr_read_b32 v201, a211\n" \
+  "v_accvgpr_read_b32 v204, a212\n" \
+  "v_accvgpr_read_b32 v205, a213\n" \
+  "v_accvgpr_read_b32 v206, a214\n" \
+  "v_accvgpr_read_b32 v208, a215\n" \
+  "v_accvgpr_read_b32 v209, a216\n" \
+  "v_accvgpr_read_b32 v207, a217\n" \
+  "v_lshlrev_b32 v214, 2, v0\n" \
+  "s_mul_i32 s4, s10, 0x54\n" \
+  "v_add_u32 v214, s4, v214\n" \
+  "s_lshl_b32 s4, s10, 2\n" \
+  "global_store_dwordx4 v214, v[172:175], s[98:99] nt\n" \
+  "v_add_u32 v214, s4, v214\n" \
+  "global_store_dwordx4 v214, v[176:179], s[98:99] nt\n" \
+  "v_add_u32 v214, s4, v214\n" \
+  "global_store_dwordx4 v214, v[180:183], s[98:99] nt\n" \
+  "v_add_u32 v214, s4, v214\n" \
+  "global_store_dwordx4 v214, v[184:187], s[98:99] nt\n" \
+  "v_add_u32 v214, s4, v214\n" \
+  "global_store_dwordx4 v214, v[188:191], s[98:99] nt\n" \
+  "v_add_u32 v214, s4, v214\n" \
+  "global_store_dwordx4 v214, v[192:195], s[98:99] nt\n" \
+  "v_add_u32 v214, s4, v214\n" \
+  "global_store_dwordx4 v214, v[196:199], s[98:99] nt\n" \
+  "v_add_u32 v214, s4, v214\n" \
+  "global_store_dwordx4 v214, v[200:203], s[98:99] nt\n" \
+  "v_add_u32 v214, s4, v214\n" \
+  "global_store_dwordx4 v214, v[204:207], s[98:99] nt\n" \
+  "v_add_u32 v214, s4, v214\n" \
+  "global_store_dwordx4 v214, v[208:211], s[98:99] nt\n" \
+  "v_add_u32 v214, s4, v214\n" \
+  "global_store_dwordx2 v214, v[212:213], s[98:99] nt\n" \
+  "604:\n" \
   "s_mul_i32 s4, s10, 9\n" \
   "v_add_u32 v174, s4, v0\n" \
   "global_load_dword v186, v174, s[46:47] nt\n" \
@@ -6341,6 +6485,54 @@
   "v_add_u32 v174, s4, v0\n" \
   "global_load_dword v208, v174, s[42:43] nt\n" \
   "v_mov_b32 v227, 0\n" \
+  "s_add_i32 s4, s12, 1\n" \
+  "s_cmp_lt_i32 s4, s13\n" \
+  "s_cbranch_scc0 605f\n" \
+  "v_lshlrev_b32 v174, 2, v0\n" \
+  "s_lshl_b32 s4, s10, 2\n" \
+  "global_store_dwordx4 v174, v[88:91], s[98:99] nt\n" \
+  "v_add_u32 v174, s4, v174\n" \
+  "global_store_dwordx4 v174, v[92:95], s[98:99] nt\n" \
+  "v_add_u32 v174, s4, v174\n" \
+  "global_store_dwordx4 v174, v[96:99], s[98:99] nt\n" \
+  "v_add_u32 v174, s4, v174\n" \
+  "global_store_dwordx4 v174, v[100:103], s[98:99] nt\n" \
+  "v_add_u32 v174, s4, v174\n" \
+  "global_store_dwordx4 v174, v[104:107], s[98:99] nt\n" \
+  "v_add_u32 v174, s4, v174\n" \
+  "global_store_dwordx4 v174, v[108:111], s[98:99] nt\n" \
+  "v_add_u32 v174, s4, v174\n" \
+  "global_store_dwordx4 v174, v[112:115], s[98:99] nt\n" \
+  "v_add_u32 v174, s4, v174\n" \
+  "global_store_dwordx4 v174, v[116:119], s[98:99] nt\n" \
+  "v_add_u32 v174, s4, v174\n" \
+  "global_store_dwordx4 v174, v[120:123], s[98:99] nt\n" \
+  "v_add_u32 v174, s4, v174\n" \
+  "global_store_dwordx4 v174, v[124:127], s[98:99] nt\n" \
+  "v_add_u32 v174, s4, v174\n" \
+  "global_store_dwordx4 v174, v[128:131], s[98:99] nt\n" \
+  "v_add_u32 v174, s4, v174\n" \
+  "global_store_dwordx4 v174, v[132:135], s[98:99] nt\n" \
+  "v_add_u32 v174, s4, v174\n" \
+  "global_store_dwordx4 v174, v[136:139], s[98:99] nt\n" \
+  "v_add_u32 v174, s4, v174\n" \
+  "global_store_dwordx4 v174, v[140:143], s[98:99] nt\n" \
+  "v_add_u32 v174, s4, v174\n" \
+  "global_store_dwordx4 v174, v[144:147], s[98:99] nt\n" \
+  "v_add_u32 v174, s4, v174\n" \
+  "global_store_dwordx4 v174, v[148:151], s[98:99] nt\n" \
+  "v_add_u32 v174, s4, v174\n" \
+  "global_store_dwordx4 v174, v[152:155], s[98:99] nt\n" \
+  "v_add_u32 v174, s4, v174\n" \
+  "global_store_dwordx4 v174, v[156:159], s[98:99] nt\n" \
+  "v_add_u32 v174, s4, v174\n" \
+  "global_store_dwordx4 v174, v[160:163], s[98:99] nt\n" \
+  "v_add_u32 v174, s4, v174\n" \
+  "global_store_dwordx4 v174, v[164:167], s[98:99] nt\n" \
+  "v_add_u32 v174, s4, v174\n" \
+  "global_store_dwordx4 v174, v[168:171], s[98:99] nt\n" \
+  "s_branch 606f\n" \
+  "605:\n" \
   "v_mov_b32 v174, v0\n" \
   "global_store_dword v174, v88, s[42:43] nt\n" \
   "v_add_u32 v174, s10, v174\n" \
@@ -6624,6 +6816,7 @@
   "v_add_u32 v174, s10, v174\n" \
   "global_store_dword v174, v212, s[42:43] nt\n" \
   "v_add_u32 v174, s10, v174\n" \
+  "606:\n" \
   "s_waitcnt vmcnt(0)\n" \
   "v_pk_mul_f32 v[2:3], v[176:177], v[2:3] op_sel:[0,0] op_sel_hi:[1,1] neg_lo:[0,0] neg_hi:[0,0]\n" \
   "v_pk_mul_f32 v[88:89], v[176:177], v[88:89] op_sel:[0,0] op_sel_hi:[1,1] neg_lo:[0,0] neg_hi:[0,0]\n" \
@@ -8427,6 +8620,80 @@
   "s_and_saveexec_b64 s[32:33], s[62:63]\n" \
   "s_cbranch_execz 38f\n" \
   "v_mov_b32 v212, 0\n" \
+  "s_add_i32 s4, s12, 1\n" \
+  "s_cmp_lt_i32 s4, s13\n" \
+  "s_cbranch_scc0 607f\n" \
+  "v_mov_b32 v182, 0\n" \
+  "v_mov_b32 v183, 0\n" \
+  "v_mov_b32 v184, 0\n" \
+  "v_mov_b32 v185, 0\n" \
+  "v_lshlrev_b32 v174, 2, v0\n" \
+  "s_lshl_b32 s4, s10, 2\n" \
+  "global_store_dwordx4 v174, v[182:185], s[98:99] nt\n" \
+  "v_add_u32 v174, s4, v174\n" \
+  "global_store_dwordx4 v174, v[182:185], s[98:99] nt\n" \
+  "v_add_u32 v174, s4, v174\n" \
+  "global_store_dwordx4 v174, v[182:185], s[98:99] nt\n" \
+  "v_add_u32 v174, s4, v174\n" \
+  "global_store_dwordx4 v174, v[182:185], s[98:99] nt\n" \
+  "v_add_u32 v174, s4, v174\n" \
+  "global_store_dwordx4 v174, v[182:185], s[98:99] nt\n" \
+  "v_add_u32 v174, s4, v174\n" \
+  "global_store_dwordx4 v174, v[182:185], s[98:99] nt\n" \
+  "v_add_u32 v174, s4, v174\n" \
+  "global_store_dwordx4 v174, v[182:185], s[98:99] nt\n" \
+  "v_add_u32 v174, s4, v174\n" \
+  "global_store_dwordx4 v174, v[182:185], s[98:99] nt\n" \
+  "v_add_u32 v174, s4, v174\n" \
+  "global_store_dwordx4 v174, v[182:185], s[98:99] nt\n" \
+  "v_add_u32 v174, s4, v174\n" \
+  "global_store_dwordx4 v174, v[182:185], s[98:99] nt\n" \
+  "v_add_u32 v174, s4, v174\n" \
+  "global_store_dwordx4 v174, v[182:185], s[98:99] nt\n" \
+  "v_add_u32 v174, s4, v174\n" \
+  "global_store_dwordx4 v174, v[182:185], s[98:99] nt\n" \
+  "v_add_u32 v174, s4, v174\n" \
+  "global_store_dwordx4 v174, v[182:185], s[98:99] nt\n" \
+  "v_add_u32 v174, s4, v174\n" \
+  "global_store_dwordx4 v174, v[182:185], s[98:99] nt\n" \
+  "v_add_u32 v174, s4, v174\n" \
+  "global_store_dwordx4 v174, v[182:185], s[98:99] nt\n" \
+  "v_add_u32 v174, s4, v174\n" \
+  "global_store_dwordx4 v174, v[182:185], s[98:99] nt\n" \
+  "v_add_u32 v174, s4, v174\n" \
+  "global_store_dwordx4 v174, v[182:185], s[98:99] nt\n" \
+  "v_add_u32 v174, s4, v174\n" \
+  "global_store_dwordx4 v174, v[182:185], s[98:99] nt\n" \
+  "v_add_u32 v174, s4, v174\n" \
+  "global_store_dwordx4 v174, v[182:185], s[98:99] nt\n" \
+  "v_add_u32 v174, s4, v174\n" \
+  "global_store_dwordx4 v174, v[182:185], s[98:99] nt\n" \
+  "v_add_u32 v174, s4, v174\n" \
+  "global_store_dwordx4 v174, v[182:185], s[98:99] nt\n" \
+  "v_add_u32 v174, s4, v174\n" \
+  "global_store_dwordx4 v174, v[182:185], s[98:99] nt\n" \
+  "v_add_u32 v174, s4, v174\n" \
+  "global_store_dwordx4 v174, v[182:185], s[98:99] nt\n" \
+  "v_add_u32 v174, s4, v174\n" \
+  "global_store_dwordx4 v174, v[182:185], s[98:99] nt\n" \
+  "v_add_u32 v174, s4, v174\n" \
+  "global_store_dwordx4 v174, v[182:185], s[98:99] nt\n" \
+  "v_add_u32 v174, s4, v174\n" \
+  "global_store_dwordx4 v174, v[182:185], s[98:99] nt\n" \
+  "v_add_u32 v174, s4, v174\n" \
+  "global_store_dwordx4 v174, v[182:185], s[98:99] nt\n" \
+  "v_add_u32 v174, s4, v174\n" \
+  "global_store_dwordx4 v174, v[182:185], s[98:99] nt\n" \
+  "v_add_u32 v174, s4, v174\n" \
+  "global_store_dwordx4 v174, v[182:185], s[98:99] nt\n" \
+  "v_add_u32 v174, s4, v174\n" \
+  "global_store_dwordx4 v174, v[182:185], s[98:99] nt\n" \
+  "v_add_u32 v174, s4, v174\n" \
+  "global_store_dwordx4 v174, v[182:185], s[98:99] nt\n" \
+  "v_add_u32 v174, s4, v174\n" \
+  "global_store_dwordx2 v174, v[182:183], s[98:99] nt\n" \
+  "s_branch 38f\n" \
+  "607:\n" \
   "v_mov_b32 v174, v0\n" \
   "global_store_dword v174, v212, s[42:43]\n" \
   "v_add_u32 v174, s10, v174\n" \
diff --git a/robobee3d_amd/isasim.py b/robobee3d_amd/isasim.py
--- a/robobee3d_amd/isasim.py
+++ b/robobee3d_amd/isasim.py
@@ -627,6 +627,7 @@
     "v_and_b32": _bitop(lambda a, b: a & b),
     "v_or_b32": _bitop(lambda a, b: a | b),
     "v_lshrrev_b32": _bitop(lambda a, b: b >> (a & u64(31))),
+    "v_lshlrev_b32": _bitop(lambda a, b: (b << (a & u64(31))) & u64(0xFFFFFFFF)),
     "v_mul_u32_u24": _bitop(lambda a, b: ((a & u64(0xFFFFFF)) * (b & u64(0xFFFFFF))) & u64(0xFFFFFFFF)),
     "v_bfe_u32": lambda mc, t: mc.write(t[1], (mc.bits(t[2]) >> u32(t[3] & 31)) & u32((1 << t[4]) - 1)),
     "v_cvt_f32_i32": lambda mc, t: mc.wf(t[1], mc.bits(t[2]).view(np.int32).astype(f32)),
@@ -669,5 +670,6 @@
     VECTOR["v_cmp_%s_f32" % _op] = VECTOR["v_cmp_%s_f32_e64" % _op] = _cmp("f32")
 OPS = dict(SALU, **VECTOR)
 for _m in ("ds_read_b32", "ds_read_b64", "ds_read_b128", "ds_write_b32", "ds_write_b64", "ds_write_b128", "ds_min_f32",
-           "global_load_dword", "global_load_dwordx2", "global_load_dwordx4", "global_store_dword", "global_store_dwordx2"):
+           "global_load_dword", "global_load_dwordx2", "global_load_dwordx4", "global_store_dword", "global_store_dwordx2",
+           "global_store_dwordx4"):
     OPS[_m] = _ds if _m.startswith("ds_") else _global
```

Result: no change. 550.3 million (median of 6 runs) (+0.5%).
